# tusen-ai/SST

Hardware: AMD Instinct MI355X
Metric: LiDAR frames/sec (SST backbone fwd+bwd) at Waymo 0.32m voxels (higher is better)
Workload: dtype f32 (storage, accumulation, attention, LayerNorm, reductions: fp32; the dense products of the encoder layers from the EXACT three-way bf16 split of both fp32 operands, six bf16 MFMA products with fp32 accumulation - error vs float64 <= 2 x the fp32 matrix pipe's: tests/test_gpu_dense_f32x6.py)

## Files before the change

### include/sst_amd.h

```cpp
#ifndef SST_AMD_H
#define SST_AMD_H

#include <stdint.h>

#ifdef __cplusplus
extern "C" {
#endif

#define SST_OK 0
#define SST_ERR_ARG (-1)
#define SST_ERR_UNSUPPORTED (-2)
#define SST_ERR_KEYSPACE (-3)

typedef enum { SST_REDUCE_SUM = 0, SST_REDUCE_MEAN = 1, SST_REDUCE_MAX = 2 } sst_reduce_t;

const char* sst_version(void);

int sst_dynamic_voxelize_f32(const float* d_points, int64_t n, int64_t row_stride,
                             const float voxel_size[3], const float coors_range[6],
                             int32_t* d_coors, int64_t coors_stride, int coors_col0, int batch_idx,
                             void* stream);
void sst_dynamic_voxelize_grid(const float voxel_size[3], const float coors_range[6], int32_t grid_xyz[3]);

int64_t sst_scan_workspace_bytes(int64_t n);
// ... 162 lines not shown
  float* out_b;
  int32_t p, bias_side, transpose_out, reserved;
} sst_wgrad_problem_bf16;
int64_t sst_wgrad_group_workspace_bytes(const sst_wgrad_problem_bf16* problems, int n);
int sst_wgrad_group_bf16(const sst_wgrad_problem_bf16* problems, int n, void* d_workspace, void* stream);
typedef struct sst_cast_problem_bf16 {
  const float* src;
  void* dst;
  int64_t ld_src;
  int32_t rows, cols, transpose, reserved;
} sst_cast_problem_bf16;
int sst_cast_group_bf16(const sst_cast_problem_bf16* problems, int n, void* stream);

int sst_gather_rows_f32(const float* d_src, int64_t ld_src, const int32_t* d_idx, int64_t n_out, int c,
                        float fill, float* d_out, int64_t ld_out, void* stream);
int sst_add_table_rows_f32(const float* d_x, int64_t ldx, const float* d_table, int64_t ld_table, const int32_t* d_idx, int64_t m,
                           int c, float* d_out, int64_t ld_out, void* stream);
int sst_scatter_rows_f32(const float* d_src, int64_t ld_src, const int32_t* d_idx, int64_t n_src, int c,
                         float* d_out, int64_t ld_out, void* stream);

int sst_add_layernorm_act_fwd_f32(const float* d_x, const float* d_res, const float* d_weight, const float* d_bias,
                                  int64_t m, int c, float eps, int act, float* d_y, float* d_sum, float* d_stats,
                                  void* stream);
int sst_add_layernorm_act_bwd_f32(const float* d_dy, const float* d_sum, const float* d_stats, const float* d_weight,
                                  const float* d_bias, int act, int64_t m, int c, float* d_dx, float* d_dweight,
                                  float* d_dbias, void* d_workspace, void* stream);
int sst_add_layernorm_fwd_f32(const float* d_x, const float* d_res, const float* d_weight, const float* d_bias,
                              int64_t m, int c, float eps, float* d_y, float* d_sum, float* d_stats,
                              void* stream);
int sst_add_layernorm_pos_fwd_f32(const float* d_x, const float* d_res, const float* d_weight, const float* d_bias, int64_t m,
                                  int c, float eps, float* d_y, float* d_sum, float* d_stats, const float* d_pos_table,
                                  const int32_t* d_pos_idx, float* d_y_plus_pos, void* stream);
int64_t sst_add_layernorm_bwd_workspace_bytes(int64_t m, int c);
int sst_add_layernorm_bwd_f32(const float* d_dy, const float* d_sum, const float* d_stats,
                              const float* d_weight, int64_t m, int c, float* d_dx, float* d_dweight,
                              float* d_dbias, void* d_workspace, void* stream);
int64_t sst_colsum_workspace_bytes(int64_t m, int c);
int sst_colsum_f32(const float* d_x, int64_t m, int c, int64_t ld, float* d_out, void* d_workspace, void* stream);

int64_t sst_weight_grad_workspace_bytes(int64_t m, int out, int in);
int sst_weight_grad_f32(const float* d_dy, const float* d_x, int64_t m, int out, int in, int64_t ld_dy,
                        int64_t ld_x, float* d_dw, float* d_db, void* d_workspace, void* stream);
typedef struct sst_wgrad_problem_f32 {
  const float* dy;
  const float* x;
  int64_t m, ld_dy, ld_x;
  float* dw;
  float* db;
  int32_t out, in;
  const float* x_add_rows;
  const int32_t* x_add_index;
} sst_wgrad_problem_f32;
int64_t sst_weight_grad_group_workspace_bytes(const sst_wgrad_problem_f32* problems, int n);
int sst_weight_grad_group_f32(const sst_wgrad_problem_f32* problems, int n, void* d_workspace, void* stream);
int64_t sst_weight_grad_group_f32x6_workspace_bytes(const sst_wgrad_problem_f32* problems, int n);
int sst_weight_grad_group_f32x6(const sst_wgrad_problem_f32* problems, int n, void* d_workspace, void* stream);
int sst_weight_grad_group_f32x6_plan(const sst_wgrad_problem_f32* problems, int n, int* tiles, int* slices,
                                     int64_t* tokens_per_slice, int* lean_slices);

int64_t sst_bn_workspace_bytes(int64_t n, int c);
int sst_bn_stats_f32(const float* d_x, int64_t n, int c, int64_t ld, float* d_mean, float* d_var,
                     void* d_workspace, void* stream);
int sst_bn_act_fwd_f32(const float* d_x, int64_t n, int c, int64_t ldx, const float* d_scale,
                       const float* d_shift, int act, float* d_y, int64_t ldy, void* stream);
int sst_bn_act_bwd_reduce_f32(const float* d_dy, const float* d_x, int64_t n, int c, int64_t lddy, int64_t ldx,
                              const float* d_mean, const float* d_invstd, const float* d_scale,
                              const float* d_shift, int act, float* d_sum_g, float* d_sum_gxhat,
                              void* d_workspace, void* stream);
int sst_bn_act_bwd_apply_f32(const float* d_dy, const float* d_x, int64_t n, int c, int64_t lddy, int64_t ldx,
                             const float* d_mean, const float* d_invstd, const float* d_scale,
                             const float* d_shift, const float* d_coef_a, const float* d_coef_b, float coef_scale,
                             int act, float* d_dx, int64_t lddx, void* stream);
int sst_bn_prepare_f32(const float* d_x, int64_t n, int c, int64_t ld, const float* d_weight, const float* d_bias,
                       float eps, float* d_running_mean, float* d_running_var, float factor, float* d_out4,
                       void* d_workspace, void* stream);
int sst_bn_prepare_tracked_f32(const float* d_x, int64_t n, int c, int64_t ld, const float* d_weight,
                               const float* d_bias, float eps, float* d_running_mean, float* d_running_var,
                               float factor, int64_t* d_num_batches_tracked, float* d_out4, void* d_workspace,
                               void* stream);
int sst_vfe_linear_moments_f32(const float* d_x, int64_t ldx, int64_t n, int k, const float* d_w, int64_t ldw, int c,
                               float* d_y, int64_t ldy, void* d_workspace, void* stream);
int sst_bn_prepare_from_partials_f32(int64_t n, int c, const float* d_weight, const float* d_bias, float eps,
                                     float* d_running_mean, float* d_running_var, float factor,
                                     int64_t* d_num_batches_tracked, float* d_out4, void* d_workspace, void* stream);
int sst_bn_stats_from_partials_f32(int64_t n, int c, float* d_mean, float* d_var, void* d_workspace, void* stream);
int sst_bn_act_pool_bwd_reduce_f32(const float* d_dy, const float* d_x, int64_t n, int c, int64_t lddy, int64_t ldx,
                                   const float* d_mean, const float* d_invstd, const float* d_scale, const float* d_shift,
                                   int act, const int32_t* d_group, const int32_t* d_arg, const float* d_dpool, int64_t ldp,
                                   float* d_sum_g, float* d_sum_gxhat, void* d_workspace, void* stream);
int sst_bn_act_pool_bwd_apply_f32(const float* d_dy, const float* d_x, int64_t n, int c, int64_t lddy, int64_t ldx,
                                  const float* d_mean, const float* d_invstd, const float* d_scale, const float* d_shift,
                                  const float* d_coef_a, const float* d_coef_b, float coef_scale, int act,
                                  const int32_t* d_group, const int32_t* d_arg, const float* d_dpool, int64_t ldp, float* d_dx,
                                  int64_t lddx, void* stream);
int sst_bn_act_res_fwd_f32(const float* d_x, int64_t n, int c, int64_t ldx, const float* d_res, int64_t ldr,
                           const float* d_scale, const float* d_shift, int act, float* d_y, int64_t ldy, void* stream);
int sst_bn_act_res_bwd_reduce_f32(const float* d_dy, const float* d_x, const float* d_res, int64_t n, int c,
                                  int64_t lddy, int64_t ldx, int64_t ldr, const float* d_mean, const float* d_invstd,
                                  const float* d_scale, const float* d_shift, int act, float* d_sum_g,
                                  float* d_sum_gxhat, void* d_workspace, void* stream);
int sst_bn_act_res_bwd_apply_f32(const float* d_dy, const float* d_x, const float* d_res, int64_t n, int c,
                                 int64_t lddy, int64_t ldx, int64_t ldr, const float* d_mean, const float* d_invstd,
                                 const float* d_scale, const float* d_shift, const float* d_coef_a,
                                 const float* d_coef_b, float coef_scale, int act, float* d_dres, int64_t lddres,
                                 float* d_dx, int64_t lddx, void* stream);

int sst_tall_linear_f32(const float* d_x, int64_t ldx, const float* d_w, int64_t ldw, const float* d_bias,
                        int64_t m, int n, int k, int trans_w, int accumulate, float* d_y, int64_t ldy,
                        void* stream);
int sst_tall_linear_ln_f32(const float* d_x, int64_t ldx, const float* d_w, int64_t ldw, const float* d_bias, int64_t m, int k,
                           const float* d_res, int64_t ldres, const float* d_ln_weight, const float* d_ln_bias, float eps,
                           float* d_y, float* d_sum, float* d_stats, const float* d_pos_table, const int32_t* d_pos_idx,
                           float* d_y_plus_pos, void* stream);
int sst_tall_linear_epi_f32x3(const float* d_x, int64_t ldx, const float* d_w, int64_t ldw, int trans_w, const float* d_bias,
                              int64_t m, int k, int n, int epilogue, const float* d_aux_in, float* d_aux_out, int64_t ldaux,
                              float* d_y, int64_t ldy, void* stream);
int sst_tall_linear_ln_f32x3(const float* d_x, int64_t ldx, const float* d_w, int64_t ldw, const float* d_bias, int64_t m, int k,
                             const float* d_res, int64_t ldres, const float* d_ln_weight, const float* d_ln_bias, float eps,
                             float* d_y, float* d_sum, float* d_stats, const float* d_pos_table, const int32_t* d_pos_idx,
                             float* d_y_plus_pos, void* stream);
int sst_tall_linear_epi_f32x6(const float* d_x, int64_t ldx, const float* d_w, int64_t ldw, int trans_w, const float* d_bias,
                              int64_t m, int k, int n, int epilogue, const float* d_aux_in, float* d_aux_out, int64_t ldaux,
                              float* d_y, int64_t ldy, void* stream);
int sst_tall_linear_epi2_f32x6(const float* d_x, const float* d_x2, int x2_from_col, int64_t ldx, const float* d_w, int64_t ldw,
                               int trans_w, const float* d_bias, int64_t m, int k, int n, int epilogue, const float* d_aux_in,
                               float* d_aux_out, int64_t ldaux, float* d_y, int64_t ldy, void* stream);
int sst_tall_linear_add_rows_f32x6(const float* d_x, int64_t ldx, const float* d_w, int64_t ldw, int64_t m, int k, int n,
                                   const float* d_rows, int64_t ldrows, const int32_t* d_row_index, float* d_y, int64_t ldy,
                                   void* stream);
int sst_inproj_pos_f32x6(const float* d_x, int64_t ldx, const float* d_rows, const int32_t* d_index, const float* d_w, int64_t ldw,
                         const float* d_bias, int64_t m, float* d_y, int64_t ldy, void* stream);
int sst_tall_linear_f32x6_partition(int64_t m, int groups, int64_t* row_blocks, int64_t* rows_per_wave);
int sst_tall_linear_ln_f32x6(const float* d_x, int64_t ldx, const float* d_w, int64_t ldw, const float* d_bias, int64_t m, int k,
                             const float* d_res, int64_t ldres, const float* d_ln_weight, const float* d_ln_bias, float eps,
                             float* d_y, float* d_sum, float* d_stats, const float* d_pos_table, const int32_t* d_pos_idx,
                             float* d_y_plus_pos, void* stream);
int sst_add_layernorm_bwd2_f32(const float* d_dy, const float* d_dy2, const float* d_sum, const float* d_stats,
                               const float* d_weight, int64_t m, int c, float* d_dx, float* d_dweight, float* d_dbias,
                               void* d_workspace, void* stream);
typedef struct sst_encoder_layer_fwd_args {
  int64_t m, n_windows;
  int32_t n_heads, act, max_tokens, impl;
  float eps, scale;
  const float *x, *xp;
  const float *w_in, *b_in, *w_out, *b_out, *w1, *b1, *w2, *b2, *n1w, *n1b, *n2w, *n2b;
  const int32_t *tok, *winoff, *order;
  const float* pos_table;
  const int32_t* pos_idx;
  float *qkv, *o, *lse, *y1, *s1, *st1, *pre, *h, *s2, *y2, *st2, *y2p;
  const float* head_scale;
  void* wpack;
  const float* xpos_table;
  const int32_t* xpos_idx;
} sst_encoder_layer_fwd_args;
typedef struct sst_encoder_layer_bwd_args {
  int64_t m, n_windows;
  int32_t n_heads, act, max_tokens, impl;
  float eps, scale;
  const float *dy2, *dy2p;
  const float *x, *xp, *qkv, *o, *lse, *s1, *st1, *y1, *pre, *h, *s2, *st2;
  const float *w_in, *w_out, *w1, *w2, *n1w, *n2w;
  const int32_t *tok, *winoff, *order;
  float *ds2, *dpre, *ds1, *d_o, *dqkv;
  float *dw_in, *db_in, *dwo, *dbo, *dw1, *db1, *dw2, *db2, *dn1w, *dn1b, *dn2w, *dn2b;
  void* workspace;
  const float* head_scale;
  float* cos_r;
  float* dy1;
  const void* wpack;
  const float* xpos_table;
  const int32_t* xpos_idx;
} sst_encoder_layer_bwd_args;
int64_t sst_encoder_layer_bwd_workspace_bytes(int64_t m, int n_heads);
int64_t sst_encoder_layer_wpack_bytes(void);
int sst_encoder_layer_fwd_f32x6(const sst_encoder_layer_fwd_args* args, void* stream);
int sst_encoder_layer_bwd_f32x6(const sst_encoder_layer_bwd_args* args, void* stream);

typedef struct sst_encoder_tail_fwd_args {
  int64_t m;
  int32_t act, reserved;
  float eps, reserved_f;
  const float *o, *x;
  const void* packed;
  const float *b_out, *b1, *b2, *n1w, *n1b, *n2w, *n2b;
  const float* pos_table;
  const int32_t* pos_idx;
  float *s1, *st1, *y1, *pre, *h, *s2, *st2, *y2, *y2p;
} sst_encoder_tail_fwd_args;
typedef struct sst_encoder_tail_bwd_args {
  int64_t m;
  int32_t act, reserved;
  const float *dy2, *dy2p, *s2, *st2, *pre, *s1, *st1;
  const void* packed;
  const float *n1w, *n2w;
  float *ds2, *dpre, *ds1, *d_o;
  float *dn2w, *dn2b, *dn1w, *dn1b;
  void* workspace;
} sst_encoder_tail_bwd_args;
int64_t sst_encoder_tail_pack_bytes(void);
int sst_encoder_tail_pack_f32x6(const float* d_w_out, const float* d_w1, const float* d_w2, void* d_packed, void* stream);
int sst_encoder_tail_pack_f32x6_many(const float* const* d_w_out, const float* const* d_w1, const float* const* d_w2,
                                     void* const* d_packed, int n, void* stream);
int64_t sst_encoder_tail_bwd_workspace_bytes(int64_t m);
int sst_encoder_tail_fwd_f32x6(const sst_encoder_tail_fwd_args* args, void* stream);
int sst_encoder_tail_bwd_f32x6(const sst_encoder_tail_bwd_args* args, void* stream);

typedef struct sst_encoder_tail_fwd_bf16_args {
  int64_t m;
  int32_t act, reserved;
  float eps, reserved_f;
  const void *o, *x;
  const void* packed;
  const float *b_out, *b1, *b2, *n1w, *n1b, *n2w, *n2b;
  const float* pos_table;
  const int32_t* pos_idx;
  void* s1;
  float* st1;
  void *y1, *pre, *h, *s2;
  float* st2;
  void *y2, *y2p;
} sst_encoder_tail_fwd_bf16_args;
typedef struct sst_encoder_tail_bwd_bf16_args {
  int64_t m;
  int32_t act, reserved;
  const void *dy2, *dy2p, *s2;
  const float* st2;
  const void *pre, *s1;
  const float* st1;
  const void* packed;
  const float *n1w, *n2w;
  void *ds2, *dpre, *ds1, *d_o;
  float *dn2w, *dn2b, *dn1w, *dn1b;
  void* workspace;
} sst_encoder_tail_bwd_bf16_args;
int64_t sst_encoder_tail_pack_bf16_bytes(void);
int sst_encoder_tail_pack_bf16(const float* d_w_out, const float* d_w1, const float* d_w2, void* d_packed, void* stream);
int sst_encoder_tail_pack_bf16_many(const float* const* d_w_out, const float* const* d_w1, const float* const* d_w2,
                                    void* const* d_packed, int n, void* stream);
int64_t sst_encoder_tail_bwd_bf16_workspace_bytes(int64_t m);
int sst_encoder_tail_fwd_bf16(const sst_encoder_tail_fwd_bf16_args* args, void* stream);
int sst_encoder_tail_bwd_bf16(const sst_encoder_tail_bwd_bf16_args* args, void* stream);

typedef struct sst_encoder_layer_fwd_bf16_args {
  int64_t m, n_windows;
  int32_t n_heads, act, max_tokens, reserved;
  float eps, scale;
  const void *x, *xp;
  const void *wqk, *wv, *wout, *w1, *w2;
  const float *b_in, *b_out, *b1, *b2, *n1w, *n1b, *n2w, *n2b;
  const int32_t *tok, *winoff, *order;
  const float* pos_table;
  const int32_t* pos_idx;
  void *qk, *v, *o;
  float* lse;
  void *y1, *s1;
  float* st1;
  void *pre, *h, *s2;
  float* st2;
  void *y2, *y2p;
  const float* head_scale;
  const void* wpack;
} sst_encoder_layer_fwd_bf16_args;
typedef struct sst_encoder_layer_bwd_bf16_args {
  int64_t m, n_windows;
  int32_t n_heads, act, max_tokens, reserved;
  float eps, scale;
  const void *dy2, *dy2p;
  const void *x, *xp, *qk, *v, *o;
  const float* lse;
  const void* s1;
  const float* st1;
  const void *y1, *pre, *h, *s2;
  const float* st2;
  const void *wqk_t, *wv_t, *wout_t, *w1_t, *w2_t;
  const float *n1w, *n2w;
  const int32_t *tok, *winoff, *order;
  void *ds2, *dpre, *dy1, *ds1, *d_o, *dqkv, *dxp, *dx;
  float *dw_in, *db_in, *dwo, *dbo, *dw1, *db1, *dw2, *db2, *dn1w, *dn1b, *dn2w, *dn2b;
  void* workspace;
  const float* head_scale;
  float* cos_r;
  const void* wpack;
} sst_encoder_layer_bwd_bf16_args;
int64_t sst_encoder_layer_bwd_bf16_workspace_bytes(int64_t m);
int sst_encoder_layer_fwd_bf16(const sst_encoder_layer_fwd_bf16_args* args, void* stream);
int sst_encoder_layer_bwd_bf16(const sst_encoder_layer_bwd_bf16_args* args, void* stream);

int sst_tall_linear_epi_f32(const float* d_x, int64_t ldx, const float* d_w, int64_t ldw, int trans_w, const float* d_bias,
                            int64_t m, int k, int n, int epilogue, const float* d_aux_in, float* d_aux_out, int64_t ldaux,
                            float* d_y, int64_t ldy, void* stream);
int sst_tall_linear_gelu_f32(const float* d_x, int64_t ldx, const float* d_w, int64_t ldw, const float* d_bias,
                             int64_t m, int n, int k, int trans_w, int mode, float* d_aux, float* d_y, int64_t ldy,
                             void* stream);

void* sst_event_create(void);
void sst_event_destroy(void* ev);
float sst_event_elapsed_ms(void* start, void* stop);
int sst_sra_attn_profile_next_fwd(void* start, void* stop);
int sst_sra_attn_profile_next_bwd(void* start, void* stop);

int64_t sst_connected_components_workspace_bytes(int64_t n);
int sst_connected_components_xy_f32(const float* d_points, int64_t ld, const int32_t* d_batch, int64_t n, float dist,
                                    int32_t* d_labels, int32_t* d_num_components, void* d_workspace, void* stream);

int64_t sst_dynamic_point_pool_workspace_bytes(int64_t n_rois, int64_t n_pts);
int sst_dynamic_point_pool_f32(const float* d_rois, const int32_t* d_rois_batch, int64_t n_rois, const float* d_pts,
                               int64_t ld_pts, const int32_t* d_pts_batch, int64_t n_pts, const float* extra_wlh,
                               int max_inbox_point, int64_t max_all_pts, int64_t* d_out_pts_idx,
                               int64_t* d_out_roi_idx, float* d_out_feats, int64_t* d_num_out, void* d_workspace,
                               void* stream);

int sst_spconv_candidates_i32(const int32_t* d_coors, int64_t n, const int32_t* in_shape, const int32_t* out_shape,
                              const int32_t* ksize, const int32_t* stride, const int32_t* padding,
                              const int32_t* dilation, int transpose, int32_t* d_rows, void* stream);
int sst_spconv_inverse_to_map_i32(const int32_t* d_inverse, int64_t total, int32_t* d_in2out, void* stream);
int sst_spconv_grid_subm_i32(const int32_t* d_coors, int64_t n, int batch, const int32_t* shape, const int32_t* ksize,
                             const int32_t* dilation, int32_t* d_grid, int32_t* d_in2out, int32_t* d_out2in,
                             void* stream);
int64_t sst_spconv_grid_conv_workspace_bytes(int64_t cells);
int sst_spconv_grid_conv_count_i32(const int32_t* d_coors, int64_t n, int batch, const int32_t* in_shape,
                                   const int32_t* out_shape, const int32_t* ksize, const int32_t* stride,
                                   const int32_t* padding, const int32_t* dilation, int transpose, void* d_workspace,
                                   int32_t* d_num_out, void* stream);
int sst_spconv_grid_conv_maps_i32(const int32_t* d_coors, int64_t n, int batch, const int32_t* in_shape,
                                  const int32_t* out_shape, const int32_t* ksize, const int32_t* stride,
                                  const int32_t* padding, const int32_t* dilation, int transpose, void* d_workspace,
                                  int64_t m, int32_t* d_outids, int32_t* d_in2out, int32_t* d_out2in, void* stream);
int sst_spconv_subm_map_i32(const int32_t* d_coors, int64_t n, const int32_t* shape, const int32_t* ksize,
                            const int32_t* dilation, const uint64_t* d_sorted_keys, const uint32_t* d_perm,
                            int32_t* d_in2out, void* stream);
int sst_spconv_invert_map_i32(const int32_t* d_in2out, int kvol, int64_t n, int64_t m, int32_t* d_out2in,
                              void* stream);
int64_t sst_spconv_pair_lists_workspace_bytes(int kvol, int64_t n);
int sst_spconv_pair_lists_i32(const int32_t* d_in2out, int kvol, int64_t n, int32_t* d_pairs, int32_t* d_num,
                              void* d_workspace, void* stream);
int sst_spconv_gather_gemm_f32(const float* d_x, int64_t ldx, const int32_t* d_map, int64_t m, int kvol,
                               const float* d_w, int cin, int cout, int trans_w, const float* d_bias, float* d_y,
                               int64_t ldy, int form, void* stream);
int sst_spconv_maxpool_fwd_f32(const float* d_x, int64_t ldx, const int32_t* d_out2in, int64_t m, int kvol, int c,
                               float* d_y, int64_t ldy, void* stream);
int sst_spconv_maxpool_bwd_f32(const float* d_x, int64_t ldx, const float* d_y, int64_t ldy, const float* d_dy,
                               int64_t lddy, const int32_t* d_in2out, int64_t n, int kvol, int c, float* d_dx,
                               int64_t lddx, void* stream);
int64_t sst_spconv_conv_os_workspace_bytes(int kvol, int cin, int cout);
int sst_spconv_conv_os_tile_rows(int64_t m, int cout, int tile_cfg);
int sst_spconv_os_tile_work_i32(const int32_t* d_map, int64_t m, int kvol, int tile_rows, int32_t* d_work, void* stream);
int sst_spconv_conv_os_f32(const float* d_x, int64_t ldx, const int32_t* d_map, int64_t m, int kvol, const float* d_w,
                           int cin, int cout, int trans_w, const float* d_bias, float* d_y, int64_t ldy,
                           int tile_cfg, const int32_t* d_tile_order, void* d_workspace, void* stream);
int sst_spconv_conv_os_f32x3(const float* d_x, int64_t ldx, const int32_t* d_map, int64_t m, int kvol, const float* d_w,
                             int cin, int cout, int trans_w, const float* d_bias, float* d_y, int64_t ldy, int tile_cfg,
                             const int32_t* d_tile_order, void* d_workspace, void* stream);
int64_t sst_spconv_conv_os_f32x6_workspace_bytes(int kvol, int cin, int cout);
int sst_spconv_conv_os_f32x6(const float* d_x, int64_t ldx, const int32_t* d_map, int64_t m, int kvol, const float* d_w,
                             int cin, int cout, int trans_w, const float* d_bias, float* d_y, int64_t ldy, int tile_cfg,
// ... 555 lines not shown
```

### sst_amd/_lib.py

```python
import ctypes
import os
import subprocess

import torch

_HERE = os.path.dirname(os.path.abspath(__file__))
_CSRC = os.path.join(_HERE, 'csrc')
LIB_PATH = os.path.join(_CSRC, 'libsst_amd.so')

_lib = None

c_i64 = ctypes.c_int64
c_i32 = ctypes.c_int
c_f32 = ctypes.c_float
c_ptr = ctypes.c_void_p



class WgradProblemBF16(ctypes.Structure):
    _fields_ = [('a', c_ptr), ('b', c_ptr), ('lda', c_i64), ('ldb', c_i64), ('m', c_i64), ('out_w', c_ptr),
                ('out_b', c_ptr), ('p', ctypes.c_int32), ('bias_side', ctypes.c_int32),
                ('transpose_out', ctypes.c_int32), ('reserved', ctypes.c_int32)]


class CastProblemBF16(ctypes.Structure):
    _fields_ = [('src', c_ptr), ('dst', c_ptr), ('ld_src', c_i64), ('rows', ctypes.c_int32), ('cols', ctypes.c_int32),
                ('transpose', ctypes.c_int32), ('reserved', ctypes.c_int32)]


class ClusterLossTask(ctypes.Structure):
    _fields_ = [('logits', c_ptr), ('reg_preds', c_ptr), ('labels', c_ptr), ('bbox_targets', c_ptr), ('bbox_weights', c_ptr),
                ('d_logits', c_ptr), ('d_reg_preds', c_ptr), ('classes', ctypes.c_int32), ('reserved', ctypes.c_int32)]


class WgradProblemF32(ctypes.Structure):
    _fields_ = [('dy', c_ptr), ('x', c_ptr), ('m', c_i64), ('ld_dy', c_i64), ('ld_x', c_i64), ('dw', c_ptr), ('db', c_ptr),
                ('out', ctypes.c_int32), ('inn', ctypes.c_int32), ('x_add_rows', c_ptr), ('x_add_index', c_ptr)]


def _struct(name, doc, fields):
    return type(name, (ctypes.Structure,), {'__doc__': doc, '_fields_': fields})


_I32 = ctypes.c_int32
RoiAssignArgs = _struct('RoiAssignArgs', 'sst_roi_assign_args of include/sst_amd.h', (
    [(k, ctypes.c_void_p) for k in ('props', 'prop_labels', 'prop_offsets', 'gts', 'gt_labels', 'gt_offsets', 'iou', 'max_iou',
                                    'argmax')]
    + [(k, c_i64) for k in ('n_props', 'n_gts', 'ld')]
    + [(k, _I32) for k in ('prop_cols', 'gt_cols', 'batch', 'num_classes', 'class_mask', 'reserved')]))
RoiSampleArgs = _struct('RoiSampleArgs', 'sst_roi_sample_args of include/sst_amd.h', (
    [(k, ctypes.c_void_p) for k in ('props', 'prop_labels', 'prop_offsets', 'gts', 'gt_labels', 'gt_offsets', 'iou', 'max_iou',
                                    'argmax', 'keys', 'assigned', 'rois', 'src', 'gt_index', 'labels', 'iou_out', 'soft_label',
                                    'reg_mask', 'targets', 'counts')]
    + [(k, c_i64) for k in ('n_props', 'n_gts', 'ld', 'max_props_per_sample')]
    + [(k, _I32) for k in ('prop_cols', 'gt_cols', 'batch', 'num_classes', 'class_mask', 'num', 'num_expected_pos', 'n_pieces')]
    + [(k, ctypes.c_float * 16) for k in ('pos_iou_thr', 'neg_iou_thr', 'min_pos_iou')]
    + [('piece_thr', ctypes.c_float * 8)]
    + [(k, ctypes.c_double * 16) for k in ('cls_pos_thr', 'cls_neg_thr')]
    + [('piece_frac', ctypes.c_double * 8)]))
RoiLossArgs = _struct('RoiLossArgs', 'sst_roi_loss_args of include/sst_amd.h', (
    [(k, ctypes.c_void_p) for k in ('cls_score', 'bbox_pred', 'nonempty', 'rois', 'soft_label', 'reg_mask', 'targets',
                                    'gt_index', 'labels', 'gts')]
    + [(k, c_i64) for k in ('n', 'n_gts')]
    + [(k, _I32) for k in ('roi_cols', 'gt_cols', 'with_corner', 'car_index')]
    + [(k, ctypes.c_float) for k in ('beta', 'w_cls', 'w_reg', 'w_corner')]
    + [('code_weight', ctypes.c_float * 7), ('reserved', ctypes.c_float)]))

AnchorGrid = _struct('AnchorGrid', 'sst_anchor_grid of include/sst_amd.h', (
    [('centers', ctypes.c_void_p)] + [(k, _I32) for k in ('H', 'W', 'n_sizes', 'n_rots')]
    + [('sizes', ctypes.c_float * 3 * 8), ('rots', ctypes.c_float * 4)]))
AnchorLossArgs = _struct('AnchorLossArgs', 'sst_anchor_loss_args of include/sst_amd.h', (
    [(k, ctypes.c_void_p) for k in ('cls_score', 'bbox_pred', 'dir_pred', 'assigned', 'gts', 'gt_labels', 'gt_offsets',
                                    'pos_counts')]
    + [('n_gts', c_i64)]
    + [(k, _I32) for k in ('gt_cols', 'batch', 'num_classes', 'smooth_l1', 'sin_diff', 'reserved')]
    + [(k, ctypes.c_float) for k in ('gamma', 'alpha', 'w_cls', 'w_bbox', 'w_dir', 'beta', 'pos_weight', 'dir_offset')]
    + [('code_weight', ctypes.c_float * 7), ('reserved_f', ctypes.c_float)]))

FgSampleArgs = _struct('FgSampleArgs', 'sst_fg_sample_args of include/sst_amd.h', (
    [(k, ctypes.c_void_p) for k in ('logits', 'votes', 'points', 'batch_idx', 'extra_mask', 'slot', 'mask', 'src', 'centers',
                                    'batch_out', 'points_out', 'info', 'aux', 'aux_out', 'aux_inv')]
    + [(k, c_i64) for k in ('n', 'ld_logits', 'ld_votes', 'ld_points', 'max_rows', 'aux_rows')]
    + [(k, _I32) for k in ('num_classes', 'point_cols', 'batch', 'batch_is_i64', 'apply_rule', 'sample_major')]
    + [('thresholds', ctypes.c_float * 32)]))
FgGatherArgs = _struct('FgGatherArgs', 'sst_fg_gather_args of include/sst_amd.h', (
    [(k, ctypes.c_void_p) for k in ('idx', 'logits', 'votes', 'feats', 'points', 'out', 'points_out')]
    + [(k, c_i64) for k in ('m', 'n', 'ld_logits', 'ld_votes', 'ld_feats', 'ld_points')]
    + [(k, _I32) for k in ('c_logits', 'c_votes', 'c_feats', 'c_points')]))
FgGroupSampleArgs = _struct('FgGroupSampleArgs', 'sst_fg_group_sample_args of include/sst_amd.h', (
    [(k, ctypes.c_void_p) for k in ('logits', 'votes', 'points', 'batch_idx', 'extra_mask', 'slot', 'mask', 'src', 'centers',
                                    'batch_out', 'points_out', 'info')]
    + [(k, c_i64) for k in ('n', 'ld_logits', 'ld_votes', 'ld_points', 'max_rows')]
    + [(k, _I32) for k in ('num_groups', 'num_logits', 'point_cols', 'batch', 'batch_is_i64', 'apply_rule')]
    + [('offset_scale', ctypes.c_float), ('thresholds', ctypes.c_float * 32), ('group_begin', ctypes.c_uint8 * 33),
       ('group_class', ctypes.c_uint8 * 64)]))
FgVirtualRowsArgs = _struct('FgVirtualRowsArgs', 'sst_fg_virtual_rows_args of include/sst_amd.h', (
    [(k, ctypes.c_void_p) for k in ('src', 'centers', 'feats', 'logits', 'points', 'out', 'clipped')]
    + [(k, c_i64) for k in ('m', 'n', 'ld_feats', 'ld_logits', 'ld_points')]
    + [(k, _I32) for k in ('c_feats', 'c_logits', 'c_points', 'reserved')]
    + [('lo', ctypes.c_float * 3), ('hi', ctypes.c_float * 3)]))
DeformConvShape = _struct('DeformConvShape', 'sst_deform_conv_shape of include/sst_amd.h', [
    (k, _I32) for k in ('batch', 'in_channels', 'height', 'width', 'out_channels', 'kernel_h', 'kernel_w', 'stride_h', 'stride_w',
                        'pad_h', 'pad_w', 'dil_h', 'dil_w', 'groups', 'deform_groups', 'reserved')])
OptimHyper = _struct('OptimHyper', 'sst_optim_hyper of include/sst_amd.h', (
    [(k, ctypes.c_double * 8) for k in ('lr', 'wd', 'b1', 'b2', 'eps')]
    + [(k, ctypes.c_double) for k in ('max_norm', 'growth_factor', 'backoff_factor')]
    + [(k, _I32) for k in ('growth_interval', 'scale_mode', 'skip_nonfinite', 'n_groups')]))
TrackletTargetsArgs = _struct('TrackletTargetsArgs', 'sst_tracklet_targets_args of include/sst_amd.h', (
    [(k, ctypes.c_void_p) for k in ('boxes', 'ts', 'scores', 'trk_offsets', 'cand_boxes', 'cand_ts', 'cand_offsets',
                                    'trk_cand_offsets', 'trk_class', 'chosen', 'counts', 'matched', 'overlaps',
                                    'assigned_gt_inds', 'rois', 'src', 'frame_inds', 'gt_index', 'labels', 'iou_out',
                                    'scores_out', 'soft_label', 'reg_mask', 'targets', 'pos_gt_bboxes')]
    + [(k, c_i64) for k in ('n_rows', 'n_cand_rows', 'n_cands', 'n_tracklets')]
    + [(k, _I32) for k in ('num_classes', 'object_centric')]
    + [(k, ctypes.c_float) for k in ('candidate_thresh', 'iou_thr')]
    + [(k, ctypes.c_double * 16) for k in ('cls_pos_thr', 'cls_neg_thr')]))
TrackletRowsArgs = _struct('TrackletRowsArgs', 'sst_tracklet_rows_args of include/sst_amd.h', (
    [(k, ctypes.c_void_p) for k in ('feats', 'xyz', 'pts_frame_inds', 'pts_inds', 'roi_inds', 'roi_frame_inds', 'roi_scores',
                                    'out', 'xyz_out')]
    + [(k, c_i64) for k in ('m', 'n_points', 'n_rois', 'ld_feats', 'ld_xyz')]
    + [(k, _I32) for k in ('feat_cols', 'xyz_cols', 'combined', 'with_roi_scores')]))
IncrArgs = _struct('IncrArgs', 'sst_incr_args of include/sst_amd.h', (
    [('points', ctypes.c_void_p * 16), ('frame_inds', ctypes.c_void_p * 16), ('n_points', c_i64 * 16)]
    + [(k, ctypes.c_void_p) for k in ('boxes', 'box_offsets', 'keys', 'counts', 'out', 'workspace')]
    + [('workspace_bytes', c_i64), ('seg_base', c_i64 * (16 * 20))]
    + [(k, _I32) for k in ('n_samples', 'cols', 'n_frames', 'n_queries', 'n_boxes', 'max_crop_points', 'lower_bound')]
    + [(k, _I32 * 4) for k in ('q_inc', 'q_lo', 'q_hi')]
    + [('q_tag', ctypes.c_float * 4), ('lo', ctypes.c_float * 3), ('vs', ctypes.c_float * 3), ('grid', _I32 * 3)]))
IncrDeltaArgs = _struct('IncrDeltaArgs', 'sst_incr_delta_args of include/sst_amd.h', (
    [('base', ctypes.c_void_p * 8), ('n_base', c_i64 * 8), ('ld_base', c_i64 * 8), ('query', ctypes.c_void_p),
     ('n_query', c_i64), ('ld_query', c_i64), ('mask', ctypes.c_void_p), ('workspace', ctypes.c_void_p),
     ('workspace_bytes', c_i64), ('n_clouds', _I32), ('lower_bound', _I32), ('lo', ctypes.c_float * 3),
     ('vs', ctypes.c_float * 3), ('grid', _I32 * 3)]))
FrameTransformArgs = _struct('FrameTransformArgs', 'sst_frame_transform_args of include/sst_amd.h', (
    [('src', ctypes.c_void_p * 8), ('dst', ctypes.c_void_p * 8), ('n', c_i64 * 8), ('mat', (ctypes.c_float * 12) * 8),
     ('n_clouds', _I32), ('cols', _I32)]))
AugmentParams = _struct('AugmentParams', 'sst_augment_params of include/sst_amd.h', (
    [(k, _I32) for k in ('flip_h', 'flip_v', 'rotate', 'shuffle')]
    + [(k, ctypes.c_float) for k in ('cos', 'sin', 'scale', 'angle')]
    + [('trans', ctypes.c_float * 3), ('reserved', ctypes.c_float), ('range', ctypes.c_float * 6), ('seed', ctypes.c_uint64)]))
AugmentArgs = _struct('AugmentArgs', 'sst_augment_args of include/sst_amd.h', (
    [(k, ctypes.c_void_p) for k in ('points', 'row_offsets', 'n_pasted', 'block_offsets', 'params', 'planes', 'plane_offsets',
                                    'out', 'counts', 'workspace')]
    + [(k, c_i64) for k in ('workspace_bytes', 'n_total')]
    + [(k, _I32) for k in ('batch', 'cols', 'n_blocks', 'n_planes', 'norm_mask', 'reserved')]
    + [('norm_mean', ctypes.c_float * 8), ('norm_std', ctypes.c_float * 8)]))
AugmentBoxArgs = _struct('AugmentBoxArgs', 'sst_augment_box_args of include/sst_amd.h', (
    [(k, ctypes.c_void_p) for k in ('boxes', 'labels', 'box_offsets', 'params', 'boxes_out', 'labels_out', 'counts')]
    + [(k, _I32) for k in ('batch', 'cols', 'n_boxes', 'filter', 'always_rotate', 'reserved')]))
FgGroupOffsets = _struct('FgGroupOffsets', 'sst_fg_group_offsets of include/sst_amd.h', [('off', c_i64 * 33)])

_P = ctypes.c_void_p
EncoderLayerFwdArgs = _struct('EncoderLayerFwdArgs', 'sst_encoder_layer_fwd_args of include/sst_amd.h', (
    [('m', c_i64), ('n_windows', c_i64)] + [(k, ctypes.c_int32) for k in ('n_heads', 'act', 'max_tokens', 'impl')]
    + [('eps', ctypes.c_float), ('scale', ctypes.c_float)]
    + [(k, _P) for k in ('x', 'xp', 'w_in', 'b_in', 'w_out', 'b_out', 'w1', 'b1', 'w2', 'b2', 'n1w', 'n1b', 'n2w', 'n2b',
                         'tok', 'winoff', 'order', 'pos_table', 'pos_idx',
                         'qkv', 'o', 'lse', 'y1', 's1', 'st1', 'pre', 'h', 's2', 'y2', 'st2', 'y2p', 'head_scale', 'wpack',
                         'xpos_table', 'xpos_idx')]))
EncoderLayerBwdArgs = _struct('EncoderLayerBwdArgs', 'sst_encoder_layer_bwd_args of include/sst_amd.h', (
    [('m', c_i64), ('n_windows', c_i64)] + [(k, ctypes.c_int32) for k in ('n_heads', 'act', 'max_tokens', 'impl')]
    + [('eps', ctypes.c_float), ('scale', ctypes.c_float)]
    + [(k, _P) for k in ('dy2', 'dy2p', 'x', 'xp', 'qkv', 'o', 'lse', 's1', 'st1', 'y1', 'pre', 'h', 's2', 'st2',
                         'w_in', 'w_out', 'w1', 'w2', 'n1w', 'n2w', 'tok', 'winoff', 'order',
                         'ds2', 'dpre', 'ds1', 'd_o', 'dqkv',
                         'dw_in', 'db_in', 'dwo', 'dbo', 'dw1', 'db1', 'dw2', 'db2', 'dn1w', 'dn1b', 'dn2w', 'dn2b',
                         'workspace', 'head_scale', 'cos_r', 'dy1', 'wpack', 'xpos_table', 'xpos_idx')]))


EncoderTailFwdArgs = _struct('EncoderTailFwdArgs', 'sst_encoder_tail_fwd_args of include/sst_amd.h', (
    [('m', c_i64), ('act', ctypes.c_int32), ('reserved', ctypes.c_int32), ('eps', ctypes.c_float), ('reserved_f', ctypes.c_float)]
    + [(k, _P) for k in ('o', 'x', 'packed', 'b_out', 'b1', 'b2', 'n1w', 'n1b', 'n2w', 'n2b', 'pos_table', 'pos_idx',
                         's1', 'st1', 'y1', 'pre', 'h', 's2', 'st2', 'y2', 'y2p')]))
EncoderTailBwdArgs = _struct('EncoderTailBwdArgs', 'sst_encoder_tail_bwd_args of include/sst_amd.h', (
    [('m', c_i64), ('act', ctypes.c_int32), ('reserved', ctypes.c_int32)]
    + [(k, _P) for k in ('dy2', 'dy2p', 's2', 'st2', 'pre', 's1', 'st1', 'packed', 'n1w', 'n2w',
                         'ds2', 'dpre', 'ds1', 'd_o', 'dn2w', 'dn2b', 'dn1w', 'dn1b', 'workspace')]))

EncoderTailFwdBF16Args = _struct('EncoderTailFwdBF16Args', 'sst_encoder_tail_fwd_bf16_args of include/sst_amd.h', (
    [('m', c_i64), ('act', ctypes.c_int32), ('reserved', ctypes.c_int32), ('eps', ctypes.c_float), ('reserved_f', ctypes.c_float)]
    + [(k, _P) for k in ('o', 'x', 'packed', 'b_out', 'b1', 'b2', 'n1w', 'n1b', 'n2w', 'n2b', 'pos_table', 'pos_idx',
                         's1', 'st1', 'y1', 'pre', 'h', 's2', 'st2', 'y2', 'y2p')]))
EncoderTailBwdBF16Args = _struct('EncoderTailBwdBF16Args', 'sst_encoder_tail_bwd_bf16_args of include/sst_amd.h', (
    [('m', c_i64), ('act', ctypes.c_int32), ('reserved', ctypes.c_int32)]
    + [(k, _P) for k in ('dy2', 'dy2p', 's2', 'st2', 'pre', 's1', 'st1', 'packed', 'n1w', 'n2w',
                         'ds2', 'dpre', 'ds1', 'd_o', 'dn2w', 'dn2b', 'dn1w', 'dn1b', 'workspace')]))


EncoderLayerFwdBF16Args = _struct('EncoderLayerFwdBF16Args', 'sst_encoder_layer_fwd_bf16_args of include/sst_amd.h', (
    [('m', c_i64), ('n_windows', c_i64)] + [(k, ctypes.c_int32) for k in ('n_heads', 'act', 'max_tokens', 'reserved')]
    + [('eps', ctypes.c_float), ('scale', ctypes.c_float)]
    + [(k, _P) for k in ('x', 'xp', 'wqk', 'wv', 'wout', 'w1', 'w2', 'b_in', 'b_out', 'b1', 'b2', 'n1w', 'n1b', 'n2w', 'n2b',
                         'tok', 'winoff', 'order', 'pos_table', 'pos_idx',
                         'qk', 'v', 'o', 'lse', 'y1', 's1', 'st1', 'pre', 'h', 's2', 'st2', 'y2', 'y2p', 'head_scale', 'wpack')]))
EncoderLayerBwdBF16Args = _struct('EncoderLayerBwdBF16Args', 'sst_encoder_layer_bwd_bf16_args of include/sst_amd.h', (
    [('m', c_i64), ('n_windows', c_i64)] + [(k, ctypes.c_int32) for k in ('n_heads', 'act', 'max_tokens', 'reserved')]
    + [('eps', ctypes.c_float), ('scale', ctypes.c_float)]
    + [(k, _P) for k in ('dy2', 'dy2p', 'x', 'xp', 'qk', 'v', 'o', 'lse', 's1', 'st1', 'y1', 'pre', 'h', 's2', 'st2',
                         'wqk_t', 'wv_t', 'wout_t', 'w1_t', 'w2_t', 'n1w', 'n2w', 'tok', 'winoff', 'order',
                         'ds2', 'dpre', 'dy1', 'ds1', 'd_o', 'dqkv', 'dxp', 'dx',
                         'dw_in', 'db_in', 'dwo', 'dbo', 'dw1', 'db1', 'dw2', 'db2', 'dn1w', 'dn1b', 'dn2w', 'dn2b',
                         'workspace', 'head_scale', 'cos_r', 'wpack')]))


_SIGNATURES = {
    'sst_version': (ctypes.c_char_p, []),
    'sst_dynamic_voxelize_f32': (c_i32, [c_ptr, c_i64, c_i64, c_ptr, c_ptr, c_ptr, c_i64, c_i32, c_i32, c_ptr]),
    'sst_dynamic_voxelize_grid': (None, [c_ptr, c_ptr, c_ptr]),
    'sst_scan_workspace_bytes': (c_i64, [c_i64]),
    'sst_exclusive_scan_i32': (c_i32, [c_ptr, c_ptr, c_i64, c_ptr, c_ptr, c_ptr]),
    'sst_sort_workspace_bytes': (c_i64, [c_i64]),
    'sst_sort_pairs_u64': (c_i32, [c_ptr, c_ptr, c_ptr, c_i64, c_i32, c_ptr, c_ptr]),
    'sst_unique_workspace_bytes': (c_i64, [c_i64]),
    'sst_unique_rows': (c_i32, [c_ptr, c_i32, c_i64, c_i32, c_i64, c_ptr, c_ptr, c_i32,
                                c_ptr, c_ptr, c_ptr, c_ptr, c_ptr, c_ptr, c_ptr]),
    'sst_unpack_keys': (c_i32, [c_ptr, c_i64, c_i32, c_ptr, c_ptr, c_ptr, c_i32, c_i64, c_i32, c_ptr]),
    'sst_segment_reduce_fwd_f32': (c_i32, [c_ptr, c_i64, c_i32, c_ptr, c_ptr, c_ptr, c_i64, c_i32, c_ptr, c_ptr,
                                           c_ptr, c_ptr]),
    'sst_encoder_layer_bwd_workspace_bytes': (c_i64, [c_i64, c_i32]),
    'sst_tall_linear_f32x6_partition': (c_i32, [c_i64, c_i32, c_ptr, c_ptr]),
    'sst_inproj_pos_f32x6': (c_i32, [c_ptr, c_i64, c_ptr, c_ptr, c_ptr, c_i64, c_ptr, c_i64, c_ptr, c_i64, c_ptr]),
    'sst_encoder_layer_wpack_bytes': (c_i64, []),
    'sst_encoder_layer_fwd_f32x6': (c_i32, [c_ptr, c_ptr]),
    'sst_encoder_layer_bwd_f32x6': (c_i32, [c_ptr, c_ptr]),
    'sst_encoder_tail_pack_bytes': (c_i64, []),
    'sst_encoder_tail_pack_f32x6': (c_i32, [c_ptr, c_ptr, c_ptr, c_ptr, c_ptr]),
    'sst_encoder_tail_pack_f32x6_many': (c_i32, [c_ptr, c_ptr, c_ptr, c_ptr, c_i32, c_ptr]),
    'sst_encoder_tail_bwd_workspace_bytes': (c_i64, [c_i64]),
    'sst_encoder_tail_fwd_f32x6': (c_i32, [c_ptr, c_ptr]),
    'sst_encoder_tail_bwd_f32x6': (c_i32, [c_ptr, c_ptr]),
    'sst_encoder_tail_pack_bf16_bytes': (c_i64, []),
    'sst_encoder_tail_pack_bf16': (c_i32, [c_ptr, c_ptr, c_ptr, c_ptr, c_ptr]),
    'sst_encoder_tail_pack_bf16_many': (c_i32, [c_ptr, c_ptr, c_ptr, c_ptr, c_i32, c_ptr]),
    'sst_encoder_tail_bwd_bf16_workspace_bytes': (c_i64, [c_i64]),
    'sst_encoder_tail_fwd_bf16': (c_i32, [c_ptr, c_ptr]),
    'sst_encoder_tail_bwd_bf16': (c_i32, [c_ptr, c_ptr]),
    'sst_encoder_layer_bwd_bf16_workspace_bytes': (c_i64, [c_i64]),
    'sst_encoder_layer_fwd_bf16': (c_i32, [c_ptr, c_ptr]),
    'sst_encoder_layer_bwd_bf16': (c_i32, [c_ptr, c_ptr]),
    'sst_segment_reduce_work_words': (c_i64, [c_i64, c_i64, c_i32]),
    'sst_segment_reduce_fwd_work_f32': (c_i32, [c_ptr, c_i64, c_i32, c_ptr, c_ptr, c_ptr, c_i64, c_i32, c_ptr, c_ptr,
                                                c_ptr, c_ptr, c_i64, c_ptr, c_ptr, c_ptr]),
    'sst_vfe_linear_moments_f32': (c_i32, [c_ptr, c_i64, c_i64, c_i32, c_ptr, c_i64, c_i32, c_ptr, c_i64, c_ptr, c_ptr]),
    'sst_bn_prepare_from_partials_f32': (c_i32, [c_i64, c_i32, c_ptr, c_ptr, c_f32, c_ptr, c_ptr, c_f32, c_ptr, c_ptr, c_ptr,
                                                 c_ptr]),
    'sst_bn_stats_from_partials_f32': (c_i32, [c_i64, c_i32, c_ptr, c_ptr, c_ptr, c_ptr]),
    'sst_bn_act_pool_bwd_reduce_f32': (c_i32, [c_ptr, c_ptr, c_i64, c_i32, c_i64, c_i64, c_ptr, c_ptr, c_ptr, c_ptr, c_i32,
                                               c_ptr, c_ptr, c_ptr, c_i64, c_ptr, c_ptr, c_ptr, c_ptr]),
    'sst_bn_act_pool_bwd_apply_f32': (c_i32, [c_ptr, c_ptr, c_i64, c_i32, c_i64, c_i64, c_ptr, c_ptr, c_ptr, c_ptr, c_ptr,
                                              c_ptr, c_f32, c_i32, c_ptr, c_ptr, c_ptr, c_i64, c_ptr, c_i64, c_ptr]),
    'sst_tall_linear_add_rows_f32x6': (c_i32, [c_ptr, c_i64, c_ptr, c_i64, c_i64, c_i32, c_i32, c_ptr, c_i64, c_ptr, c_ptr,
                                               c_i64, c_ptr]),
    'sst_segment_long_scratch_bytes': (c_i64, [c_i64, c_i64, c_i32]),
    'sst_segment_reduce_long_f32': (c_i32, [c_ptr, c_i64, c_i32, c_ptr, c_ptr, c_i32, c_ptr, c_i64, c_i32, c_ptr, c_ptr, c_ptr,
                                            c_ptr]),
    'sst_segment_reduce_profile_next': (c_i32, [c_ptr, c_ptr]),
    'sst_segment_reduce_bwd_f32': (c_i32, [c_ptr, c_i64, c_i32, c_ptr, c_i32, c_ptr, c_ptr, c_ptr, c_i64, c_i32,
                                           c_ptr, c_ptr, c_ptr]),
    'sst_ingroup_rank_workspace_bytes': (c_i64, [c_i64]),
    'sst_ingroup_rank_i64': (c_i32, [c_ptr, c_i64, c_i32, c_ptr, c_ptr, c_ptr]),
    'sst_window_coors': (c_i32, [c_ptr, c_i32, c_i64, c_ptr, c_ptr, c_ptr, c_ptr, c_ptr, c_ptr, c_ptr]),
    'sst_window_order_i32': (c_i32, [c_ptr, c_i32, c_i32, c_ptr, c_ptr]),
    'sst_region_batching_workspace_bytes': (c_i64, [c_i64]),
    'sst_region_batching': (c_i32, [c_ptr, c_ptr, c_i64, c_i32, c_ptr, c_i32] + [c_ptr] * 15 + [c_ptr, c_ptr]),
    'sst_frame_windows_per_sample': (c_i64, [c_ptr, c_ptr]),
    'sst_frame_voxels_i32': (c_i32, [c_ptr, c_ptr, c_ptr, c_i64, c_i32, c_ptr, c_i32, c_ptr, c_ptr, c_ptr, c_ptr,
                                     c_ptr, c_ptr, c_ptr]),
    'sst_window_plan_workspace_bytes': (c_i64, [c_i64, c_i64]),
    'sst_window_plan_i32': (c_i32, [c_ptr, c_ptr, c_i64, c_i32, c_ptr, c_ptr, c_ptr, c_i32, ctypes.c_uint32] + [c_ptr] * 11),
    'sst_sra_attn_fwd_f32': (c_i32, [c_ptr, c_ptr, c_ptr, c_i64, c_i64, c_i64, c_ptr, c_ptr, c_i64, c_i32,
                                     c_f32, c_i32, c_i32, c_ptr, c_i64, c_ptr, c_ptr]),
    'sst_sra_attn_bwd_f32': (c_i32, [c_ptr] * 6 + [c_i64] * 5 + [c_ptr, c_ptr, c_i64, c_i64, c_i32, c_f32,
                                                                 c_i32, c_i32, c_ptr, c_ptr, c_ptr,
                                                                 c_i64, c_i64, c_i64, c_ptr, c_ptr]),
    'sst_sra_attn_fwd_ord_f32': (c_i32, [c_ptr, c_ptr, c_ptr, c_i64, c_i64, c_i64, c_ptr, c_ptr, c_ptr, c_i64, c_i32,
                                         c_f32, c_i32, c_i32, c_ptr, c_i64, c_ptr, c_ptr]),
    'sst_sra_attn_bwd_ord_f32': (c_i32, [c_ptr] * 6 + [c_i64] * 5 + [c_ptr, c_ptr, c_ptr, c_i64, c_i64, c_i32, c_f32,
                                                                     c_i32, c_i32, c_ptr, c_ptr, c_ptr,
                                                                     c_i64, c_i64, c_i64, c_ptr, c_ptr]),
    'sst_sra_attn_bwd_workspace_bytes': (c_i64, [c_i64, c_i32]),
    'sst_sra_attn_cos_fwd_f32': (c_i32, [c_ptr, c_ptr, c_ptr, c_i64, c_i64, c_i64, c_ptr, c_ptr, c_ptr, c_i64, c_i32,
                                         c_ptr, c_i32, c_ptr, c_i64, c_ptr, c_ptr]),
    'sst_sra_attn_cos_bwd_f32': (c_i32, [c_ptr] * 6 + [c_i64] * 5 + [c_ptr, c_ptr, c_ptr, c_i64, c_i64, c_i32, c_ptr,
                                                                     c_i32, c_ptr, c_ptr, c_ptr,
                                                                     c_i64, c_i64, c_i64, c_ptr, c_ptr]),
    'sst_sra_attn_fwd_bf16': (c_i32, [c_ptr, c_ptr, c_ptr, c_i64, c_i64, c_i64, c_ptr, c_ptr, c_i64, c_i32, c_f32, c_i32,
                                      c_ptr, c_i64, c_ptr, c_ptr]),
    'sst_sra_attn_bwd_bf16': (c_i32, [c_ptr] * 6 + [c_i64] * 5 + [c_ptr, c_ptr, c_i64, c_i32, c_f32, c_i32, c_ptr, c_ptr,
                                                                  c_ptr, c_i64, c_i64, c_i64, c_ptr]),
    'sst_sra_attn_bf16_profile_next': (c_i32, [c_i32, c_ptr, c_ptr]),
    'sst_sra_attn_fwd_ord_bf16': (c_i32, [c_ptr, c_ptr, c_ptr, c_i64, c_i64, c_i64, c_ptr, c_ptr, c_ptr, c_i64, c_i32, c_f32,
                                          c_i32, c_ptr, c_i64, c_ptr, c_ptr]),
    'sst_sra_attn_bwd_ord_bf16': (c_i32, [c_ptr] * 6 + [c_i64] * 5 + [c_ptr, c_ptr, c_ptr, c_i64, c_i32, c_f32, c_i32, c_ptr,
                                                                      c_ptr, c_ptr, c_i64, c_i64, c_i64, c_ptr]),
    'sst_sra_attn_cos_fwd_bf16': (c_i32, [c_ptr, c_ptr, c_ptr, c_i64, c_i64, c_i64, c_ptr, c_ptr, c_ptr, c_i64, c_i32, c_ptr,
                                          c_i32, c_ptr, c_i64, c_ptr, c_ptr]),
    'sst_sra_attn_cos_bwd_bf16': (c_i32, [c_ptr] * 6 + [c_i64] * 5 + [c_ptr, c_ptr, c_ptr, c_i64, c_i32, c_ptr, c_i32, c_ptr,
                                                                      c_ptr, c_ptr, c_i64, c_i64, c_i64, c_ptr, c_ptr]),
    'sst_add_layernorm_fwd_bf16': (c_i32, [c_ptr, c_ptr, c_ptr, c_ptr, c_i64, c_i32, c_f32, c_ptr, c_ptr, c_ptr, c_ptr,
                                           c_ptr, c_ptr, c_ptr]),
    'sst_add_layernorm_bwd_bf16': (c_i32, [c_ptr, c_ptr, c_ptr, c_ptr, c_ptr, c_i64, c_i32, c_ptr, c_ptr, c_ptr, c_ptr,
                                           c_ptr]),
    'sst_cast_add_pos_bf16': (c_i32, [c_ptr, c_i32, c_i64, c_i32, c_ptr, c_ptr, c_ptr, c_ptr]),
    'sst_weight_grad_group_workspace_bytes': (c_i64, [c_ptr, c_i32]),
    'sst_weight_grad_group_f32': (c_i32, [c_ptr, c_i32, c_ptr, c_ptr]),
    'sst_weight_grad_group_f32x6_workspace_bytes': (c_i64, [c_ptr, c_i32]),
    'sst_weight_grad_group_f32x6': (c_i32, [c_ptr, c_i32, c_ptr, c_ptr]),
    'sst_weight_grad_group_f32x6_plan': (c_i32, [c_ptr, c_i32, c_ptr, c_ptr, c_ptr, c_ptr]),
    'sst_tall_linear_ln_f32': (c_i32, [c_ptr, c_i64, c_ptr, c_i64, c_ptr, c_i64, c_i32, c_ptr, c_i64, c_ptr, c_ptr, c_f32, c_ptr,
                                       c_ptr, c_ptr, c_ptr, c_ptr, c_ptr, c_ptr]),
    'sst_tall_linear_ln_f32x3': (c_i32, [c_ptr, c_i64, c_ptr, c_i64, c_ptr, c_i64, c_i32, c_ptr, c_i64, c_ptr, c_ptr, c_f32, c_ptr,
                                         c_ptr, c_ptr, c_ptr, c_ptr, c_ptr, c_ptr]),
    'sst_tall_linear_epi_f32x3': (c_i32, [c_ptr, c_i64, c_ptr, c_i64, c_i32, c_ptr, c_i64, c_i32, c_i32, c_i32, c_ptr, c_ptr,
                                          c_i64, c_ptr, c_i64, c_ptr]),
    'sst_tall_linear_ln_f32x6': (c_i32, [c_ptr, c_i64, c_ptr, c_i64, c_ptr, c_i64, c_i32, c_ptr, c_i64, c_ptr, c_ptr, c_f32, c_ptr,
                                         c_ptr, c_ptr, c_ptr, c_ptr, c_ptr, c_ptr]),
    'sst_tall_linear_epi_f32x6': (c_i32, [c_ptr, c_i64, c_ptr, c_i64, c_i32, c_ptr, c_i64, c_i32, c_i32, c_i32, c_ptr, c_ptr,
                                          c_i64, c_ptr, c_i64, c_ptr]),
    'sst_tall_linear_epi2_f32x6': (c_i32, [c_ptr, c_ptr, c_i32, c_i64, c_ptr, c_i64, c_i32, c_ptr, c_i64, c_i32, c_i32, c_i32,
                                           c_ptr, c_ptr, c_i64, c_ptr, c_i64, c_ptr]),
    'sst_add_layernorm_bwd2_f32': (c_i32, [c_ptr, c_ptr, c_ptr, c_ptr, c_ptr, c_i64, c_i32, c_ptr, c_ptr, c_ptr, c_ptr, c_ptr]),
    'sst_tall_linear_epi_f32': (c_i32, [c_ptr, c_i64, c_ptr, c_i64, c_i32, c_ptr, c_i64, c_i32, c_i32, c_i32, c_ptr, c_ptr,
                                        c_i64, c_ptr, c_i64, c_ptr]),
    'sst_tall_linear_bf16': (c_i32, [c_ptr, c_i64, c_ptr, c_ptr, c_i64, c_i32, c_i32, c_i32, c_ptr, c_ptr, c_i64, c_ptr,
                                     c_i64, c_ptr]),
    'sst_tall_linear_bf16_partition': (c_i32, [c_i64, c_i32, c_i32, c_i32, c_ptr, c_ptr]),
    'sst_tall_linear_ln_bf16': (c_i32, [c_ptr, c_i64, c_ptr, c_ptr, c_i64, c_i32, c_ptr, c_i64, c_ptr, c_ptr, c_f32, c_ptr, c_ptr,
                                        c_ptr, c_ptr, c_ptr, c_ptr, c_ptr]),
    'sst_wgrad_group_workspace_bytes': (c_i64, [c_ptr, c_i32]),
    'sst_wgrad_group_bf16': (c_i32, [c_ptr, c_i32, c_ptr, c_ptr]),
    'sst_cast_group_bf16': (c_i32, [c_ptr, c_i32, c_ptr]),
    'sst_gather_rows_f32': (c_i32, [c_ptr, c_i64, c_ptr, c_i64, c_i32, c_f32, c_ptr, c_i64, c_ptr]),
    'sst_add_table_rows_f32': (c_i32, [c_ptr, c_i64, c_ptr, c_i64, c_ptr, c_i64, c_i32, c_ptr, c_i64, c_ptr]),
    'sst_scatter_rows_f32': (c_i32, [c_ptr, c_i64, c_ptr, c_i64, c_i32, c_ptr, c_i64, c_ptr]),
    'sst_add_layernorm_fwd_f32': (c_i32, [c_ptr, c_ptr, c_ptr, c_ptr, c_i64, c_i32, c_f32, c_ptr, c_ptr, c_ptr,
                                          c_ptr]),
    'sst_add_layernorm_bwd_workspace_bytes': (c_i64, [c_i64, c_i32]),
    'sst_add_layernorm_pos_fwd_f32': (c_i32, [c_ptr, c_ptr, c_ptr, c_ptr, c_i64, c_i32, c_f32, c_ptr, c_ptr, c_ptr, c_ptr, c_ptr,
                                              c_ptr, c_ptr]),
    'sst_add_layernorm_act_fwd_f32': (c_i32, [c_ptr, c_ptr, c_ptr, c_ptr, c_i64, c_i32, c_f32, c_i32, c_ptr, c_ptr, c_ptr,
                                              c_ptr]),
    'sst_add_layernorm_act_bwd_f32': (c_i32, [c_ptr, c_ptr, c_ptr, c_ptr, c_ptr, c_i32, c_i64, c_i32, c_ptr, c_ptr, c_ptr,
                                              c_ptr, c_ptr]),
    'sst_add_layernorm_bwd_f32': (c_i32, [c_ptr, c_ptr, c_ptr, c_ptr, c_i64, c_i32, c_ptr, c_ptr, c_ptr, c_ptr,
                                          c_ptr]),
    'sst_weight_grad_workspace_bytes': (c_i64, [c_i64, c_i32, c_i32]),
    'sst_weight_grad_f32': (c_i32, [c_ptr, c_ptr, c_i64, c_i32, c_i32, c_i64, c_i64, c_ptr, c_ptr, c_ptr, c_ptr]),
    'sst_colsum_workspace_bytes': (c_i64, [c_i64, c_i32]),
    'sst_colsum_f32': (c_i32, [c_ptr, c_i64, c_i32, c_i64, c_ptr, c_ptr, c_ptr]),
    'sst_tall_linear_f32': (c_i32, [c_ptr, c_i64, c_ptr, c_i64, c_ptr, c_i64, c_i32, c_i32, c_i32, c_i32, c_ptr, c_i64,
                                    c_ptr]),
    'sst_tall_linear_gelu_f32': (c_i32, [c_ptr, c_i64, c_ptr, c_i64, c_ptr, c_i64, c_i32, c_i32, c_i32, c_i32, c_ptr, c_ptr,
                                         c_i64, c_ptr]),
    'sst_connected_components_workspace_bytes': (c_i64, [c_i64]),
    'sst_connected_components_xy_f32': (c_i32, [c_ptr, c_i64, c_ptr, c_i64, ctypes.c_float, c_ptr, c_ptr, c_ptr, c_ptr]),
    'sst_dynamic_point_pool_workspace_bytes': (c_i64, [c_i64, c_i64]),
    'sst_dynamic_point_pool_f32': (c_i32, [c_ptr, c_ptr, c_i64, c_ptr, c_i64, c_ptr, c_i64, c_ptr, c_i32, c_i64, c_ptr,
                                           c_ptr, c_ptr, c_ptr, c_ptr, c_ptr]),
    'sst_spconv_candidates_i32': (c_i32, [c_ptr, c_i64, c_ptr, c_ptr, c_ptr, c_ptr, c_ptr, c_ptr, c_i32, c_ptr, c_ptr]),
    'sst_spconv_inverse_to_map_i32': (c_i32, [c_ptr, c_i64, c_ptr, c_ptr]),
    'sst_spconv_grid_subm_i32': (c_i32, [c_ptr, c_i64, c_i32, c_ptr, c_ptr, c_ptr, c_ptr, c_ptr, c_ptr, c_ptr]),
    'sst_spconv_grid_conv_workspace_bytes': (c_i64, [c_i64]),
    'sst_spconv_grid_conv_count_i32': (c_i32, [c_ptr, c_i64, c_i32, c_ptr, c_ptr, c_ptr, c_ptr, c_ptr, c_ptr, c_i32, c_ptr,
                                               c_ptr, c_ptr]),
    'sst_spconv_grid_conv_maps_i32': (c_i32, [c_ptr, c_i64, c_i32, c_ptr, c_ptr, c_ptr, c_ptr, c_ptr, c_ptr, c_i32, c_ptr,
                                              c_i64, c_ptr, c_ptr, c_ptr, c_ptr]),
    'sst_spconv_subm_map_i32': (c_i32, [c_ptr, c_i64, c_ptr, c_ptr, c_ptr, c_ptr, c_ptr, c_ptr, c_ptr]),
    'sst_spconv_invert_map_i32': (c_i32, [c_ptr, c_i32, c_i64, c_i64, c_ptr, c_ptr]),
    'sst_spconv_pair_lists_workspace_bytes': (c_i64, [c_i32, c_i64]),
    'sst_spconv_pair_lists_i32': (c_i32, [c_ptr, c_i32, c_i64, c_ptr, c_ptr, c_ptr, c_ptr]),
    'sst_spconv_gather_gemm_f32': (c_i32, [c_ptr, c_i64, c_ptr, c_i64, c_i32, c_ptr, c_i32, c_i32, c_i32, c_ptr, c_ptr,
                                           c_i64, c_i32, c_ptr]),
    'sst_spconv_conv_os_workspace_bytes': (c_i64, [c_i32, c_i32, c_i32]),
    'sst_spconv_conv_os_f32': (c_i32, [c_ptr, c_i64, c_ptr, c_i64, c_i32, c_ptr, c_i32, c_i32, c_i32, c_ptr, c_ptr, c_i64,
                                       c_i32, c_ptr, c_ptr, c_ptr]),
    'sst_spconv_conv_os_tile_rows': (c_i32, [c_i64, c_i32, c_i32]),
    'sst_spconv_conv_os_f32x3': (c_i32, [c_ptr, c_i64, c_ptr, c_i64, c_i32, c_ptr, c_i32, c_i32, c_i32, c_ptr, c_ptr, c_i64,
                                         c_i32, c_ptr, c_ptr, c_ptr]),
    'sst_spconv_conv_os_f32x6': (c_i32, [c_ptr, c_i64, c_ptr, c_i64, c_i32, c_ptr, c_i32, c_i32, c_i32, c_ptr, c_ptr, c_i64,
                                         c_i32, c_ptr, c_ptr, c_ptr]),
# ... 291 lines not shown
```

### sst_amd/csrc/layer_exec.hip

```cpp
#include <stdint.h>
#include "common.h"

namespace {

enum { kEpiBias = 0, kEpiGelu = 1, kEpiRelu = 2, kEpiMulGeluGrad = 3, kEpiMulReluGrad = 4, kEpiAdd = 5 };
constexpr int kC = 128, kFF = 256;

int64_t wg_ws(int64_t m, int which) {
  sst_wgrad_problem_f32 p[5];
  float* const any = (float*)(uintptr_t)256;
  for (auto& q : p) {
    q.dy = q.x = any;
    q.dw = q.db = any;
    q.m = m;
    q.x_add_rows = nullptr, q.x_add_index = nullptr;
  }
  if (which == 0 || which == 2) {
    p[0].ld_dy = kC, p[0].ld_x = kFF, p[0].out = kC, p[0].in = kFF;
    p[1].ld_dy = kFF, p[1].ld_x = kC, p[1].out = kFF, p[1].in = kC;
    if (which == 0) return sst_weight_grad_group_f32x6_workspace_bytes(p, 2);
    p[2].ld_dy = kC, p[2].ld_x = kC, p[2].out = kC, p[2].in = kC;
    p[3].ld_dy = 3 * kC, p[3].ld_x = kC, p[3].out = 2 * kC, p[3].in = kC;
    p[4].ld_dy = 3 * kC, p[4].ld_x = kC, p[4].out = kC, p[4].in = kC;
    return sst_weight_grad_group_f32x6_workspace_bytes(p, 5);
  }
  p[0].ld_dy = kC, p[0].ld_x = kC, p[0].out = kC, p[0].in = kC;
  p[1].ld_dy = 3 * kC, p[1].ld_x = kC, p[1].out = 2 * kC, p[1].in = kC;
  p[2].ld_dy = 3 * kC, p[2].ld_x = kC, p[2].out = kC, p[2].in = kC;
  return sst_weight_grad_group_f32x6_workspace_bytes(p, 3);
}

int64_t wg_ws_bf16(int64_t m) {
  sst_wgrad_problem_bf16 p[5];
  for (auto& q : p) q.m = m;
  p[0].p = 2 * kC, p[1].p = kC, p[2].p = kC, p[3].p = kFF, p[4].p = kFF;
  return sst_wgrad_group_workspace_bytes(p, 5);
}

}

extern "C" {

int64_t sst_encoder_layer_bwd_workspace_bytes(int64_t m, int n_heads) {
  if (m < 0 || n_heads < 1) return SST_ERR_ARG;
  const int64_t a = sst_encoder_tail_bwd_workspace_bytes(m), d = sst_sra_attn_bwd_workspace_bytes(m, n_heads), e = wg_ws(m, 2);
  if (a < 0 || d < 0 || e < 0) return SST_ERR_UNSUPPORTED;
  return sst_align_up(a, 256) + sst_align_up(e, 256) + sst_align_up(d, 256) + 256;
}

int64_t sst_encoder_layer_wpack_bytes(void) { return sst_encoder_tail_pack_bytes(); }

int sst_encoder_layer_fwd_f32x6(const sst_encoder_layer_fwd_args* a, void* stream) {
  if (!a || a->m < 0 || a->n_heads * 16 != kC || (a->act != 1 && a->act != 2)) return SST_ERR_ARG;
  if (a->m == 0) return SST_OK;
  if (!a->x || !a->qkv || !a->o || !a->lse || !a->y1 || !a->st1 || !a->pre || !a->h || !a->s2 || !a->y2 || !a->st2)
    return SST_ERR_ARG;
  if (!a->xp && (!a->xpos_table || !a->xpos_idx)) return SST_ERR_ARG;
  const int64_t m = a->m;
  int rc;
  if (a->xp == nullptr)
    rc = sst_inproj_pos_f32x6(a->x, kC, a->xpos_table, a->xpos_idx, a->w_in, kC, a->b_in, m, a->qkv, 3 * kC, stream);
  else
    rc = sst_tall_linear_epi2_f32x6(a->xp, a->x, 2 * kC, kC, a->w_in, kC, 0, a->b_in, m, kC, 3 * kC, kEpiBias, nullptr, nullptr, 0,
                                    a->qkv, 3 * kC, stream);
  if (rc) return rc;
  if (a->head_scale != nullptr)
    rc = sst_sra_attn_cos_fwd_f32(a->qkv, a->qkv + kC, a->qkv + 2 * kC, 3 * kC, 3 * kC, 3 * kC, a->tok, a->winoff, a->order,
                                  a->n_windows, a->n_heads, a->head_scale, a->max_tokens, a->o, kC, a->lse, stream);
  else
    rc = sst_sra_attn_fwd_ord_f32(a->qkv, a->qkv + kC, a->qkv + 2 * kC, 3 * kC, 3 * kC, 3 * kC, a->tok, a->winoff, a->order,
                                  a->n_windows, a->n_heads, a->scale, a->max_tokens, a->impl, a->o, kC, a->lse, stream);
  if (rc) return rc;
  if (!a->wpack) return SST_ERR_ARG;
  if (a->w_out || a->w1 || a->w2) {
    rc = sst_encoder_tail_pack_f32x6(a->w_out, a->w1, a->w2, a->wpack, stream);
    if (rc) return rc;
  }
  sst_encoder_tail_fwd_args t;
  t.m = m, t.act = a->act, t.reserved = 0, t.eps = a->eps, t.reserved_f = 0.f;
  t.o = a->o, t.x = a->x, t.packed = a->wpack;
  t.b_out = a->b_out, t.b1 = a->b1, t.b2 = a->b2, t.n1w = a->n1w, t.n1b = a->n1b, t.n2w = a->n2w, t.n2b = a->n2b;
  t.pos_table = a->pos_table, t.pos_idx = a->pos_idx;
  t.s1 = a->s1, t.st1 = a->st1, t.y1 = a->y1, t.pre = a->pre, t.h = a->h, t.s2 = a->s2, t.st2 = a->st2, t.y2 = a->y2;
  t.y2p = a->pos_table != nullptr ? a->y2p : nullptr;
  return sst_encoder_tail_fwd_f32x6(&t, stream);
}

int sst_encoder_layer_bwd_f32x6(const sst_encoder_layer_bwd_args* a, void* stream) {
  if (!a || a->m < 0 || a->n_heads * 16 != kC || (a->act != 1 && a->act != 2)) return SST_ERR_ARG;
  if (a->m == 0) return SST_OK;
  if (!a->dy2 || !a->workspace || !a->ds2 || !a->dpre || !a->ds1 || !a->d_o || !a->dqkv || !a->wpack) return SST_ERR_ARG;
  if (!a->dn2w || !a->dn2b || !a->dn1w || !a->dn1b) return SST_ERR_ARG;
  if (!a->xp && (!a->xpos_table || !a->xpos_idx)) return SST_ERR_ARG;
  const int64_t m = a->m;
  char* ws = (char*)a->workspace;
  void* ws_tail = ws;
  ws += sst_align_up(sst_encoder_tail_bwd_workspace_bytes(m), 256);
  void* ws_wg = ws;
  ws += sst_align_up(wg_ws(m, 2), 256);
  void* ws_sra = ws;
  int rc;
  sst_encoder_tail_bwd_args t;
  t.m = m, t.act = a->act, t.reserved = 0;
  t.dy2 = a->dy2, t.dy2p = a->dy2p, t.s2 = a->s2, t.st2 = a->st2, t.pre = a->pre, t.s1 = a->s1, t.st1 = a->st1;
  t.packed = a->wpack, t.n1w = a->n1w, t.n2w = a->n2w;
  t.ds2 = a->ds2, t.dpre = a->dpre, t.ds1 = a->ds1, t.d_o = a->d_o;
  t.dn2w = a->dn2w, t.dn2b = a->dn2b, t.dn1w = a->dn1w, t.dn1b = a->dn1b;
  t.workspace = ws_tail;
  float *part2 = nullptr, *part1 = nullptr;
  int rows = 0;
  rc = sst_internal_encoder_tail_bwd_f32x6(&t, &part2, &part1, &rows, stream);
  if (rc) return rc;
  sst_colsum_rider riders[2];
  riders[0].partials = part2, riders[0].nb = rows, riders[0].width = 2 * kC, riders[0].split = kC;
  riders[0].out0 = a->dn2w, riders[0].out1 = a->dn2b;
  riders[1].partials = part1, riders[1].nb = rows, riders[1].width = 2 * kC, riders[1].split = kC;
  riders[1].out0 = a->dn1w, riders[1].out1 = a->dn1b;
  if (a->head_scale != nullptr)
    rc = sst_sra_attn_cos_bwd_f32(a->qkv, a->qkv + kC, a->qkv + 2 * kC, a->o, a->d_o, a->lse, 3 * kC, 3 * kC, 3 * kC, kC, kC, a->tok,
                                  a->winoff, a->order, a->n_windows, m, a->n_heads, a->head_scale, a->max_tokens, a->dqkv,
                                  a->dqkv + kC, a->dqkv + 2 * kC, 3 * kC, 3 * kC, 3 * kC, a->cos_r, stream);
  else
    rc = sst_sra_attn_bwd_ord_f32(a->qkv, a->qkv + kC, a->qkv + 2 * kC, a->o, a->d_o, a->lse, 3 * kC, 3 * kC, 3 * kC, kC, kC, a->tok,
                                  a->winoff, a->order, a->n_windows, m, a->n_heads, a->scale, a->max_tokens, a->impl, a->dqkv,
                                  a->dqkv + kC, a->dqkv + 2 * kC, 3 * kC, 3 * kC, 3 * kC, ws_sra, stream);
  if (rc) return rc;
  sst_wgrad_problem_f32 g[5];
  for (auto& q : g) q.x_add_rows = nullptr, q.x_add_index = nullptr;
  g[0].dy = a->ds2, g[0].x = a->h, g[0].m = m, g[0].ld_dy = kC, g[0].ld_x = kFF, g[0].dw = a->dw2, g[0].db = a->db2;
  g[0].out = kC, g[0].in = kFF;
  g[1].dy = a->dpre, g[1].x = a->y1, g[1].m = m, g[1].ld_dy = kFF, g[1].ld_x = kC, g[1].dw = a->dw1, g[1].db = a->db1;
  g[1].out = kFF, g[1].in = kC;
  g[2].dy = a->ds1, g[2].x = a->o, g[2].m = m, g[2].ld_dy = kC, g[2].ld_x = kC, g[2].dw = a->dwo, g[2].db = a->dbo;
  g[2].out = kC, g[2].in = kC;
  g[3].dy = a->dqkv, g[3].x = a->xp ? a->xp : a->x, g[3].m = m, g[3].ld_dy = 3 * kC, g[3].ld_x = kC, g[3].dw = a->dw_in;
  g[3].db = a->db_in, g[3].out = 2 * kC, g[3].in = kC;
  if (!a->xp) g[3].x_add_rows = a->xpos_table, g[3].x_add_index = a->xpos_idx;
  g[4].dy = a->dqkv + 2 * kC, g[4].x = a->x, g[4].m = m, g[4].ld_dy = 3 * kC, g[4].ld_x = kC;
  g[4].dw = a->dw_in + 2 * kC * kC, g[4].db = a->db_in + 2 * kC, g[4].out = kC, g[4].in = kC;
  rc = sst_internal_weight_grad_group_f32x6(g, 5, ws_wg, riders, 2, stream);
  if (rc) return rc;
  return sst_tall_linear_epi_f32x6(a->dqkv, 3 * kC, a->w_in, kC, 1, nullptr, m, 3 * kC, kC, kEpiAdd, a->ds1, nullptr, kC, a->ds1, kC,
                                   stream);
}

int64_t sst_encoder_layer_bwd_bf16_workspace_bytes(int64_t m) {
  if (m < 0) return SST_ERR_ARG;
  const int64_t a = sst_encoder_tail_bwd_bf16_workspace_bytes(m), b = wg_ws_bf16(m);
  if (a < 0 || b < 0) return SST_ERR_UNSUPPORTED;
  return sst_align_up(a, 256) + sst_align_up(b, 256) + 256;
}

int sst_encoder_layer_fwd_bf16(const sst_encoder_layer_fwd_bf16_args* a, void* stream) {
  if (!a || a->m < 0 || a->n_heads * 16 != kC || (a->act != 1 && a->act != 2)) return SST_ERR_ARG;
  if (a->m == 0) return SST_OK;
  if (!a->x || !a->xp || !a->wqk || !a->wv || !a->wout || !a->w1 || !a->w2 || !a->qk || !a->v || !a->o || !a->lse || !a->y1 ||
      !a->st1 || !a->pre || !a->h || !a->y2 || !a->st2)
    return SST_ERR_ARG;
  const int64_t m = a->m;
  const unsigned short* qk = (const unsigned short*)a->qk;
  int rc;
  rc = sst_tall_linear_bf16(a->xp, kC, a->wqk, a->b_in, m, kC, 2 * kC, kEpiBias, nullptr, nullptr, 0, a->qk, 2 * kC, stream);
  if (rc) return rc;
  rc = sst_tall_linear_bf16(a->x, kC, a->wv, a->b_in ? a->b_in + 2 * kC : nullptr, m, kC, kC, kEpiBias, nullptr, nullptr, 0, a->v,
                            kC, stream);
  if (rc) return rc;
  if (a->head_scale != nullptr)
    rc = sst_sra_attn_cos_fwd_bf16(qk, qk + kC, a->v, 2 * kC, 2 * kC, kC, a->tok, a->winoff, a->order, a->n_windows, a->n_heads,
                                   a->head_scale, a->max_tokens, a->o, kC, a->lse, stream);
  else
    rc = sst_sra_attn_fwd_ord_bf16(qk, qk + kC, a->v, 2 * kC, 2 * kC, kC, a->tok, a->winoff, a->order, a->n_windows, a->n_heads,
                                   a->scale, a->max_tokens, a->o, kC, a->lse, stream);
  if (rc) return rc;
  if (!a->wpack) return SST_ERR_ARG;
  sst_encoder_tail_fwd_bf16_args t;
  t.m = m, t.act = a->act, t.reserved = 0, t.eps = a->eps, t.reserved_f = 0.f;
  t.o = a->o, t.x = a->x, t.packed = a->wpack;
  t.b_out = a->b_out, t.b1 = a->b1, t.b2 = a->b2, t.n1w = a->n1w, t.n1b = a->n1b, t.n2w = a->n2w, t.n2b = a->n2b;
  t.pos_table = a->pos_table, t.pos_idx = a->pos_idx;
  t.s1 = a->s1, t.st1 = a->st1, t.y1 = a->y1, t.pre = a->pre, t.h = a->h, t.s2 = a->s2, t.st2 = a->st2, t.y2 = a->y2;
  t.y2p = a->pos_table ? a->y2p : nullptr;
  return sst_encoder_tail_fwd_bf16(&t, stream);
}

int sst_encoder_layer_bwd_bf16(const sst_encoder_layer_bwd_bf16_args* a, void* stream) {
  if (!a || a->m < 0 || a->n_heads * 16 != kC || (a->act != 1 && a->act != 2)) return SST_ERR_ARG;
  if (a->m == 0) return SST_OK;
  if (!a->dy2 || !a->workspace || !a->ds2 || !a->dpre || !a->ds1 || !a->d_o || !a->dqkv || !a->dxp || !a->dx ||
      !a->s1 || !a->s2 || !a->wpack)
    return SST_ERR_ARG;
  if (!a->dn2w || !a->dn2b || !a->dn1w || !a->dn1b) return SST_ERR_ARG;
  const int64_t m = a->m;
  char* ws = (char*)a->workspace;
  void* ws_tail = ws;
  ws += sst_align_up(sst_encoder_tail_bwd_bf16_workspace_bytes(m), 256);
  void* ws_wg = ws;
  const unsigned short* qk = (const unsigned short*)a->qk;
  unsigned short* dqkv = (unsigned short*)a->dqkv;
  int rc;
  sst_encoder_tail_bwd_bf16_args t;
  t.m = m, t.act = a->act, t.reserved = 0;
  t.dy2 = a->dy2, t.dy2p = a->dy2p, t.s2 = a->s2, t.st2 = a->st2, t.pre = a->pre, t.s1 = a->s1, t.st1 = a->st1;
  t.packed = a->wpack, t.n1w = a->n1w, t.n2w = a->n2w;
  t.ds2 = a->ds2, t.dpre = a->dpre, t.ds1 = a->ds1, t.d_o = a->d_o;
  t.dn2w = a->dn2w, t.dn2b = a->dn2b, t.dn1w = a->dn1w, t.dn1b = a->dn1b;
  t.workspace = ws_tail;
  float *part2 = nullptr, *part1 = nullptr;
  int rows = 0;
  rc = sst_internal_encoder_tail_bwd_bf16(&t, &part2, &part1, &rows, stream);
  if (rc) return rc;
  sst_colsum_rider riders[2];
  riders[0].partials = part2, riders[0].nb = rows, riders[0].width = 2 * kC, riders[0].split = kC;
  riders[0].out0 = a->dn2w, riders[0].out1 = a->dn2b;
  riders[1].partials = part1, riders[1].nb = rows, riders[1].width = 2 * kC, riders[1].split = kC;
  riders[1].out0 = a->dn1w, riders[1].out1 = a->dn1b;
  if (a->head_scale != nullptr)
    rc = sst_sra_attn_cos_bwd_bf16(qk, qk + kC, a->v, a->o, a->d_o, a->lse, 2 * kC, 2 * kC, kC, kC, kC, a->tok, a->winoff,
                                   a->order, a->n_windows, a->n_heads, a->head_scale, a->max_tokens, dqkv, dqkv + kC,
                                   dqkv + 2 * kC, 3 * kC, 3 * kC, 3 * kC, a->cos_r, stream);
  else
    rc = sst_sra_attn_bwd_ord_bf16(qk, qk + kC, a->v, a->o, a->d_o, a->lse, 2 * kC, 2 * kC, kC, kC, kC, a->tok, a->winoff,
                                   a->order, a->n_windows, a->n_heads, a->scale, a->max_tokens, dqkv, dqkv + kC, dqkv + 2 * kC,
                                   3 * kC, 3 * kC, 3 * kC, stream);
  if (rc) return rc;
  rc = sst_tall_linear_bf16(dqkv, 3 * kC, a->wqk_t, nullptr, m, 2 * kC, kC, kEpiBias, nullptr, nullptr, 0, a->dxp, kC, stream);
  if (rc) return rc;
  rc = sst_tall_linear_bf16(dqkv + 2 * kC, 3 * kC, a->wv_t, nullptr, m, kC, kC, kEpiAdd, a->ds1, nullptr, kC, a->dx, kC, stream);
  if (rc) return rc;
  sst_wgrad_problem_bf16 g[5];
  for (auto& q : g) {
    q.m = m;
    q.ldb = kC;
    q.bias_side = 1;
    q.transpose_out = 0;
    q.reserved = 0;
  }
  g[0].a = dqkv, g[0].lda = 3 * kC, g[0].b = a->xp, g[0].out_w = a->dw_in, g[0].out_b = a->db_in, g[0].p = 2 * kC;
// ... 11 lines not shown
```

### sst_amd/csrc/layer_tail_x6.hip

```cpp
#include <math.h>
#include <stdlib.h>
#include "common.h"
#include "gelu.h"
#include "mfma_tile.h"

#ifndef SST_NT_OUT
#define SST_NT_OUT false
#endif
#ifndef SST_NT_BWD
#define SST_NT_BWD true
#endif

namespace {

struct img3 {
  u32x4 p0, p1, p2;
};
__device__ __forceinline__ img3 split8(const f32x4& a, const f32x4& b) {
  img3 r;
  split8(a, b, r.p0, r.p1, r.p2);
  return r;
}
__device__ __forceinline__ void join8(const img3& v, f32x4& a, f32x4& b) {
#pragma unroll
  for (int i = 0; i < 2; ++i) {
    a[2 * i] = (lo_f(v.p2[i]) + lo_f(v.p1[i])) + lo_f(v.p0[i]);
    a[2 * i + 1] = (hi_f(v.p2[i]) + hi_f(v.p1[i])) + hi_f(v.p0[i]);
    b[2 * i] = (lo_f(v.p2[2 + i]) + lo_f(v.p1[2 + i])) + lo_f(v.p0[2 + i]);
    b[2 * i + 1] = (hi_f(v.p2[2 + i]) + hi_f(v.p1[2 + i])) + hi_f(v.p0[2 + i]);
  }
}

constexpr int kC = 128, kFF = 256, kHC = 32, kNF = kFF / kHC;
constexpr int kI1 = 2 * 4 * kFrag;
constexpr int kI2 = 8 * 1 * kFrag;
constexpr int kIA = 8 * 2 * kFrag;
constexpr int kPart1 = 3 * kI1, kPart2 = 3 * kI2;
constexpr int kSlot = kPart1 + kPart2;
static_assert(3 * kIA <= kSlot, "slot");
#ifndef SST_TAIL_WAVES
#define SST_TAIL_WAVES 4
#endif
constexpr int kWaves = SST_TAIL_WAVES, kNTH = 64 * kWaves, kRowsPerWg = 16 * kWaves;
static_assert(kNTH >= 2 * kC, "one thread per LayerNorm parameter-gradient column");
constexpr int kNChunks = kNF + 2;
constexpr int kPackDir = kNChunks * kSlot;
constexpr int kParF = 6 * kC + kFF;
constexpr int kArea = kSlot;
constexpr int kScr = 2048;
constexpr int kLdsFwd = kArea + kParF * 4 + kWaves * kScr;
constexpr int kLdsBwd = kArea + 2 * kC * 4 + kWaves * 2 * kC * 4 + kWaves * kScr;

struct tail_weights {
  const float* wo;
  const float* w1;
  const float* w2;
};

template <bool BWD>
__device__ __forceinline__ void stage_load(const tail_weights W, int chunk, int t, float (&r)[16]) {
  if (!BWD) {
    if (chunk < 2) {
#pragma unroll
      for (int u = 0; u < 2; ++u) {
        const int idx = t + 512 * u, n = idx >> 3, k8 = (idx & 7) * 8;
        const float* p = W.wo + n * kC + 64 * chunk + k8;
        const f32x4 a = *(const f32x4*)p, b = *(const f32x4*)(p + 4);
#pragma unroll
        for (int e = 0; e < 4; ++e) r[8 * u + e] = a[e], r[8 * u + 4 + e] = b[e];
      }
    } else {
      const int j = chunk - 2;
      {
        const float* p = W.w1 + (size_t)(kHC * j + (t >> 4)) * kC + (t & 15) * 8;
        const f32x4 a = *(const f32x4*)p, b = *(const f32x4*)(p + 4);
#pragma unroll
        for (int e = 0; e < 4; ++e) r[e] = a[e], r[4 + e] = b[e];
      }
      {
        const float* p = W.w2 + (size_t)(t >> 2) * kFF + kHC * j + (t & 3) * 8;
        const f32x4 a = *(const f32x4*)p, b = *(const f32x4*)(p + 4);
#pragma unroll
        for (int e = 0; e < 4; ++e) r[8 + e] = a[e], r[12 + e] = b[e];
      }
    }
  } else {
    if (chunk >= kNF) {
      const int q = chunk - kNF;
#pragma unroll
      for (int u = 0; u < 2; ++u) {
        const int idx = t + 512 * u, jn = idx & 127, k8 = (idx >> 7) * 8;
        const float* p = W.wo + (size_t)(64 * q + k8) * kC + jn;
#pragma unroll
        for (int e = 0; e < 8; ++e) r[8 * u + e] = p[e * kC];
      }
    } else {
      const int j = chunk;
      {
        const float* p = W.w2 + (size_t)((t >> 5) * 8) * kFF + kHC * j + (t & 31);
#pragma unroll
        for (int e = 0; e < 8; ++e) r[e] = p[e * kFF];
      }
      {
        const float* p = W.w1 + (size_t)(kHC * j + (t >> 7) * 8) * kC + (t & 127);
#pragma unroll
        for (int e = 0; e < 8; ++e) r[8 + e] = p[e * kC];
      }
    }
  }
}

__device__ __forceinline__ void store_images(unsigned char* base, int image_bytes, int off, const float* v) {
  const f32x4 a = {v[0], v[1], v[2], v[3]}, b = {v[4], v[5], v[6], v[7]};
  const img3 s = split8(a, b);
  *(u32x4*)(base + off) = s.p0;
  *(u32x4*)(base + image_bytes + off) = s.p1;
  *(u32x4*)(base + 2 * image_bytes + off) = s.p2;
}

template <bool BWD>
__device__ __forceinline__ void stage_store(unsigned char* slot, int chunk, int t, const float (&r)[16]) {
  const bool outproj = BWD ? chunk >= kNF : chunk < 2;
  if (outproj) {
#pragma unroll
    for (int u = 0; u < 2; ++u) {
      const int idx = t + 512 * u;
      const int n = BWD ? (idx & 127) : (idx >> 3), k8 = BWD ? (idx >> 7) * 8 : (idx & 7) * 8;
      store_images(slot, kIA, frag_off(w_lds_row(n), k8, 2), r + 8 * u);
    }
  } else {
    const int n1 = BWD ? (t & 31) : (t >> 4), k1 = BWD ? (t >> 5) * 8 : (t & 15) * 8;
    store_images(slot, kI1, frag_off(w_lds_row(n1), k1, 4), r);
    const int n2 = BWD ? (t & 127) : (t >> 2), k2 = BWD ? (t >> 7) * 8 : (t & 3) * 8;
    store_images(slot + kPart1, kI2, frag_off(w_lds_row(n2), k2, 1), r + 8);
  }
}

constexpr int kPackMany = 16;
struct pack_batch {
  tail_weights w[kPackMany];
  unsigned char* dst[kPackMany];
};
__global__ __launch_bounds__(512) void encoder_tail_pack_k(const pack_batch B) {
  extern __shared__ __attribute__((aligned(16))) unsigned char lds[];
  const int layer = blockIdx.x / (2 * kNChunks), blk = blockIdx.x % (2 * kNChunks);
  const tail_weights W = B.w[layer];
  const int chunk = blk % kNChunks, dir = blk / kNChunks;
  float r[16];
  if (dir == 0) {
    stage_load<false>(W, chunk, threadIdx.x, r);
    stage_store<false>(lds, chunk, threadIdx.x, r);
  } else {
    stage_load<true>(W, chunk, threadIdx.x, r);
    stage_store<true>(lds, chunk, threadIdx.x, r);
  }
  __syncthreads();
  unsigned char* dst = B.dst[layer] + (size_t)blk * kSlot;
  for (int i = threadIdx.x; i < kSlot / 16; i += 512) *(u32x4*)(dst + 16 * i) = *(const u32x4*)(lds + 16 * i);
}

__device__ __forceinline__ void barrier_lds_only() { asm volatile("s_waitcnt lgkmcnt(0)\n\ts_barrier" ::: "memory"); }

struct tile_io {
  unsigned char* scr;
  int frag_off0;
  int row_off[2];
  int64_t rrow[2];
  bool rvalid[2];
  int rcol;
};
__device__ __forceinline__ tile_io make_tile_io(unsigned char* scr, int lane, int64_t r0, int64_t m) {
  tile_io t;
  const int c = lane & 15, g = lane >> 4;
  t.scr = scr;
  t.frag_off0 = c * 128 + (((2 * g) ^ (c & 7)) << 4);
#pragma unroll
  for (int i = 0; i < 2; ++i) {
    const int r = 8 * i + (lane >> 3), p = lane & 7;
    t.row_off[i] = r * 128 + ((p ^ (r & 7)) << 4);
    t.rvalid[i] = r0 + r < m;
    t.rrow[i] = t.rvalid[i] ? r0 + r : m - 1;
  }
  t.rcol = (lane & 7) * 4;
  return t;
}
template <bool STREAM>
__device__ __forceinline__ void store32(const tile_io& t, float* __restrict__ base, int64_t ld, int col0, const f32x4& v0,
                                        const f32x4& v1) {
  *(f32x4*)(t.scr + t.frag_off0) = v0;
  *(f32x4*)(t.scr + (t.frag_off0 ^ 16)) = v1;
#pragma unroll
  for (int i = 0; i < 2; ++i) {
    const f32x4 w = *(const f32x4*)(t.scr + t.row_off[i]);
    if (t.rvalid[i]) {
      if (STREAM)
        __builtin_nontemporal_store(w, (f32x4*)(base + t.rrow[i] * ld + col0 + t.rcol));
      else
        *(f32x4*)(base + t.rrow[i] * ld + col0 + t.rcol) = w;
    }
  }
}
__device__ __forceinline__ void load32_issue(const tile_io& t, const float* __restrict__ base, int64_t ld, int col0, f32x4 (&w)[2]) {
#pragma unroll
  for (int i = 0; i < 2; ++i) w[i] = *(const f32x4*)(base + t.rrow[i] * ld + col0 + t.rcol);
}
__device__ __forceinline__ void load32_finish(const tile_io& t, const f32x4 (&w)[2], f32x4& v0, f32x4& v1) {
#pragma unroll
  for (int i = 0; i < 2; ++i) *(f32x4*)(t.scr + t.row_off[i]) = w[i];
  v0 = *(const f32x4*)(t.scr + t.frag_off0);
  v1 = *(const f32x4*)(t.scr + (t.frag_off0 ^ 16));
}

template <int HALF>
__device__ __forceinline__ void mma_half(const unsigned char* slot, int lane_off, const f32x4 (&x)[4][2], f32x4 (&acc)[8]) {
#pragma unroll
  for (int s2 = 0; s2 < 2; ++s2) {
    const img3 xs = split8(x[2 * HALF + s2][0], x[2 * HALF + s2][1]);
#pragma unroll
    for (int t0 = 0; t0 < 8; t0 += 4) {
      u32x4 a0[4], a1[4], a2[4];
#pragma unroll
      for (int u = 0; u < 4; ++u) {
        const int off = lane_off + ((t0 + u) * 2 + s2) * kFrag;
        a0[u] = *(const u32x4*)(slot + off);
        a1[u] = *(const u32x4*)(slot + kIA + off);
        a2[u] = *(const u32x4*)(slot + 2 * kIA + off);
      }
#pragma unroll
      for (int u = 0; u < 4; ++u) acc[t0 + u] = mma32(a0[u], xs.p2, acc[t0 + u]);
#pragma unroll
      for (int u = 0; u < 4; ++u) acc[t0 + u] = mma32(a2[u], xs.p0, acc[t0 + u]);
#pragma unroll
      for (int u = 0; u < 4; ++u) acc[t0 + u] = mma32(a1[u], xs.p1, acc[t0 + u]);
#pragma unroll
      for (int u = 0; u < 4; ++u) acc[t0 + u] = mma32(a0[u], xs.p1, acc[t0 + u]);
#pragma unroll
      for (int u = 0; u < 4; ++u) acc[t0 + u] = mma32(a1[u], xs.p0, acc[t0 + u]);
#pragma unroll
      for (int u = 0; u < 4; ++u) acc[t0 + u] = mma32(a0[u], xs.p0, acc[t0 + u]);
    }
  }
}

__device__ __forceinline__ f32x4 add4(const f32x4& a, const f32x4& b) {
  return (f32x4){a[0] + b[0], a[1] + b[1], a[2] + b[2], a[3] + b[3]};
}

__device__ __forceinline__ void mma_first(const unsigned char* slot, int lane_off1, const img3 (&y)[4], f32x4& out0, f32x4& out1) {
  const f32x4 z = {0.f, 0.f, 0.f, 0.f};
  f32x4 am[2] = {z, z}, ca[2] = {z, z}, cb[2] = {z, z};
#pragma unroll
  for (int s = 0; s < 4; ++s) {
    u32x4 a0[2], a1[2], a2[2];
#pragma unroll
    for (int T = 0; T < 2; ++T) {
      const int off = lane_off1 + (T * 4 + s) * kFrag;
      a0[T] = *(const u32x4*)(slot + off);
      a1[T] = *(const u32x4*)(slot + kI1 + off);
      a2[T] = *(const u32x4*)(slot + 2 * kI1 + off);
    }
#pragma unroll
    for (int T = 0; T < 2; ++T) ca[T] = mma32(a0[T], y[s].p2, ca[T]);
#pragma unroll
    for (int T = 0; T < 2; ++T) cb[T] = mma32(a0[T], y[s].p1, cb[T]);
#pragma unroll
    for (int T = 0; T < 2; ++T) ca[T] = mma32(a2[T], y[s].p0, ca[T]);
#pragma unroll
    for (int T = 0; T < 2; ++T) am[T] = mma32(a0[T], y[s].p0, am[T]);
#pragma unroll
    for (int T = 0; T < 2; ++T) ca[T] = mma32(a1[T], y[s].p1, ca[T]);
#pragma unroll
    for (int T = 0; T < 2; ++T) cb[T] = mma32(a1[T], y[s].p0, cb[T]);
  }
  out0 = add4(am[0], add4(cb[0], ca[0]));
  out1 = add4(am[1], add4(cb[1], ca[1]));
}

__device__ __forceinline__ void mma_second(const unsigned char* slot2, int lane_off2, const img3& h, f32x4 (&acc)[8]) {
#pragma unroll
  for (int t0 = 0; t0 < 8; t0 += 4) {
    u32x4 a0[4], a1[4], a2[4];
#pragma unroll
    for (int u = 0; u < 4; ++u) {
      const int off = lane_off2 + (t0 + u) * kFrag;
      a0[u] = *(const u32x4*)(slot2 + off);
      a1[u] = *(const u32x4*)(slot2 + kI2 + off);
      a2[u] = *(const u32x4*)(slot2 + 2 * kI2 + off);
    }
#pragma unroll
    for (int u = 0; u < 4; ++u) acc[t0 + u] = mma32(a0[u], h.p2, acc[t0 + u]);
#pragma unroll
    for (int u = 0; u < 4; ++u) acc[t0 + u] = mma32(a2[u], h.p0, acc[t0 + u]);
#pragma unroll
    for (int u = 0; u < 4; ++u) acc[t0 + u] = mma32(a1[u], h.p1, acc[t0 + u]);
#pragma unroll
    for (int u = 0; u < 4; ++u) acc[t0 + u] = mma32(a0[u], h.p1, acc[t0 + u]);
#pragma unroll
    for (int u = 0; u < 4; ++u) acc[t0 + u] = mma32(a1[u], h.p0, acc[t0 + u]);
#pragma unroll
    for (int u = 0; u < 4; ++u) acc[t0 + u] = mma32(a0[u], h.p0, acc[t0 + u]);
  }
}

__device__ __forceinline__ void ln_stats(f32x4 (&v)[4][2], float eps, float& mean, float& rstd) {
  float sum = 0.f;
#pragma unroll
  for (int s = 0; s < 4; ++s)
#pragma unroll
    for (int r = 0; r < 4; ++r) sum += v[s][0][r] + v[s][1][r];
  sum += __shfl_xor(sum, 16, 64);
  sum += __shfl_xor(sum, 32, 64);
  mean = sum * (1.f / 128.f);
  float sq = 0.f;
#pragma unroll
  for (int s = 0; s < 4; ++s)
#pragma unroll
    for (int h = 0; h < 2; ++h)
#pragma unroll
      for (int r = 0; r < 4; ++r) {
        v[s][h][r] -= mean;
        sq = fmaf(v[s][h][r], v[s][h][r], sq);
      }
  sq += __shfl_xor(sq, 16, 64);
  sq += __shfl_xor(sq, 32, 64);
  rstd = rsqrtf(sq * (1.f / 128.f) + eps);
}

struct tail_fwd_params {
  const float *o, *x;
  const unsigned char* packed;
  const float *b_out, *b1, *b2, *n1w, *n1b, *n2w, *n2b;
  float eps;
  int64_t m;
  float *s1, *st1, *y1, *pre, *h, *s2, *st2, *y2;
  const float* pos_table;
  const int32_t* pos_idx;
  float* y2p;
};

template <int ACT>
__global__ __launch_bounds__(kNTH, 2) void encoder_tail_fwd_x6_k(const tail_fwd_params P) {
  extern __shared__ __attribute__((aligned(16))) unsigned char lds[];
  float* par = (float*)(lds + kArea);
  const int lane = threadIdx.x & 63, g = lane >> 4, c = lane & 15, wave = threadIdx.x >> 6;
  const int64_t r0 = (int64_t)blockIdx.x * kRowsPerWg + wave * 16;
  const bool valid = r0 + c < P.m;
  const int64_t row = valid ? r0 + c : P.m - 1;
  const tile_io io = make_tile_io(lds + kArea + kParF * 4 + wave * kScr, lane, r0, P.m);
  const unsigned char* packed = P.packed;
  unsigned char* const part2 = lds + kPart1;
  dma_pieces<kWaves>(packed, lds, 3 * kIA / 1024, wave, lane);
  f32x4 ob[4][2], xr[4][2];
  {
    f32x4 wo[4][2], wx[4][2];
#pragma unroll
    for (int s = 0; s < 4; ++s) load32_issue(io, P.o, kC, 32 * s, wo[s]);
#pragma unroll
    for (int s = 0; s < 4; ++s) load32_issue(io, P.x, kC, 32 * s, wx[s]);
#pragma unroll
    for (int s = 0; s < 4; ++s) load32_finish(io, wo[s], ob[s][0], ob[s][1]);
#pragma unroll
    for (int s = 0; s < 4; ++s) load32_finish(io, wx[s], xr[s][0], xr[s][1]);
  }
  for (int i = threadIdx.x; i < kC; i += kNTH) {
    par[i] = P.b_out ? P.b_out[i] : 0.f;
    par[kC + i] = P.n1w[i];
    par[2 * kC + i] = P.n1b[i];
    par[3 * kC + i] = P.b2 ? P.b2[i] : 0.f;
    par[4 * kC + i] = P.n2w[i];
    par[5 * kC + i] = P.n2b[i];
  }
  for (int i = threadIdx.x; i < kFF; i += kNTH) par[6 * kC + i] = P.b1 ? P.b1[i] : 0.f;

  const int lane_offA = lane * 16, lane_off1 = lane * 16, lane_off2 = lane * 16;
  const f32x4 z4 = {0.f, 0.f, 0.f, 0.f};
  f32x4 acc[8];
#pragma unroll
  for (int T = 0; T < 8; ++T) acc[T] = z4;
  img3 yi[4];

  barrier_drain();
  mma_half<0>(lds, lane_offA, ob, acc);
  barrier_drain();
  dma_pieces<kWaves>(packed + kSlot, lds, 3 * kIA / 1024, wave, lane);
  barrier_drain();
  mma_half<1>(lds, lane_offA, ob, acc);
  barrier_drain();
  dma_pieces<kWaves>(packed + 2 * kSlot, lds, kSlot / 1024, wave, lane);
  {
    f32x4 v[4][2];
#pragma unroll
    for (int s = 0; s < 4; ++s) {
      const int n0 = 32 * s + 8 * g;
      v[s][0] = acc[2 * s] + *(const f32x4*)(par + n0) + xr[s][0];
      v[s][1] = acc[2 * s + 1] + *(const f32x4*)(par + n0 + 4) + xr[s][1];
      if (P.s1 != nullptr) store32<true>(io, P.s1, kC, 32 * s, v[s][0], v[s][1]);
    }
    float mean, rstd;
    ln_stats(v, P.eps, mean, rstd);
    if (valid && g == 0) ((float2*)P.st1)[row] = make_float2(mean, rstd);
#pragma unroll
    for (int s = 0; s < 4; ++s) {
      const int n0 = 32 * s + 8 * g;
      const f32x4 y0 = v[s][0] * rstd * *(const f32x4*)(par + kC + n0) + *(const f32x4*)(par + 2 * kC + n0);
      const f32x4 y1 = v[s][1] * rstd * *(const f32x4*)(par + kC + n0 + 4) + *(const f32x4*)(par + 2 * kC + n0 + 4);
      store32<true>(io, P.y1, kC, 32 * s, y0, y1);
      yi[s] = split8(y0, y1);
    }
#pragma unroll
    for (int T = 0; T < 8; ++T) acc[T] = z4;
  }
  barrier_drain();
  f32x4 sp0 = z4, sp1 = z4, sh0 = z4, sh1 = z4;
#pragma unroll 1
  for (int j = 0; j < kNF; ++j) {
    if (j > 0) {
      store32<true>(io, P.pre, kFF, kHC * (j - 1), sp0, sp1);
      store32<true>(io, P.h, kFF, kHC * (j - 1), sh0, sh1);
    }
    f32x4 p0, p1;
    mma_first(lds, lane_off1, yi, p0, p1);
    const int nl = kHC * j + 8 * g;
    p0 = add4(p0, *(const f32x4*)(par + 6 * kC + nl));
    p1 = add4(p1, *(const f32x4*)(par + 6 * kC + nl + 4));
    f32x4 h0, h1;
#pragma unroll
    for (int r = 0; r < 4; ++r) {
      h0[r] = ACT == 1 ? gelu_f(p0[r]) : fmaxf(p0[r], 0.f);
      h1[r] = ACT == 1 ? gelu_f(p1[r]) : fmaxf(p1[r], 0.f);
    }
    const img3 hs = split8(h0, h1);
    barrier_drain();
    if (j + 1 < kNF) dma_pieces<kWaves>(packed + (size_t)(j + 3) * kSlot, lds, kPart1 / 1024, wave, lane);
    mma_second(part2, lane_off2, hs, acc);
    sp0 = p0, sp1 = p1, sh0 = h0, sh1 = h1;
    barrier_drain();
    if (j + 1 < kNF) dma_pieces<kWaves>(packed + (size_t)(j + 3) * kSlot + kPart1, part2, kPart2 / 1024, wave, lane);
  }
  store32<true>(io, P.pre, kFF, kHC * (kNF - 1), sp0, sp1);
  store32<true>(io, P.h, kFF, kHC * (kNF - 1), sh0, sh1);
  f32x4 v[4][2];
#pragma unroll
  for (int s = 0; s < 4; ++s) {
    const int n0 = 32 * s + 8 * g;
    f32x4 ya, yb;
    join8(yi[s], ya, yb);
    v[s][0] = acc[2 * s] + *(const f32x4*)(par + 3 * kC + n0) + ya;
    v[s][1] = acc[2 * s + 1] + *(const f32x4*)(par + 3 * kC + n0 + 4) + yb;
    if (P.s2 != nullptr) store32<true>(io, P.s2, kC, 32 * s, v[s][0], v[s][1]);
  }
  float mean, rstd;
  ln_stats(v, P.eps, mean, rstd);
  if (valid && g == 0) ((float2*)P.st2)[row] = make_float2(mean, rstd);
  const float* prow = P.pos_table != nullptr ? P.pos_table + (size_t)P.pos_idx[row] * kC : nullptr;
#pragma unroll
  for (int s = 0; s < 4; ++s) {
    const int n0 = 32 * s + 8 * g;
    const f32x4 y0 = v[s][0] * rstd * *(const f32x4*)(par + 4 * kC + n0) + *(const f32x4*)(par + 5 * kC + n0);
    const f32x4 y1 = v[s][1] * rstd * *(const f32x4*)(par + 4 * kC + n0 + 4) + *(const f32x4*)(par + 5 * kC + n0 + 4);
    store32<SST_NT_OUT>(io, P.y2, kC, 32 * s, y0, y1);
    if (prow != nullptr) store32<SST_NT_OUT>(io, P.y2p, kC, 32 * s, y0 + *(const f32x4*)(prow + n0), y1 + *(const f32x4*)(prow + n0 + 4));
  }
}

struct tail_bwd_params {
  const float *dy2, *dy2p, *s2, *st2, *n2w, *pre, *s1, *st1, *n1w;
  const unsigned char* packed;
  int64_t m;
  float *ds2, *dpre, *ds1, *d_o;
  float *part2, *part1;
};

__device__ __forceinline__ void ln_bwd(f32x4 (&d)[4][2], f32x4 (&sv)[4][2], const float2 st, const float* gamma, int g, int c,
                                       bool valid, float* red) {
  float sg = 0.f, sgx = 0.f;
#pragma unroll
  for (int s = 0; s < 4; ++s)
#pragma unroll
    for (int h = 0; h < 2; ++h) {
      const f32x4 w = *(const f32x4*)(gamma + 32 * s + 8 * g + 4 * h);
      sv[s][h] = (sv[s][h] - st.x) * st.y;
      f32x4 a, b;
#pragma unroll
      for (int r = 0; r < 4; ++r) {
        a[r] = row_sum16(valid ? d[s][h][r] * sv[s][h][r] : 0.f);
        b[r] = row_sum16(valid ? d[s][h][r] : 0.f);
      }
      if (c == 0) {
        *(f32x4*)(red + 32 * s + 8 * g + 4 * h) = a;
        *(f32x4*)(red + kC + 32 * s + 8 * g + 4 * h) = b;
      }
      d[s][h] *= w;
#pragma unroll
      for (int r = 0; r < 4; ++r) {
        sg += d[s][h][r];
        sgx = fmaf(d[s][h][r], sv[s][h][r], sgx);
      }
    }
  sg += __shfl_xor(sg, 16, 64);
  sg += __shfl_xor(sg, 32, 64);
  sgx += __shfl_xor(sgx, 16, 64);
  sgx += __shfl_xor(sgx, 32, 64);
  const float mg = sg * (1.f / 128.f), mgx = sgx * (1.f / 128.f);
#pragma unroll
  for (int s = 0; s < 4; ++s)
#pragma unroll
    for (int h = 0; h < 2; ++h)
#pragma unroll
      for (int r = 0; r < 4; ++r) d[s][h][r] = st.y * (d[s][h][r] - mg - sv[s][h][r] * mgx);
}

template <int ACT>
__global__ __launch_bounds__(kNTH, 2) void encoder_tail_bwd_x6_k(const tail_bwd_params P) {
  extern __shared__ __attribute__((aligned(16))) unsigned char lds[];
  float* par = (float*)(lds + kArea);
  float* red = par + 2 * kC;
  const int lane = threadIdx.x & 63, g = lane >> 4, c = lane & 15, wave = threadIdx.x >> 6;
  const int64_t r0 = (int64_t)blockIdx.x * kRowsPerWg + wave * 16;
  const bool valid = r0 + c < P.m;
  const int64_t row = valid ? r0 + c : P.m - 1;
  const tile_io io = make_tile_io(lds + kArea + 2 * kC * 4 + kWaves * 2 * kC * 4 + wave * kScr, lane, r0, P.m);
  const unsigned char* packed = P.packed;
  unsigned char* const part2 = lds + kPart1;
  dma_pieces<kWaves>(packed, lds, kSlot / 1024, wave, lane);
  f32x4 d[4][2], sv[4][2];
  {
    f32x4 wd[4][2], we[4][2];
#pragma unroll
    for (int s = 0; s < 4; ++s) load32_issue(io, P.dy2, kC, 32 * s, wd[s]);
    if (P.dy2p != nullptr) {
#pragma unroll
      for (int s = 0; s < 4; ++s) load32_issue(io, P.dy2p, kC, 32 * s, we[s]);
#pragma unroll
      for (int s = 0; s < 4; ++s) {
        wd[s][0] += we[s][0];
        wd[s][1] += we[s][1];
      }
    }
#pragma unroll
    for (int s = 0; s < 4; ++s) load32_issue(io, P.s2, kC, 32 * s, we[s]);
#pragma unroll
    for (int s = 0; s < 4; ++s) load32_finish(io, wd[s], d[s][0], d[s][1]);
#pragma unroll
    for (int s = 0; s < 4; ++s) load32_finish(io, we[s], sv[s][0], sv[s][1]);
  }
  const float2 st2 = ((const float2*)P.st2)[row];
  for (int i = threadIdx.x; i < kC; i += kNTH) {
    par[i] = P.n2w[i];
    par[kC + i] = P.n1w[i];
  }
  barrier_drain();

  img3 di[4];
  {
    ln_bwd(d, sv, st2, par, g, c, valid, red + wave * 2 * kC);
#pragma unroll
    for (int s = 0; s < 4; ++s) {
      store32<SST_NT_BWD>(io, P.ds2, kC, 32 * s, d[s][0], d[s][1]);
      di[s] = split8(d[s][0], d[s][1]);
    }
  }
  const int lane_offA = lane * 16, lane_off1 = lane * 16, lane_off2 = lane * 16;
  const f32x4 z4 = {0.f, 0.f, 0.f, 0.f};
  f32x4 acc[8];
#pragma unroll
  for (int T = 0; T < 8; ++T) acc[T] = z4;
  f32x4 xs1[4][2];
  f32x4 pq[2];
  load32_issue(io, P.pre, kFF, 0, pq);

  f32x4 sd0 = z4, sd1 = z4;
  auto ffn_chunk = [&](int j, const f32x4 q0, const f32x4 q1) __attribute__((always_inline)) {
    if (j > 0) store32<SST_NT_BWD>(io, P.dpre, kFF, kHC * (j - 1), sd0, sd1);
    f32x4 p0, p1;
    mma_first(lds, lane_off1, di, p0, p1);
#pragma unroll
    for (int r = 0; r < 4; ++r) {
      p0[r] *= ACT == 1 ? gelu_grad_f(q0[r]) : (q0[r] > 0.f ? 1.f : 0.f);
      p1[r] *= ACT == 1 ? gelu_grad_f(q1[r]) : (q1[r] > 0.f ? 1.f : 0.f);
    }
    const img3 hs = split8(p0, p1);
    barrier_drain();
    if (j + 1 < kNF) dma_pieces<kWaves>(packed + (size_t)(j + 1) * kSlot, lds, kPart1 / 1024, wave, lane);
    mma_second(part2, lane_off2, hs, acc);
    sd0 = p0, sd1 = p1;
    barrier_drain();
    if (j + 1 < kNF)
      dma_pieces<kWaves>(packed + (size_t)(j + 1) * kSlot + kPart1, part2, kPart2 / 1024, wave, lane);
    else
      dma_pieces<kWaves>(packed + (size_t)kNF * kSlot, lds, 3 * kIA / 1024, wave, lane);
  };
  barrier_drain();
  if (threadIdx.x < 2 * kC) {
    float a = 0.f;
#pragma unroll
    for (int w = 0; w < kWaves; ++w) a += red[w * 2 * kC + threadIdx.x];
    P.part2[(int64_t)blockIdx.x * 2 * kC + threadIdx.x] = a;
  }
#pragma unroll 1
  for (int j = 0; j < kNF - 1; ++j) {
    f32x4 q0, q1;
    load32_finish(io, pq, q0, q1);
    load32_issue(io, P.pre, kFF, kHC * (j + 1), pq);
    ffn_chunk(j, q0, q1);
  }
  {
    f32x4 q0, q1;
    load32_finish(io, pq, q0, q1);
    ffn_chunk(kNF - 1, q0, q1);
    store32<SST_NT_BWD>(io, P.dpre, kFF, kHC * (kNF - 1), sd0, sd1);
    {
      f32x4 ws[4][2];
#pragma unroll
      for (int s = 0; s < 4; ++s) load32_issue(io, P.s1, kC, 32 * s, ws[s]);
#pragma unroll
      for (int s = 0; s < 4; ++s) load32_finish(io, ws[s], xs1[s][0], xs1[s][1]);
    }
    f32x4 dd[4][2];
#pragma unroll
    for (int s = 0; s < 4; ++s) {
      f32x4 ya, yb;
      join8(di[s], ya, yb);
      dd[s][0] = acc[2 * s] + ya;
      dd[s][1] = acc[2 * s + 1] + yb;
    }
    const float2 st1 = ((const float2*)P.st1)[row];
    barrier_drain();
    ln_bwd(dd, xs1, st1, par + kC, g, c, valid, red + wave * 2 * kC);
#pragma unroll
    for (int s = 0; s < 4; ++s) {
      store32<SST_NT_BWD>(io, P.ds1, kC, 32 * s, dd[s][0], dd[s][1]);
      xs1[s][0] = dd[s][0];
      xs1[s][1] = dd[s][1];
    }
#pragma unroll
    for (int T = 0; T < 8; ++T) acc[T] = z4;
    barrier_drain();
    mma_half<0>(lds, lane_offA, xs1, acc);
    barrier_drain();
    dma_pieces<kWaves>(packed + (size_t)(kNF + 1) * kSlot, lds, 3 * kIA / 1024, wave, lane);
    barrier_drain();
    mma_half<1>(lds, lane_offA, xs1, acc);
  }
#pragma unroll
  for (int s = 0; s < 4; ++s) store32<SST_NT_OUT>(io, P.d_o, kC, 32 * s, acc[2 * s], acc[2 * s + 1]);
  barrier_drain();
  if (threadIdx.x < 2 * kC) {
    float b = 0.f;
#pragma unroll
    for (int w = 0; w < kWaves; ++w) b += red[w * 2 * kC + threadIdx.x];
    P.part1[(int64_t)blockIdx.x * 2 * kC + threadIdx.x] = b;
  }
}

bool aligned16(const void* p) { return ((uintptr_t)p & 15) == 0; }

template <typename K>
int configure(K kernel, int lds_bytes, unsigned long long* mask) {
  if (sst_first_use_on_device(mask)) {
    SST_HIP(hipFuncSetAttribute((const void*)kernel, hipFuncAttributeMaxDynamicSharedMemorySize, lds_bytes));
    sst_mark_device(mask);
  }
  return SST_OK;
}

}

int sst_internal_encoder_tail_bwd_f32x6(const sst_encoder_tail_bwd_args* a, float** part2, float** part1, int* partial_rows,
                                        void* stream) {
  if (!a || a->m <= 0 || (a->act != 1 && a->act != 2)) return SST_ERR_ARG;
  const void* need[] = {a->dy2, a->s2, a->st2, a->n2w, a->pre, a->s1, a->st1, a->n1w, a->packed,
                        a->ds2, a->dpre, a->ds1, a->d_o, a->workspace};
  for (const void* p : need)
    if (!p || !aligned16(p)) return SST_ERR_ARG;
  if (a->dy2p && !aligned16(a->dy2p)) return SST_ERR_ARG;
  const int64_t rows = sst_div_up(a->m, (int64_t)kRowsPerWg);
  if (rows > 0x7fffffff / 2) return SST_ERR_UNSUPPORTED;
  tail_bwd_params P;
  P.dy2 = a->dy2, P.dy2p = a->dy2p, P.s2 = a->s2, P.st2 = a->st2, P.n2w = a->n2w, P.pre = a->pre, P.s1 = a->s1, P.st1 = a->st1;
  P.n1w = a->n1w, P.packed = (const unsigned char*)a->packed + kPackDir, P.m = a->m;
  P.ds2 = a->ds2, P.dpre = a->dpre, P.ds1 = a->ds1, P.d_o = a->d_o;
  P.part2 = (float*)a->workspace;
  P.part1 = P.part2 + rows * 2 * kC;
  hipStream_t st = (hipStream_t)stream;
  static unsigned long long cfg1 = 0, cfg2 = 0;
  if (a->act == 1) {
    const int rc = configure(encoder_tail_bwd_x6_k<1>, kLdsBwd, &cfg1);
    if (rc) return rc;
    hipLaunchKernelGGL(encoder_tail_bwd_x6_k<1>, dim3((unsigned)rows), dim3(kNTH), kLdsBwd, st, P);
  } else {
    const int rc = configure(encoder_tail_bwd_x6_k<2>, kLdsBwd, &cfg2);
    if (rc) return rc;
    hipLaunchKernelGGL(encoder_tail_bwd_x6_k<2>, dim3((unsigned)rows), dim3(kNTH), kLdsBwd, st, P);
  }
  SST_LAUNCH_CHECK();
  *part2 = P.part2, *part1 = P.part1, *partial_rows = (int)rows;
  return SST_OK;
}

namespace {
__global__ __launch_bounds__(1024) void tail_colsum_k(const float* __restrict__ partials, int nb, int width, float* __restrict__ out0,
                                                      float* __restrict__ out1, int split) {
  __shared__ float red[32][33];
  const int cx = threadIdx.x & 31, gy = threadIdx.x >> 5;
  const int i = blockIdx.x * 32 + cx;
  float acc = 0.f;
  if (i < width)
    for (int b = gy; b < nb; b += 32) acc += partials[(int64_t)b * width + i];
  red[gy][cx] = acc;
  __syncthreads();
  if (gy == 0 && i < width) {
    float t = 0.f;
#pragma unroll
    for (int k = 0; k < 32; ++k) t += red[k][cx];
    if (i < split)
      out0[i] = t;
    else
      out1[i - split] = t;
  }
}
}

extern "C" {

int64_t sst_encoder_tail_pack_bytes(void) { return 2 * (int64_t)kPackDir; }

int sst_encoder_tail_pack_f32x6_many(const float* const* d_w_out, const float* const* d_w1, const float* const* d_w2,
                                     void* const* d_packed, int n, void* stream) {
  if (n < 0 || (n > 0 && (!d_w_out || !d_w1 || !d_w2 || !d_packed))) return SST_ERR_ARG;
  static unsigned long long cfg = 0;
  const int rc = configure(encoder_tail_pack_k, kSlot, &cfg);
  if (rc) return rc;
  for (int base = 0; base < n; base += kPackMany) {
    pack_batch B;
    const int cnt = n - base < kPackMany ? n - base : kPackMany;
    for (int i = 0; i < cnt; ++i) {
      const float *wo = d_w_out[base + i], *w1 = d_w1[base + i], *w2 = d_w2[base + i];
      void* dst = d_packed[base + i];
      if (!wo || !w1 || !w2 || !dst || !aligned16(wo) || !aligned16(w1) || !aligned16(w2) || !aligned16(dst)) return SST_ERR_ARG;
      B.w[i].wo = wo, B.w[i].w1 = w1, B.w[i].w2 = w2;
      B.dst[i] = (unsigned char*)dst;
    }
    hipLaunchKernelGGL(encoder_tail_pack_k, dim3(cnt * 2 * kNChunks), dim3(512), kSlot, (hipStream_t)stream, B);
  }
  SST_LAUNCH_CHECK();
  return SST_OK;
}

int sst_encoder_tail_pack_f32x6(const float* d_w_out, const float* d_w1, const float* d_w2, void* d_packed, void* stream) {
  return sst_encoder_tail_pack_f32x6_many(&d_w_out, &d_w1, &d_w2, &d_packed, 1, stream);
}

int64_t sst_encoder_tail_bwd_workspace_bytes(int64_t m) {
  if (m < 0) return SST_ERR_ARG;
  return sst_align_up(2 * sst_div_up(m > 0 ? m : 1, (int64_t)kRowsPerWg) * 2 * kC * (int64_t)sizeof(float), 256);
}

int sst_encoder_tail_fwd_f32x6(const sst_encoder_tail_fwd_args* a, void* stream) {
  if (!a || a->m < 0 || (a->act != 1 && a->act != 2)) return SST_ERR_ARG;
  if (a->m == 0) return SST_OK;
  const void* need[] = {a->o, a->x, a->packed, a->n1w, a->n1b, a->n2w, a->n2b, a->st1, a->y1, a->pre, a->h, a->st2, a->y2};
  for (const void* p : need)
    if (!p || !aligned16(p)) return SST_ERR_ARG;
  if ((a->s1 && !aligned16(a->s1)) || (a->s2 && !aligned16(a->s2))) return SST_ERR_ARG;
  if ((a->pos_table != nullptr) != (a->pos_idx != nullptr) || (a->pos_table != nullptr) != (a->y2p != nullptr)) return SST_ERR_ARG;
  if (a->pos_table && (!aligned16(a->pos_table) || !aligned16(a->y2p))) return SST_ERR_ARG;
  tail_fwd_params P;
  P.o = a->o, P.x = a->x, P.packed = (const unsigned char*)a->packed;
  P.b_out = a->b_out, P.b1 = a->b1, P.b2 = a->b2, P.n1w = a->n1w, P.n1b = a->n1b, P.n2w = a->n2w, P.n2b = a->n2b;
  P.eps = a->eps, P.m = a->m;
  P.s1 = a->s1, P.st1 = a->st1, P.y1 = a->y1, P.pre = a->pre, P.h = a->h, P.s2 = a->s2, P.st2 = a->st2, P.y2 = a->y2;
  P.pos_table = a->pos_table, P.pos_idx = a->pos_idx, P.y2p = a->y2p;
  const int64_t rows = sst_div_up(a->m, (int64_t)kRowsPerWg);
  if (rows > 0x7fffffff) return SST_ERR_UNSUPPORTED;
  hipStream_t st = (hipStream_t)stream;
  static unsigned long long cfg1 = 0, cfg2 = 0;
  if (a->act == 1) {
    const int rc = configure(encoder_tail_fwd_x6_k<1>, kLdsFwd, &cfg1);
    if (rc) return rc;
    hipLaunchKernelGGL(encoder_tail_fwd_x6_k<1>, dim3((unsigned)rows), dim3(kNTH), kLdsFwd, st, P);
  } else {
    const int rc = configure(encoder_tail_fwd_x6_k<2>, kLdsFwd, &cfg2);
    if (rc) return rc;
    hipLaunchKernelGGL(encoder_tail_fwd_x6_k<2>, dim3((unsigned)rows), dim3(kNTH), kLdsFwd, st, P);
  }
  SST_LAUNCH_CHECK();
  return SST_OK;
}

int sst_encoder_tail_bwd_f32x6(const sst_encoder_tail_bwd_args* a, void* stream) {
  if (!a || a->m < 0) return SST_ERR_ARG;
  if (!a->dn2w || !a->dn2b || !a->dn1w || !a->dn1b) return SST_ERR_ARG;
  hipStream_t st = (hipStream_t)stream;
  if (a->m == 0) {
    for (float* p : {a->dn2w, a->dn2b, a->dn1w, a->dn1b}) SST_HIP(hipMemsetAsync(p, 0, sizeof(float) * kC, st));
    return SST_OK;
  }
  float *part2 = nullptr, *part1 = nullptr;
  int rows = 0;
  const int rc = sst_internal_encoder_tail_bwd_f32x6(a, &part2, &part1, &rows, stream);
  if (rc) return rc;
  hipLaunchKernelGGL(tail_colsum_k, dim3(2 * kC / 32), dim3(1024), 0, st, part2, rows, 2 * kC, a->dn2w, a->dn2b, kC);
  hipLaunchKernelGGL(tail_colsum_k, dim3(2 * kC / 32), dim3(1024), 0, st, part1, rows, 2 * kC, a->dn1w, a->dn1b, kC);
  SST_LAUNCH_CHECK();
  return SST_OK;
}

}
```

### sst_amd/dense.py

```python
import torch
from torch.autograd import Function

from . import _lib


def colsum(x):
    m, c = x.shape
    if x.dtype != torch.float32 or (c % 4) != 0 or c > 1024 or x.stride(1) != 1 or not x.is_cuda:
        return x.sum(0)
    out = torch.empty(c, dtype=torch.float32, device=x.device)
    lib = _lib.load()
    ws = _lib.workspace(lib.sst_colsum_workspace_bytes(m, c), x.device)
    rc = lib.sst_colsum_f32(_lib.ptr(x), m, c, x.stride(0), _lib.ptr(out), _lib.ptr(ws), _lib.stream_ptr())
    _lib.check(rc, 'sst_colsum_f32')
    return out


def weight_grad_splitk(dy, x, chunk=1024):
    m = dy.size(0)
    s = m // chunk
    if s < 4:
        return dy.t() @ x
    body = s * chunk
    dw = torch.bmm(dy[:body].view(s, chunk, -1).transpose(1, 2), x[:body].view(s, chunk, -1)).sum(0)
# ... 219 lines not shown
    return pre, h


def dgrad_gelu(dy, w2, pre):
    m, k = dy.shape
    n = w2.size(1)
    if w2.size(0) != k or not _gelu_gemm_ok(dy, w2, n, k) or pre.shape != (m, n) or not pre.is_contiguous():
        return None
    out = torch.empty((m, n), dtype=torch.float32, device=dy.device)
    lib = _lib.load()
    for j in range(0, n, 128):
        rc = lib.sst_tall_linear_gelu_f32(_lib.ptr(dy), dy.stride(0), _lib.ptr(w2[:, j:]), w2.stride(0), None, m, 128,
                                          k, 1, 1, _lib.ptr(pre[:, j:]), _lib.ptr(out[:, j:]), n, _lib.stream_ptr())
        _lib.check(rc, 'sst_tall_linear_gelu_f32')
    return out


class TallLinear(Function):

    @staticmethod
    def forward(ctx, x, weight, bias):
        ctx.save_for_backward(x, weight)
        ctx.has_bias = bias is not None
        if bias is not None:
            return torch.addmm(bias, x, weight.t())
        return x @ weight.t()

    @staticmethod
    def backward(ctx, dy):
        x, weight = ctx.saved_tensors
        dy = dy.contiguous()
        dx = dw = db = None
        if ctx.needs_input_grad[0]:
            dx = dy @ weight
        want_b = ctx.has_bias and ctx.needs_input_grad[2]
        if ctx.needs_input_grad[1]:
            dw, db = weight_bias_grad(dy, x, want_b)
        elif want_b:
            db = colsum(dy)
        return dx, dw, db


def tall_linear(x, weight, bias=None):
    if x.dim() != 2 or x.dtype != torch.float32 or not x.is_cuda:
        return torch.nn.functional.linear(x, weight, bias)
    return TallLinear.apply(x, weight, bias)


_LN_ACTS = {None: 0, 'gelu': 1, 'relu': 2}


def add_ln_fwd(x, res, weight, bias, eps, save_sum=True, act=None, pos=None):
    x = x.contiguous()
    m, c = x.shape
    if res is not None:
        res = res.contiguous()
    y = torch.empty_like(x)
    s = (torch.empty_like(x) if save_sum else None) if res is not None else x
    stats = torch.empty((m, 2), dtype=torch.float32, device=x.device)
    if pos is not None:
        assert act is None
        yp = torch.empty_like(x)
        rc = _lib.load().sst_add_layernorm_pos_fwd_f32(_lib.ptr(x), _lib.ptr(res), _lib.ptr(weight), _lib.ptr(bias), m, c, float(eps),
                                                       _lib.ptr(y), _lib.ptr(s) if (res is not None and save_sum) else None,
                                                       _lib.ptr(stats), _lib.ptr(pos[0]), _lib.ptr(pos[1]), _lib.ptr(yp),
                                                       _lib.stream_ptr())
        _lib.check(rc, 'sst_add_layernorm_pos_fwd_f32')
        return y, s, stats, yp
    rc = _lib.load().sst_add_layernorm_act_fwd_f32(_lib.ptr(x), _lib.ptr(res), _lib.ptr(weight), _lib.ptr(bias), m, c,
                                                   float(eps), _LN_ACTS[act], _lib.ptr(y),
                                                   _lib.ptr(s) if (res is not None and save_sum) else None,
                                                   _lib.ptr(stats), _lib.stream_ptr())
    _lib.check(rc, 'sst_add_layernorm_act_fwd_f32')
    return y, s, stats


def add_ln_act_bwd(dy, s, stats, weight, bias, act):
    dy = dy.contiguous()
    m, c = s.shape
    dx = torch.empty_like(s)
    dw = torch.empty(c, dtype=torch.float32, device=s.device)
    db = torch.empty(c, dtype=torch.float32, device=s.device)
    lib = _lib.load()
    ws = _lib.workspace(lib.sst_add_layernorm_bwd_workspace_bytes(m, c), s.device)
    rc = lib.sst_add_layernorm_act_bwd_f32(_lib.ptr(dy), _lib.ptr(s), _lib.ptr(stats), _lib.ptr(weight), _lib.ptr(bias),
                                           _LN_ACTS[act], m, c, _lib.ptr(dx), _lib.ptr(dw), _lib.ptr(db), _lib.ptr(ws),
                                           _lib.stream_ptr())
    _lib.check(rc, 'sst_add_layernorm_act_bwd_f32')
    return dx, dw, db


def add_ln_bwd(dy, s, stats, weight, dy2=None):
    dy = dy.contiguous()
    m, c = s.shape
    dx = torch.empty_like(s)
    dw = torch.empty(c, dtype=torch.float32, device=s.device)
    db = torch.empty(c, dtype=torch.float32, device=s.device)
    lib = _lib.load()
    ws = _lib.workspace(lib.sst_add_layernorm_bwd_workspace_bytes(m, c), s.device)
    if dy2 is not None and c != 128:
        dy, dy2 = dy + dy2, None
    rc = lib.sst_add_layernorm_bwd2_f32(_lib.ptr(dy), _lib.ptr(dy2.contiguous() if dy2 is not None else None), _lib.ptr(s),
                                        _lib.ptr(stats), _lib.ptr(weight), m, c, _lib.ptr(dx), _lib.ptr(dw), _lib.ptr(db),
                                        _lib.ptr(ws), _lib.stream_ptr())
    _lib.check(rc, 'sst_add_layernorm_bwd2_f32')
    return dx, dw, db


def lds_linear_add_ln_ok(x, w, res, c):
    return (c == 128 and lds_linear_ok(x, w) and w.size(0) == 128 and res.is_cuda and res.dtype == torch.float32
            and res.shape == (x.size(0), 128) and res.is_contiguous() and res.data_ptr() % 16 == 0)


def lds_linear_add_ln(x, w, bias, res, ln_weight, ln_bias, eps, save_sum=True, pos=None):
    m, k = x.shape
    y = torch.empty((m, 128), dtype=torch.float32, device=x.device)
    s = torch.empty((m, 128), dtype=torch.float32, device=x.device) if save_sum else None
    stats = torch.empty((m, 2), dtype=torch.float32, device=x.device)
    yp = torch.empty((m, 128), dtype=torch.float32, device=x.device) if pos is not None else None
    lib = _lib.load()
    if _MATMUL_MODE == 'f32x6' and k != 128:
        s = lds_linear(x, w, bias, EPI_ADD, aux_in=res)
        out = add_ln_fwd(s, None, ln_weight, ln_bias, eps, pos=pos)
        return out[0], s, out[2], (out[3] if pos is not None else None)
    entry = getattr(lib, 'sst_tall_linear_ln_' + _MATMUL_MODE)
    rc = entry(
        _lib.ptr(x), x.stride(0), _lib.ptr(w), w.stride(0), _lib.ptr(bias), m, k, _lib.ptr(res), 128, _lib.ptr(ln_weight),
        _lib.ptr(ln_bias), float(eps), _lib.ptr(y), _lib.ptr(s), _lib.ptr(stats),
        _lib.ptr(pos[0]) if pos is not None else None, _lib.ptr(pos[1]) if pos is not None else None, _lib.ptr(yp),
        _lib.stream_ptr())
    _lib.check(rc, 'sst_tall_linear_ln_' + _MATMUL_MODE)
    return y, s, stats, yp


def encoder_tail_ok(o, x, w_out, w1, w2):
    if _MATMUL_MODE != 'f32x6':
        return False
    if not (o.shape == x.shape and x.dim() == 2 and x.size(1) == 128 and w_out.shape == (128, 128) and w1.shape == (256, 128)
            and w2.shape == (128, 256)):
        return False
    return all(t.is_cuda and t.dtype == torch.float32 and t.is_contiguous() and t.data_ptr() % 16 == 0
               for t in (o, x, w_out, w1, w2))


def encoder_tail_pack(w_out, w1, w2, out=None):
    lib = _lib.load()
    if out is None:
        out = torch.empty(int(lib.sst_encoder_tail_pack_bytes()), dtype=torch.uint8, device=w_out.device)
    _lib.check(lib.sst_encoder_tail_pack_f32x6(_lib.ptr(w_out), _lib.ptr(w1), _lib.ptr(w2), _lib.ptr(out), _lib.stream_ptr()),
               'sst_encoder_tail_pack_f32x6')
    return out


def encoder_tail_fwd(o, x, packed, b_out, b1, b2, n1w, n1b, n2w, n2b, eps, act, save=True, pos=None, out=None):
    m = x.size(0)
    dev = x.device
    out = dict(out) if out else {}

    def e(name, cols):
        if name not in out or out[name] is None:
            out[name] = torch.empty((m, cols), dtype=torch.float32, device=dev)
        return out[name]
    s1 = e('s1', 128) if save else None
    out['s1'] = s1
    st1, y1, pre, h, s2, st2, y2 = e('st1', 2), e('y1', 128), e('pre', 256), e('h', 256), e('s2', 128), e('st2', 2), e('y2', 128)
    y2p = e('y2p', 128) if pos is not None else None
    out['y2p'] = y2p
    P = lambda t: None if t is None else t.data_ptr()
    args = _lib.EncoderTailFwdArgs(
        m, 1 if act == 'gelu' else 2, 0, float(eps), 0.0, P(o), P(x), P(packed), P(b_out), P(b1), P(b2), P(n1w), P(n1b),
        P(n2w), P(n2b), P(pos[0]) if pos is not None else None, P(pos[1]) if pos is not None else None,
        P(s1), P(st1), P(y1), P(pre), P(h), P(s2), P(st2), P(y2), P(y2p))
    import ctypes
    _lib.check(_lib.load().sst_encoder_tail_fwd_f32x6(ctypes.byref(args), _lib.stream_ptr()), 'sst_encoder_tail_fwd_f32x6')
    return out


def encoder_tail_bwd(dy2, dy2p, s2, st2, pre, s1, st1, packed, n1w, n2w, act, out=None):
    m = dy2.size(0)
    dev = dy2.device
    out = out or {}

    def e(name, cols):
        return out[name] if name in out else torch.empty((m, cols), dtype=torch.float32, device=dev)
    ds2, dpre, ds1, d_o = e('ds2', 128), e('dpre', 256), e('ds1', 128), e('d_o', 128)
    dn = out['dn'] if 'dn' in out else torch.empty((4, 128), dtype=torch.float32, device=dev)
    lib = _lib.load()
    ws = out['ws'] if 'ws' in out else _lib.workspace(lib.sst_encoder_tail_bwd_workspace_bytes(m), dev)
    P = lambda t: None if t is None else t.data_ptr()
    d0 = dn.data_ptr()
    args = _lib.EncoderTailBwdArgs(m, 1 if act == 'gelu' else 2, 0, P(dy2), P(dy2p), P(s2), P(st2), P(pre), P(s1), P(st1), P(packed),
                                   P(n1w), P(n2w), P(ds2), P(dpre), P(ds1), P(d_o), d0, d0 + 512, d0 + 1024, d0 + 1536, P(ws))
    import ctypes
    _lib.check(lib.sst_encoder_tail_bwd_f32x6(ctypes.byref(args), _lib.stream_ptr()), 'sst_encoder_tail_bwd_f32x6')
    return ds2, dpre, ds1, d_o, dn


class AddLayerNorm(Function):

    @staticmethod
    def forward(ctx, x, res, weight, bias, eps, act=None):
        y, s, stats = add_ln_fwd(x, res, weight, bias, eps, act=act)
        ctx.save_for_backward(s, stats, weight, bias)
        ctx.has_res, ctx.act = res is not None, act
        return y

    @staticmethod
    def backward(ctx, dy):
        s, stats, weight, bias = ctx.saved_tensors
        if ctx.act is None:
            dx, dw, db = add_ln_bwd(dy, s, stats, weight)
        else:
            dx, dw, db = add_ln_act_bwd(dy, s, stats, weight, bias, ctx.act)
        return dx, (dx if ctx.has_res else None), dw, db, None, None


def _act_name(act):
    if act is None or isinstance(act, torch.nn.Identity):
        return None
    if isinstance(act, torch.nn.GELU) and getattr(act, 'approximate', 'none') == 'none':
        return 'gelu'
    if type(act) is torch.nn.ReLU:
        return 'relu'
    return False


def add_layer_norm(x, res, norm, act=None):
    c = x.size(-1)
    post = (lambda t: t) if act is None else act
    if not isinstance(norm, torch.nn.LayerNorm):
        return post(norm(x + res if res is not None else x))
    ok = (x.dim() == 2 and x.dtype == torch.float32 and x.is_cuda
          and norm.elementwise_affine and norm.bias is not None and 1 <= c <= 512 and len(norm.normalized_shape) == 1)
    if not ok:
        y = x + res if res is not None else x
        return post(torch.nn.functional.layer_norm(y, norm.normalized_shape, norm.weight, norm.bias, norm.eps))
    name = _act_name(act)
    if name is False:
        return act(AddLayerNorm.apply(x, res, norm.weight, norm.bias, norm.eps))
    return AddLayerNorm.apply(x, res, norm.weight, norm.bias, norm.eps, name)
```

### sst_amd/sst_basic_block.py

```python
import math

import torch
import torch.nn as nn
import torch.nn.functional as F
from torch.utils.checkpoint import checkpoint

from . import _lib
from . import kernels as K
from .sra_composed import sra_attention_composed
from .dense import (encoder_tail_ok, encoder_tail_pack, encoder_tail_fwd, encoder_tail_bwd, inproj_pos_ok, inproj_pos,
                    EPI_ADD, EPI_BIAS, EPI_GELU, EPI_MUL_GELU_GRAD, EPI_MUL_RELU_GRAD, EPI_RELU, lds_linear, lds_linear_ok,
                    lds_linear_add_ln, lds_linear_add_ln_ok, lds_linear_dqkv_ok, lds_linear_qkv, lds_linear_qkv_ok,
                    weight_bias_grad_group,
                    tall_gemm, add_layer_norm, add_ln_bwd, add_ln_fwd, dgrad_gelu, linear_gelu, tall_linear,
                    weight_bias_grad)
from .norm import build_norm_layer


class CosineMultiheadAttention(nn.MultiheadAttention):

    def __init__(self, embed_dim, num_heads, dropout=0.0, batch_first=False, tau_min=0.01, cosine=True,
                 non_shared_tau=False):
        super().__init__(embed_dim, num_heads, dropout=dropout)
        self.tau_min = tau_min
        self.cosine = cosine
        if cosine:
            if non_shared_tau:
                self.tau = nn.Parameter(torch.ones(1, num_heads, 1, 1))
            else:
                self.tau = nn.Parameter(torch.ones(1, 1, 1))


def plan_from_reference_dicts(ind_dict, num_voxels, device):
    info = ind_dict['batching_info']
    wkeys, inner, toks = [], [], []
    wbase, tmax = 0, 1
    for dl in info:
        if dl not in ind_dict:
            continue
        f2w, (flat_pos,) = ind_dict[dl][0].long(), ind_dict[dl][1]
        if f2w.numel() == 0:
            continue
        t = int(info[dl]['max_tokens'])
        tmax = max(tmax, t)
        w = torch.div(f2w, t, rounding_mode='floor')
        wkeys.append(w + wbase)
        inner.append(f2w - w * t)
        toks.append(flat_pos.long())
        wbase += int(w.max().item()) + 1
    wkeys, inner, toks = torch.cat(wkeys), torch.cat(inner), torch.cat(toks)
    order = torch.argsort(wkeys * tmax + inner)
    _, counts = torch.unique_consecutive(wkeys[order], return_counts=True)
    winoff = torch.zeros(counts.numel() + 1, dtype=torch.int32, device=device)
    winoff[1:] = torch.cumsum(counts, 0).to(torch.int32)
    return K.WindowPlan(toks[order].to(torch.int32).contiguous(), winoff, counts.numel(), num_voxels, tmax)


def flat_pos_from_reference_dict(pos_dict, ind_dict, num_voxels):
    from .sst_ops import window2flat_v2
    if pos_dict is None or any(v is None for v in pos_dict.values()):
        return None
    return window2flat_v2(pos_dict, ind_dict)


class WindowAttention(nn.Module):

    def __init__(self, d_model, nhead, dropout, batch_first=False, layer_id=None, layer_cfg=dict()):
        super().__init__()
        self.nhead = nhead
        self.d_model = d_model
        if d_model % nhead != 0:
            raise ValueError('embed_dim must be divisible by num_heads')
        self.head_dim = d_model // nhead
        self.cosine = layer_cfg.get('cosine', False)
        if self.cosine:
            tau_min = layer_cfg.get('tau_min', 0.01)
            self.self_attn = CosineMultiheadAttention(
                d_model, nhead, dropout=dropout, batch_first=False, tau_min=tau_min, cosine=True,
                non_shared_tau=layer_cfg.get('non_shared_tau', False))
        elif layer_cfg.get('linear', False):
            raise NotImplementedError
        else:
            self.self_attn = nn.MultiheadAttention(d_model, nhead, dropout=dropout)
        self.attn_dropout = dropout
        self.exe_counter = 0
        self.layer_id = layer_id
        self.impl = 0

    def head_scale(self):
        if not self.cosine:
            return None
        attn = self.self_attn
        return (1.0 / attn.tau.float().clamp(min=attn.tau_min)).reshape(-1).expand(self.nhead).contiguous()

    def forward(self, feat_2d, pos_dict, ind_dict, key_padding_dict=None):
        composed = self.head_dim != 16 or (self.attn_dropout > 0 and self.training)
        if isinstance(ind_dict, K.WindowPlan):
            plan, pos = ind_dict, pos_dict
        else:
            plan = plan_from_reference_dicts(ind_dict, feat_2d.size(0), feat_2d.device)
            pos = flat_pos_from_reference_dict(pos_dict, ind_dict, feat_2d.size(0)) if isinstance(pos_dict, dict) \
                else pos_dict
        attn = self.self_attn
        c = self.d_model
        x = feat_2d.float()
        w, b = attn.in_proj_weight, attn.in_proj_bias
        xp = x + pos if pos is not None else x
        qk = tall_linear(xp, w[:2 * c], b[:2 * c])
        v = tall_linear(x, w[2 * c:], b[2 * c:])
        if self.cosine and not composed and K.cosine_kernels_ok(plan, self.nhead, self.impl) and qk.is_cuda:
            o = K.sra_cosine_attention_qk_v(qk, v, self.head_scale(), plan, self.nhead)
        elif self.cosine:
            h = self.nhead
            q = F.normalize(qk[:, :c].reshape(-1, h, self.head_dim), dim=2)
            k = F.normalize(qk[:, c:].reshape(-1, h, self.head_dim), dim=2)
            tau = attn.tau.clamp(min=attn.tau_min).reshape(1, -1, 1)
            q = (q / tau).reshape(-1, c)
            if composed:
                o = sra_attention_composed(q, k.reshape(-1, c), v, plan, h, 1.0, self.attn_dropout, self.training)
            else:
                o = K.sra_attention(q, k.reshape(-1, c), v, plan, h, scale=1.0, impl=self.impl)
        elif composed:
            o = sra_attention_composed(qk[:, :c], qk[:, c:], v, plan, self.nhead, 1.0 / math.sqrt(self.head_dim),
                                       self.attn_dropout, self.training)
        else:
            o = K.sra_attention_qk_v(qk, v, plan, self.nhead, scale=1.0 / math.sqrt(16.0), impl=self.impl)
        return tall_linear(o, attn.out_proj.weight, attn.out_proj.bias)


import os as _os
_TALL_GEMM = int(_os.environ.get('SST_AMD_TALL_GEMM', '1'))
_FUSED_GELU = int(_os.environ.get('SST_AMD_FUSED_GELU', '0'))
_LDS_LINEAR = int(_os.environ.get('SST_AMD_LDS_LINEAR', '1'))


def _linear_fwd(x, w, b):
    if _LDS_LINEAR and lds_linear_ok(x, w):
        return lds_linear(x, w, b)
    if _TALL_GEMM and w.size(0) == 128 and (w.size(1) == 128 or _TALL_GEMM > 1):
        y = tall_gemm(x, w, b)
        if y is not None:
            return y
    return torch.addmm(b, x, w.t())


def _linear_dgrad(dy, w, out=None, add=None):
    if _LDS_LINEAR and lds_linear_ok(dy, w, trans_w=True):
        if out is not None:
            return lds_linear(dy, w, None, EPI_ADD, trans_w=True, aux_in=out if add is None else add, out=out)
        return lds_linear(dy, w, None, trans_w=True)
    if out is not None and add is not None:
        out.copy_(add)
    if _TALL_GEMM and w.size(1) == 128 and (w.size(0) == 128 or _TALL_GEMM > 1):
        y = tall_gemm(dy, w, None, trans_w=True, out=out, accumulate=out is not None)
        if y is not None:
            return y
    if out is not None:
        return out.addmm_(dy, w)
    return dy @ w


_LAYER_EXEC = int(_os.environ.get('SST_AMD_LAYER_EXEC', '1'))
_POS_FOLD = int(_os.environ.get('SST_AMD_POS_FOLD', '1'))


def _layer_exec_ok(x, xp, plan, nhead, act, params):
    from . import dense
    if not (_LAYER_EXEC and _LDS_LINEAR and dense.matmul_mode() == 'f32x6' and act in ('gelu', 'relu') and nhead == 8):
        return False
    w_in, b_in, w_out, b_out, w1, b1, w2, b2, n1w, n1b, n2w, n2b = params
    if any(p is None for p in params):
        return False
    m = x.size(0)
    shapes_ok = (x.shape == (m, 128) and (xp is None or xp.shape == (m, 128)) and w_in.shape == (384, 128) and w_out.shape == (128, 128)
                 and w1.shape == (256, 128) and w2.shape == (128, 256) and plan.n_tokens == m
                 and m >= 4096)
    if not shapes_ok:
        return False
    for t in (x,) + ((xp,) if xp is not None else ()) + tuple(params):
        if not (t.is_cuda and t.dtype == torch.float32 and t.is_contiguous() and t.data_ptr() % 16 == 0):
            return False
    from . import _lib
    return int(_lib.load().sst_encoder_layer_bwd_workspace_bytes(m, nhead)) >= 0


_SLAB = (('qkv', 384), ('o', 128), ('lse', 8), ('s1', 128), ('st1', 2), ('y1', 128), ('pre', 256), ('h', 256), ('s2', 128),
         ('st2', 2))


def _slab_offsets(m):
    off, out = 0, {}
    for name, cols in _SLAB:
        out[name] = off
        off += (m * cols * 4 + 255) // 256 * 256
    return out, off


def _layer_exec_fwd(x, xp, plan, nhead, impl, act, params, eps, scale, pos_next, need_bwd, head_scale=None, pos_spec=None,
                    wpack=None):
    from . import _lib
    import ctypes
    w_in, b_in, w_out, b_out, w1, b1, w2, b2, n1w, n1b, n2w, n2b = params
    m = x.size(0)
    dev = x.device
    offs, total = _slab_offsets(m)
    slab = torch.empty(total, dtype=torch.uint8, device=dev)
    base = slab.data_ptr()
    y2 = torch.empty((m, 128), dtype=torch.float32, device=dev)
    y2p = torch.empty((m, 128), dtype=torch.float32, device=dev) if pos_next is not None else None
    lib = _lib.load()
    packed = wpack is not None
    if not packed:
        wpack = torch.empty(int(lib.sst_encoder_layer_wpack_bytes()), dtype=torch.uint8, device=dev)
    order = plan.order
    P = lambda t: None if t is None else t.data_ptr()
    S = lambda name: base + offs[name]
    args = _lib.EncoderLayerFwdArgs(
        m, plan.n_windows, nhead, 1 if act == 'gelu' else 2, plan.max_tokens, impl, float(eps), float(scale),
        P(x), P(xp), P(w_in), P(b_in), None if packed else P(w_out), P(b_out), None if packed else P(w1), P(b1),
        None if packed else P(w2), P(b2), P(n1w), P(n1b), P(n2w), P(n2b),
        None if plan.tok_ptr(impl) is None else plan.tok.data_ptr(), P(plan.winoff), P(order),
        P(pos_next[0]) if pos_next is not None else None, P(pos_next[1]) if pos_next is not None else None,
        S('qkv'), S('o'), S('lse'), S('y1'), S('s1') if need_bwd else None, S('st1'), S('pre'), S('h'), S('s2'), P(y2), S('st2'),
        P(y2p), P(head_scale), P(wpack), P(pos_spec[0]) if pos_spec is not None else None,
        P(pos_spec[1]) if pos_spec is not None else None)
    rc = K._bracket('sra_fwd', plan.n_tokens, lambda: lib.sst_encoder_layer_fwd_f32x6(ctypes.byref(args), _lib.stream_ptr()))
    if rc == _lib.SST_ERR_UNSUPPORTED:
        return None
    _lib.check(rc, 'sst_encoder_layer_fwd_f32x6')
    return slab, y2, y2p, wpack


def _layer_exec_bwd(ctx, dy2, dy2p, saved):
    from . import _lib
    import ctypes
    x, xp, slab, w_in, w_out, w1, w2, n1w, n2w, wpack = saved[:10]
    rest = list(saved[10:])
    pos_spec = (rest.pop(0), rest.pop(0)) if ctx.pos_fold else None
    if ctx.pos_fold:
        xp = None
    head_scale = rest.pop(0) if rest else None
    m = x.size(0)
    dev = x.device
    plan, nhead, impl = ctx.plan, ctx.nhead, ctx.impl
    offs, _ = _slab_offsets(m)
    base = slab.data_ptr()

    def e(*shape):
        return torch.empty(shape, dtype=torch.float32, device=dev)
    dy2 = dy2.contiguous()
    dy2p = dy2p.contiguous() if dy2p is not None else None
    ds1 = e(m, 128)
    scratch = e(m, 128 + 256 + 128 + 384)
    sb = scratch.data_ptr()
    p_ds2, p_dpre, p_do, p_dqkv = sb, sb + 4 * m * 128, sb + 4 * m * 384, sb + 4 * m * 512
    dw_in, db_in, dwo, dbo = e(384, 128), e(384), e(128, 128), e(128)
    dw1, db1, dw2, db2 = e(256, 128), e(256), e(128, 256), e(128)
    dn = e(4, 128)
    cos_r = e(m, nhead) if head_scale is not None else None
    lib = _lib.load()
    nbytes = lib.sst_encoder_layer_bwd_workspace_bytes(m, nhead)
    if nbytes < 0:
        _lib.check(int(nbytes), 'sst_encoder_layer_bwd_workspace_bytes')
    ws = _lib.workspace(nbytes, dev)
    order = plan.order
    P = lambda t: None if t is None else t.data_ptr()
    S = lambda name: base + offs[name]
    dnp = dn.data_ptr()
    args = _lib.EncoderLayerBwdArgs(
        m, plan.n_windows, nhead, 1 if ctx.act == 'gelu' else 2, plan.max_tokens, impl, 0.0, float(ctx.scale),
        P(dy2), P(dy2p), P(x), P(xp), S('qkv'), S('o'), S('lse'), S('s1'), S('st1'), S('y1'), S('pre'), S('h'), S('s2'), S('st2'),
        P(w_in), P(w_out), P(w1), P(w2), P(n1w), P(n2w),
        None if plan.tok_ptr(impl) is None else plan.tok.data_ptr(), P(plan.winoff), P(order),
        p_ds2, p_dpre, P(ds1), p_do, p_dqkv,
        P(dw_in), P(db_in), P(dwo), P(dbo), P(dw1), P(db1), P(dw2), P(db2), dnp, dnp + 512, dnp + 1024, dnp + 1536, P(ws),
        P(head_scale), P(cos_r), None, P(wpack), P(pos_spec[0]) if pos_spec is not None else None,
        P(pos_spec[1]) if pos_spec is not None else None)
    rc = K._bracket('sra_bwd', plan.n_tokens, lambda: lib.sst_encoder_layer_bwd_f32x6(ctypes.byref(args), _lib.stream_ptr()))
    _lib.check(rc, 'sst_encoder_layer_bwd_f32x6')
    d_scale = K.head_scale_grad(cos_r, head_scale) if head_scale is not None else None
    return (ds1, None, None, None, None, None, dw_in, db_in, dwo, dbo, dw1, db1, dw2, db2, dn[0], dn[1], dn[2], dn[3], None, None,
            None, d_scale, None, None, None, None)


def _bn_rows_fwd(bn, s):
    from .norm import bn_prepare
    prep, batch_stats, count, sync = bn_prepare(bn, s)
    m, c = s.shape
    y = torch.empty((m, c), dtype=torch.float32, device=s.device)
    _lib.check(_lib.load().sst_bn_act_res_fwd_f32(_lib.ptr(s), m, c, s.stride(0), None, 0, _lib.ptr(prep[2]), _lib.ptr(prep[3]), 0,
                                                  _lib.ptr(y), y.stride(0), _lib.stream_ptr()), 'sst_bn_act_res_fwd_f32')
    return y, prep, (bool(batch_stats), float(count), bool(sync))


def _bn_rows_bwd(dy, s, prep, cfg):
    from torch import distributed as dist
    batch_stats, count, sync = cfg
    m, c = s.shape
    dy = dy.contiguous()
    lib = _lib.load()
    sums = torch.empty((2, c), dtype=torch.float32, device=s.device)
    ws = _lib.workspace(lib.sst_bn_workspace_bytes(m, c), s.device)
    _lib.check(lib.sst_bn_act_res_bwd_reduce_f32(_lib.ptr(dy), _lib.ptr(s), None, m, c, dy.stride(0), s.stride(0), 0, _lib.ptr(prep[0]),
                                                 _lib.ptr(prep[1]), _lib.ptr(prep[2]), _lib.ptr(prep[3]), 0, _lib.ptr(sums[0]),
                                                 _lib.ptr(sums[1]), _lib.ptr(ws), _lib.stream_ptr()), 'sst_bn_act_res_bwd_reduce_f32')
    total = sums
    if sync and batch_stats:
        total = sums.clone()
        dist.all_reduce(total, async_op=False)
    ds = torch.empty((m, c), dtype=torch.float32, device=s.device)
    _lib.check(lib.sst_bn_act_res_bwd_apply_f32(_lib.ptr(dy), _lib.ptr(s), None, m, c, dy.stride(0), s.stride(0), 0, _lib.ptr(prep[0]),
                                                _lib.ptr(prep[1]), _lib.ptr(prep[2]), _lib.ptr(prep[3]), _lib.ptr(total[0]),
                                                _lib.ptr(total[1]), (1.0 / count) if batch_stats else 0.0, 0, None, 0, _lib.ptr(ds),
                                                ds.stride(0), _lib.stream_ptr()), 'sst_bn_act_res_bwd_apply_f32')
    return ds, sums[1], sums[0]


def _bn_layer_ok(norm, c):
    return (isinstance(norm, nn.BatchNorm1d) and norm.weight is not None and norm.bias is not None and norm.num_features == c
            and c % 4 == 0 and c <= 1024)


class FusedEncoderLayerFn(torch.autograd.Function):

    @staticmethod
    def forward(ctx, x, pos, plan, nhead, impl, act, w_in, b_in, w_out, b_out, w1, b1, w2, b2, n1w, n1b, n2w, n2b, eps,
                xp=None, pos_next=None, head_scale=None, xp_shares_x=False, pos_spec=None, bn=None, wpack=None):
        c = x.size(1)
        x = x.contiguous()
        if head_scale is not None:
            head_scale = head_scale.contiguous()
        ctx.cosine = head_scale is not None
        from . import dense as _dense
        ctx.matmul = _dense.matmul_mode()
        ctx.set_materialize_grads(False)
        ctx.pos_fold = False
        if pos_spec is not None:
            assert xp is None and pos is None, 'pos_spec replaces pos / xp'
            if _LDS_LINEAR and inproj_pos_ok(x, pos_spec, w_in):
                ctx.pos_fold = True
            else:
                xp = K.add_table_rows(x, pos_spec[0], pos_spec[1])
                xp_shares_x = True
        ctx.split_input = xp is not None
        ctx.fold_xp = (xp is None) or bool(xp_shares_x)
        if xp is None and not ctx.pos_fold:
            xp = x + pos if pos is not None else x
        params = (w_in, b_in, w_out, b_out, w1, b1, w2, b2, n1w, n1b, n2w, n2b)
        ctx.exec = False
        ctx.bn = bn is not None
        if bn is None and c == 128 and ctx.fold_xp and _layer_exec_ok(x, xp, plan, nhead, act, params):
            need_bwd = any(ctx.needs_input_grad)
            scale = 1.0 / math.sqrt(16.0)
            done = _layer_exec_fwd(x, xp, plan, nhead, impl, act, params, eps, scale, pos_next, need_bwd, head_scale,
                                   pos_spec if ctx.pos_fold else None, wpack)
            if done is not None:
                slab, y2, y2p, wpack = done
                if need_bwd:
                    ctx.save_for_backward(x, xp if xp is not None else x, slab, w_in, w_out, w1, w2, n1w, n2w, wpack,
                                          *(pos_spec if ctx.pos_fold else ()), *((head_scale,) if ctx.cosine else ()))
                    ctx.plan, ctx.nhead, ctx.impl, ctx.act, ctx.scale = plan, nhead, impl, act, scale
                    ctx.exec = True
                ctx.two = pos_next is not None
                return (y2, y2p) if ctx.two else y2
        if ctx.pos_fold:
            qkv = inproj_pos(x, pos_spec, w_in, b_in)
            qk, v = qkv[:, :2 * c], qkv[:, 2 * c:]
            xp = x
        elif _LDS_LINEAR and c == 128 and lds_linear_qkv_ok(xp, x, w_in):
            qkv = lds_linear_qkv(xp, x, w_in, b_in)
            qk, v = qkv[:, :2 * c], qkv[:, 2 * c:]
        else:
            qk = _linear_fwd(xp, w_in[:2 * c], b_in[:2 * c])
            v = _linear_fwd(x, w_in[2 * c:], b_in[2 * c:])
        scale = 1.0 / math.sqrt(16.0)
        if ctx.cosine:
            res = K._sra_cos_fwd(qk[:, :c], qk[:, c:], v, plan, nhead, head_scale)
            if res is None:
                raise RuntimeError('sst_amd: cosine attention kernels refused a layout _can_fuse admitted')
            o, lse = res
        else:
            o, lse = K._sra_fwd(qk[:, :c], qk[:, c:], v, plan, nhead, scale, impl)
        need_bwd = any(ctx.needs_input_grad)
        ctx.tail = False
        if bn is not None:
            y1, s1, st1, pre, h, s2, st2, y2, y2p, ctx.bn_cfg = FusedEncoderLayerFn._tail_batch_norm(
                o, x, w_out, b_out, w1, b1, w2, b2, bn, act, pos_next)
        elif (_LDS_LINEAR and c == 128 and act in ('gelu', 'relu') and o.is_contiguous()
                and encoder_tail_ok(o, x, w_out, w1, w2) and all(t is not None for t in (b_out, b1, b2))):
            if wpack is None:
                wpack = encoder_tail_pack(w_out, w1, w2)
            t = encoder_tail_fwd(o, x, wpack, b_out, b1, b2, n1w, n1b, n2w, n2b, eps, act, save=need_bwd, pos=pos_next)
            s1, st1, y1, pre, h, s2, st2, y2, y2p = (t[k] for k in ('s1', 'st1', 'y1', 'pre', 'h', 's2', 'st2', 'y2', 'y2p'))
            ctx.tail = True
        else:
            y1, s1, st1, pre, h, s2, st2, y2, y2p = FusedEncoderLayerFn._tail_by_products(
                o, x, w_out, b_out, w1, b1, w2, b2, n1w, n1b, n2w, n2b, eps, act, need_bwd, pos_next, c)
        if need_bwd:
            ctx.save_for_backward(x, xp, qk, v, o, lse, s1, st1, y1, pre, h, s2, st2, w_in, w_out, w1, w2, n1w, n2w,
                                  *((wpack,) if ctx.tail else ()), *(pos_spec if ctx.pos_fold else ()),
                                  *((head_scale,) if ctx.cosine else ()))
            ctx.plan, ctx.nhead, ctx.impl, ctx.act, ctx.scale = plan, nhead, impl, act, scale
        ctx.two = pos_next is not None
        return (y2, y2p) if ctx.two else y2

    @staticmethod
    def _tail_batch_norm(o, x, w_out, b_out, w1, b1, w2, b2, bn, act, pos_next):
        if _LDS_LINEAR and lds_linear_ok(o, w_out) and x.is_contiguous():
            s1 = lds_linear(o, w_out, b_out, EPI_ADD, aux_in=x)
        else:
            s1 = torch.addmm(b_out, o, w_out.t()).add_(x)
        y1, prep1, cfg1 = _bn_rows_fwd(bn[0], s1)
        if _LDS_LINEAR and lds_linear_ok(y1, w1) and act in ('gelu', 'relu'):
            h, pre = lds_linear(y1, w1, b1, EPI_GELU if act == 'gelu' else EPI_RELU, want_pre=True)
        else:
            pre = torch.addmm(b1, y1, w1.t())
            h = F.gelu(pre) if act == 'gelu' else F.relu(pre)
        if _LDS_LINEAR and lds_linear_ok(h, w2):
            s2 = lds_linear(h, w2, b2, EPI_ADD, aux_in=y1)
        else:
            s2 = torch.addmm(b2, h, w2.t()).add_(y1)
        y2, prep2, cfg2 = _bn_rows_fwd(bn[1], s2)
        y2p = y2 + pos_next[0].index_select(0, pos_next[1].long()) if pos_next is not None else None
        return y1, s1, prep1, pre, h, s2, prep2, y2, y2p, (cfg1, cfg2)

    @staticmethod
    def _tail_by_products(o, x, w_out, b_out, w1, b1, w2, b2, n1w, n1b, n2w, n2b, eps, act, need_bwd, pos_next, c):
        fuse_ln = _LDS_LINEAR and lds_linear_add_ln_ok(o, w_out, x, c)
        if fuse_ln:
            y1, s1, st1, _ = lds_linear_add_ln(o, w_out, b_out, x, n1w, n1b, eps, save_sum=need_bwd)
        else:
            a = _linear_fwd(o, w_out, b_out)
            y1, s1, st1 = add_ln_fwd(x, a, n1w, n1b, eps, save_sum=need_bwd)
        fused_act = linear_gelu(y1, w1, b1) if (act == 'gelu' and _FUSED_GELU) else None
        if _LDS_LINEAR and lds_linear_ok(y1, w1):
            h, pre = lds_linear(y1, w1, b1, EPI_GELU if act == 'gelu' else EPI_RELU, want_pre=True)
        elif fused_act is not None:
            pre, h = fused_act
        else:
            pre = torch.addmm(b1, y1, w1.t())
            h = F.gelu(pre) if act == 'gelu' else F.relu(pre)
        y2p = None
        if fuse_ln and lds_linear_add_ln_ok(h, w2, y1, c):
            y2, s2, st2, y2p = lds_linear_add_ln(h, w2, b2, y1, n2w, n2b, eps, save_sum=need_bwd, pos=pos_next)
        elif _LDS_LINEAR and lds_linear_ok(h, w2):
            s2 = lds_linear(h, w2, b2, EPI_ADD, aux_in=y1)
            y2, _, st2 = add_ln_fwd(s2, None, n2w, n2b, eps)
        else:
            f = _linear_fwd(h, w2, b2)
            y2, s2, st2 = add_ln_fwd(y1, f, n2w, n2b, eps, save_sum=need_bwd)
        if pos_next is not None and y2p is None:
            y2p = y2 + pos_next[0].index_select(0, pos_next[1].long())
        return y1, s1, st1, pre, h, s2, st2, y2, y2p

    @staticmethod
    def backward(ctx, dy2, dy2p=None):
        from . import dense as _dense
        with _dense.matmul_mode_scope(ctx.matmul):
            return FusedEncoderLayerFn._backward(ctx, dy2, dy2p)

    @staticmethod
    def _backward(ctx, dy2, dy2p=None):
        if ctx.exec:
            if dy2 is None:
                dy2, dy2p = dy2p, None
            return _layer_exec_bwd(ctx, dy2, dy2p if ctx.two else None, ctx.saved_tensors)
        saved = ctx.saved_tensors
        x, xp, qk, v, o, lse, s1, st1, y1, pre, h, s2, st2, w_in, w_out, w1, w2, n1w, n2w = saved[:19]
        rest = list(saved[19:])
        wpack = rest.pop(0) if ctx.tail else None
        pos_spec = (rest.pop(0), rest.pop(0)) if ctx.pos_fold else None
        head_scale = rest.pop(0) if ctx.cosine else None
        c = x.size(1)
        if dy2 is None:
            dy2, dy2p = dy2p, None
        f32 = dict(dtype=torch.float32, device=x.device)
        dw2, db2 = torch.empty_like(w2), torch.empty(w2.size(0), **f32)
        dw1, db1 = torch.empty_like(w1), torch.empty(w1.size(0), **f32)
        if ctx.tail:
            ds2, dpre, ds1, do, dn = encoder_tail_bwd(dy2.contiguous(), dy2p.contiguous() if (ctx.two and dy2p is not None) else None,
                                                      s2, st2, pre, s1, st1, wpack, n1w, n2w, ctx.act)
            ds2_for_w2 = ds2
            dn2w, dn2b, dn1w, dn1b = dn[0], dn[1], dn[2], dn[3]
        else:
            if ctx.bn:
                if ctx.two and dy2p is not None:
                    dy2 = dy2 + dy2p
                ds2, dn2w, dn2b = _bn_rows_bwd(dy2, s2, st2, ctx.bn_cfg[1])
            else:
                ds2, dn2w, dn2b = add_ln_bwd(dy2, s2, st2, n2w, dy2=dy2p if ctx.two else None)
            ds2_for_w2 = ds2
            dpre = dgrad_gelu(ds2, w2, pre) if (ctx.act == 'gelu' and _FUSED_GELU) else None
            if _LDS_LINEAR and lds_linear_ok(ds2, w2, trans_w=True) and pre.is_contiguous():
                dpre = lds_linear(ds2, w2, None, EPI_MUL_GELU_GRAD if ctx.act == 'gelu' else EPI_MUL_RELU_GRAD, trans_w=True,
                                  aux_in=pre)
            if dpre is None:
                dh = ds2 @ w2
                if ctx.act == 'gelu':
                    dpre = torch.ops.aten.gelu_backward(dh, pre)
                else:
                    dpre = dh * (pre > 0).to(dh.dtype)
            dy1 = _linear_dgrad(dpre, w1, out=torch.empty_like(ds2), add=ds2)
            if ctx.bn:
                ds1, dn1w, dn1b = _bn_rows_bwd(dy1, s1, st1, ctx.bn_cfg[0])
            else:
                ds1, dn1w, dn1b = add_ln_bwd(dy1, s1, st1, n1w)
            do = _linear_dgrad(ds1, w_out)
        dqkv = torch.empty((x.size(0), 3 * c), dtype=torch.float32, device=x.device)
        dqk, dv = dqkv[:, :2 * c], dqkv[:, 2 * c:]
        d_scale = None
        if ctx.cosine:
            r = K._sra_cos_bwd(qk[:, :c], qk[:, c:], v, o, lse, do, ctx.plan, ctx.nhead, head_scale, dqkv[:, :c],
                               dqkv[:, c:2 * c], dv)
            d_scale = K.head_scale_grad(r, head_scale)
        else:
            K._sra_bwd(qk[:, :c], qk[:, c:], v, o, lse, do, ctx.plan, ctx.nhead, ctx.scale, ctx.impl, dqkv[:, :c],
                       dqkv[:, c:2 * c], dv)
        dw_in = torch.empty_like(w_in)
        db_in = torch.empty(3 * c, **f32)
        dwo, dbo = torch.empty_like(w_out), torch.empty(w_out.size(0), **f32)
        weight_bias_grad_group([(ds2_for_w2, h, dw2, db2), (dpre, y1, dw1, db1), (ds1, o, dwo, dbo),
                                (dqk, x, dw_in[:2 * c], db_in[:2 * c], pos_spec) if ctx.pos_fold else
                                (dqk, xp, dw_in[:2 * c], db_in[:2 * c]), (dv, x, dw_in[2 * c:], db_in[2 * c:])])
        dxp = None
        if ctx.fold_xp and _LDS_LINEAR and c == 128 and lds_linear_dqkv_ok(dqkv, w_in):
            dx = lds_linear(dqkv, w_in, None, EPI_ADD, trans_w=True, aux_in=ds1, out=ds1)
        elif ctx.split_input:
            dxp = _linear_dgrad(dqk, w_in[:2 * c])
            dx = _linear_dgrad(dv, w_in[2 * c:], out=ds1)
        elif _LDS_LINEAR and lds_linear_ok(dqk, w_in[:2 * c], trans_w=True) and lds_linear_ok(dv, w_in[2 * c:], trans_w=True):
            dx = _linear_dgrad(dv, w_in[2 * c:], out=_linear_dgrad(dqk, w_in[:2 * c], out=ds1))
        else:
            dx = ds1.addmm_(dqkv, w_in)
        return (dx, None, None, None, None, None, dw_in, db_in, dwo, dbo, dw1, db1, dw2, db2, dn1w, dn1b, dn2w, dn2b,
                None, dxp, None, d_scale, None, None, None, None)


class _StackHeadScales(torch.autograd.Function):

    @staticmethod
    def forward(ctx, nhead, tau_mins, *taus):
        flat = torch.cat([t.reshape(-1).expand(nhead) if t.numel() == 1 else t.reshape(-1) for t in taus]).view(len(taus), nhead)
        mins = K.const_tensor(tau_mins, flat.device).view(-1, 1)
        scales = 1.0 / torch.maximum(flat.float(), mins)
        ctx.save_for_backward(flat, scales, mins)
        ctx.shapes = [tuple(t.shape) for t in taus]
        return scales

    @staticmethod
    def backward(ctx, g):
        flat, scales, mins = ctx.saved_tensors
        d = torch.where(flat >= mins, -(g * scales * scales), torch.zeros((), dtype=g.dtype, device=g.device))
        per_layer_sum = None
        out = []
        for l, shape in enumerate(ctx.shapes):
            n = 1
            for v in shape:
                n *= v
            if n == 1:
                if per_layer_sum is None:
                    per_layer_sum = d.sum(1)
                out.append(per_layer_sum[l].reshape(shape))
            else:
                out.append(d[l].reshape(shape))
        return (None, None) + tuple(out)


def stack_head_scales(layers):
    cos = [(i, enc.win_attn) for i, enc in enumerate(layers) if enc.win_attn.cosine]
    out = [None] * len(layers)
    if not cos:
        return out
    heads = {wa.nhead for _, wa in cos}
    if len(heads) != 1:
        for i, wa in cos:
            out[i] = wa.head_scale()
        return out
    nhead = heads.pop()
    rows = _StackHeadScales.apply(nhead, tuple(float(wa.self_attn.tau_min) for _, wa in cos),
                                  *[wa.self_attn.tau for _, wa in cos]).unbind(0)
    for (i, _), row in zip(cos, rows):
        out[i] = row
    return out


def stack_tail_images(layers, like):
    import ctypes
    out = [None] * len(layers)
    take = []
    for i, enc in enumerate(layers):
        attn = enc.win_attn.self_attn
        wo, w1, w2 = attn.out_proj.weight, enc.linear1.weight, enc.linear2.weight
        if (enc.bn_modules() is None and wo.is_cuda and wo.shape == (128, 128) and w1.shape == (256, 128) and w2.shape == (128, 256)
                and all(w.dtype == torch.float32 and w.is_contiguous() and w.data_ptr() % 16 == 0 for w in (wo, w1, w2))
                and enc.act_name in ('gelu', 'relu') and all(b is not None for b in (attn.out_proj.bias, enc.linear1.bias,
                                                                                     enc.linear2.bias))):
            take.append((i, wo, w1, w2))
    if not take or not like.is_cuda:
        return out
    lib = _lib.load()
    nbytes = (int(lib.sst_encoder_tail_pack_bytes()) + 255) // 256 * 256
    buf = torch.empty(len(take) * nbytes, dtype=torch.uint8, device=like.device)
    n = len(take)
    P = ctypes.c_void_p * n
    d = [buf[j * nbytes:(j + 1) * nbytes] for j in range(n)]
    with torch.no_grad():
        _lib.check(lib.sst_encoder_tail_pack_f32x6_many(P(*[t[1].data_ptr() for t in take]), P(*[t[2].data_ptr() for t in take]),
                                                        P(*[t[3].data_ptr() for t in take]), P(*[v.data_ptr() for v in d]), n,
                                                        _lib.stream_ptr()), 'sst_encoder_tail_pack_f32x6_many')
    for (i, _, _, _), v in zip(take, d):
        out[i] = v
    return out


def run_encoder_stack_fp32(blocks, feats, plans, pos_specs, checkpoint_blocks=()):
    n_layers = 2 * len(blocks)

    scales = stack_head_scales([enc for block in blocks for enc in block.encoder_list])

    from . import dense as _dense
    mode = _dense.matmul_mode()
    fold = _POS_FOLD and mode == 'f32x6' and _LDS_LINEAR and all(inproj_pos_ok(feats.contiguous(), spec, blocks[0].encoder_list[0].win_attn.
                                                                 self_attn.in_proj_weight) for spec in pos_specs[:2])

    layers = [enc for block in blocks for enc in block.encoder_list]
    wpacks = stack_tail_images(layers, feats) if (mode == 'f32x6' and _LDS_LINEAR) else [None] * n_layers

    def layer(enc, li, x, xp):
        attn = enc.win_attn.self_attn
        if fold:
            out = FusedEncoderLayerFn.apply(
                x, None, plans[li % 2], enc.win_attn.nhead, enc.win_attn.impl, enc.act_name, attn.in_proj_weight,
                attn.in_proj_bias, attn.out_proj.weight, attn.out_proj.bias, enc.linear1.weight, enc.linear1.bias,
                enc.linear2.weight, enc.linear2.bias, enc.norm1.weight, enc.norm1.bias, enc.norm2.weight, enc.norm2.bias,
                enc.norm1.eps, None, None, scales[li], False, pos_specs[li % 2], enc.bn_modules(), wpacks[li])
            return out, None
        pos_next = pos_specs[(li + 1) % 2] if li + 1 < n_layers else None
        out = FusedEncoderLayerFn.apply(
            x, None, plans[li % 2], enc.win_attn.nhead, enc.win_attn.impl, enc.act_name, attn.in_proj_weight,
            attn.in_proj_bias, attn.out_proj.weight, attn.out_proj.bias, enc.linear1.weight, enc.linear1.bias,
            enc.linear2.weight, enc.linear2.bias, enc.norm1.weight, enc.norm1.bias, enc.norm2.weight, enc.norm2.bias,
            enc.norm1.eps, xp, pos_next, scales[li], True, None, enc.bn_modules(), wpacks[li])
        return out if pos_next is not None else (out, None)

    def block_fn(bi):
        def run(x, xp):
            with _dense.matmul_mode_scope(mode):
                for j, enc in enumerate(blocks[bi].encoder_list):
                    x, xp = layer(enc, 2 * bi + j, x, xp)
            return (x, xp) if xp is not None else (x,)
        return run

    x = feats.contiguous()
    xp = None if fold else K.add_table_rows(x, pos_specs[0][0], pos_specs[0][1])
    for bi in range(len(blocks)):
        if bi in checkpoint_blocks and torch.is_grad_enabled():
            out = checkpoint(block_fn(bi), x, xp, use_reentrant=False)
        else:
            out = block_fn(bi)(x, xp)
        x, xp = (out[0], out[1]) if len(out) > 1 else (out[0], None)
    return x


class EncoderLayer(nn.Module):

    def __init__(self, d_model, nhead, dim_feedforward=2048, dropout=0.1, activation="relu", batch_first=False,
                 layer_id=None, mlp_dropout=0, layer_cfg=dict()):
        super().__init__()
        assert not batch_first
        self.batch_first = batch_first
        self.win_attn = WindowAttention(d_model, nhead, dropout, layer_id=layer_id, layer_cfg=layer_cfg)
        self.linear1 = nn.Linear(d_model, dim_feedforward)
        self.dropout = nn.Dropout(mlp_dropout)
        self.linear2 = nn.Linear(dim_feedforward, d_model)
        use_bn = layer_cfg.get('use_bn', False)
        if use_bn:
            self.norm1 = build_norm_layer(dict(type='naiveSyncBN1d', momentum=layer_cfg.get('mom', 0.1)), d_model)[1]
            self.norm2 = build_norm_layer(dict(type='naiveSyncBN1d', momentum=layer_cfg.get('mom', 0.1)), d_model)[1]
        else:
            self.norm1 = nn.LayerNorm(d_model)
            self.norm2 = nn.LayerNorm(d_model)
        self.dropout1 = nn.Dropout(mlp_dropout)
        self.dropout2 = nn.Dropout(mlp_dropout)
        self.activation = _get_activation_fn(activation)
        self.act_name = activation
        self.fused = True
        self.post_norm = layer_cfg.get('post_norm', True)
        self.fp16_enabled = False

    def bn_modules(self):
        return (self.norm1, self.norm2) if isinstance(self.norm1, nn.BatchNorm1d) else None

    def _ffn(self, x):
        h = self.activation(tall_linear(x, self.linear1.weight, self.linear1.bias))
        return tall_linear(self.dropout(h), self.linear2.weight, self.linear2.bias)

    def _can_fuse(self, src, pos_dict, ind_dict):
        wa = self.win_attn
        return (self.fused and self.post_norm and isinstance(ind_dict, K.WindowPlan)
                and ind_dict.n_tokens == src.size(0)
                and (pos_dict is None or torch.is_tensor(pos_dict)) and wa.head_dim == 16
                and (not wa.cosine or K.cosine_kernels_ok(ind_dict, wa.nhead, wa.impl))
                and ((isinstance(self.norm1, nn.LayerNorm) and isinstance(self.norm2, nn.LayerNorm))
                     or (_bn_layer_ok(self.norm1, src.size(1)) and _bn_layer_ok(self.norm2, src.size(1))))
                and self.act_name in ('gelu', 'relu') and src.dtype == torch.float32 and src.is_cuda
                and src.size(1) % 32 == 0 and self.linear1.out_features % 32 == 0
                and not (self.training and (wa.attn_dropout > 0 or self.dropout.p > 0 or self.dropout1.p > 0)))

    def forward(self, src, pos_dict, ind_dict, key_padding_mask_dict=None):
        if self._can_fuse(src, pos_dict, ind_dict):
            attn = self.win_attn.self_attn
            return FusedEncoderLayerFn.apply(
                src, pos_dict, ind_dict, self.win_attn.nhead, self.win_attn.impl, self.act_name, attn.in_proj_weight,
                attn.in_proj_bias, attn.out_proj.weight, attn.out_proj.bias, self.linear1.weight, self.linear1.bias,
                self.linear2.weight, self.linear2.bias, self.norm1.weight, self.norm1.bias, self.norm2.weight,
                self.norm2.bias, self.norm1.eps, None, None, self.win_attn.head_scale(), False, None, self.bn_modules())
        if self.post_norm:
            src2 = self.win_attn(src, pos_dict, ind_dict, key_padding_mask_dict)
            src = add_layer_norm(src, self.dropout1(src2), self.norm1)
            src2 = self._ffn(src)
            src = add_layer_norm(src, self.dropout2(src2), self.norm2)
        else:
            src2 = add_layer_norm(src, None, self.norm1)
            src2 = self.win_attn(src2, pos_dict, ind_dict, key_padding_mask_dict)
            src = src + self.dropout1(src2)
            src2 = add_layer_norm(src, None, self.norm2)
            src2 = self._ffn(src2)
            src = src + self.dropout2(src2)
        return src


class BasicShiftBlockV2(nn.Module):

    def __init__(self, d_model, nhead, dim_feedforward=2048, dropout=0.1, activation="relu", batch_first=False,
                 block_id=-100, layer_cfg=dict()):
        super().__init__()
        encoder_1 = EncoderLayer(d_model, nhead, dim_feedforward, dropout, activation, batch_first,
                                 layer_id=block_id * 2 + 0, layer_cfg=layer_cfg)
        encoder_2 = EncoderLayer(d_model, nhead, dim_feedforward, dropout, activation, batch_first,
                                 layer_id=block_id * 2 + 1, layer_cfg=layer_cfg)
        self.encoder_list = nn.ModuleList([encoder_1, encoder_2])

    def forward(self, src, pos_dict_list, ind_dict_list, key_mask_dict_list=None, using_checkpoint=False):
        num_shifts = len(pos_dict_list)
        assert num_shifts in (1, 2)
        output = src
        for i in range(2):
            this_id = i % num_shifts
            pos_dict = pos_dict_list[this_id]
            ind_dict = ind_dict_list[this_id]
            key_mask_dict = key_mask_dict_list[this_id] if key_mask_dict_list is not None else None
            layer = self.encoder_list[i]
            if using_checkpoint and self.training:
                output = checkpoint(layer, output, pos_dict, ind_dict, key_mask_dict, use_reentrant=False)
            else:
                output = layer(output, pos_dict, ind_dict, key_mask_dict)
        return output


def _get_activation_fn(activation):
    if activation == "relu":
        return F.relu
    if activation == "gelu":
        return F.gelu
    if activation == "glu":
        return F.glu
    raise RuntimeError(F"activation should be relu/gelu, not {activation}.")
```

Baseline: 101.8.

## Fuse next layer's in-projection into the encoder tail forward kernel

The fused encoder tail kernel can now compute the next layer's QKV in-projection, with the positional embedding added to the q/k inputs, straight from the LayerNorm2 output still held in registers. It streams a separately packed bf16x3 image of the next layer's w_in through the LDS slot parts that the FFN weights used before. The next layer then skips its own in-projection launch and the re-read of y2. In exchange the kernel needs more LDS, a static_assert keeps two workgroups per CU, and it does extra MFMA work at the tail. Python plumbing passes the precomputed qkv between layers, except across checkpointed blocks.

```diff
diff --git a/include/sst_amd.h b/include/sst_amd.h
--- a/include/sst_amd.h
+++ b/include/sst_amd.h
@@ -338,6 +338,12 @@
   void* wpack;
   const float* xpos_table;
   const int32_t* xpos_idx;
+  const void* next_in_packed;
+  const float* next_b_in;
+  const float* next_pos_table;
+  const int32_t* next_pos_idx;
+  float* qkv_next;
+  int64_t qkv_formed;
 } sst_encoder_layer_fwd_args;
 typedef struct sst_encoder_layer_bwd_args {
   int64_t m, n_windows;
@@ -372,6 +378,11 @@
   const float* pos_table;
   const int32_t* pos_idx;
   float *s1, *st1, *y1, *pre, *h, *s2, *st2, *y2, *y2p;
+  const void* in_packed;
+  const float* in_bias;
+  const float* in_pos_table;
+  const int32_t* in_pos_idx;
+  float* qkv_next;
 } sst_encoder_tail_fwd_args;
 typedef struct sst_encoder_tail_bwd_args {
   int64_t m;
@@ -387,6 +398,9 @@
 int sst_encoder_tail_pack_f32x6(const float* d_w_out, const float* d_w1, const float* d_w2, void* d_packed, void* stream);
 int sst_encoder_tail_pack_f32x6_many(const float* const* d_w_out, const float* const* d_w1, const float* const* d_w2,
                                      void* const* d_packed, int n, void* stream);
+int64_t sst_encoder_tail_inproj_pack_bytes(void);
+int sst_encoder_tail_inproj_pack_f32x6(const float* d_w_in, void* d_packed, void* stream);
+int sst_encoder_tail_inproj_pack_f32x6_many(const float* const* d_w_in, void* const* d_packed, int n, void* stream);
 int64_t sst_encoder_tail_bwd_workspace_bytes(int64_t m);
 int sst_encoder_tail_fwd_f32x6(const sst_encoder_tail_fwd_args* args, void* stream);
 int sst_encoder_tail_bwd_f32x6(const sst_encoder_tail_bwd_args* args, void* stream);
diff --git a/sst_amd/_lib.py b/sst_amd/_lib.py
--- a/sst_amd/_lib.py
+++ b/sst_amd/_lib.py
@@ -157,7 +157,8 @@
     + [(k, _P) for k in ('x', 'xp', 'w_in', 'b_in', 'w_out', 'b_out', 'w1', 'b1', 'w2', 'b2', 'n1w', 'n1b', 'n2w', 'n2b',
                          'tok', 'winoff', 'order', 'pos_table', 'pos_idx',
                          'qkv', 'o', 'lse', 'y1', 's1', 'st1', 'pre', 'h', 's2', 'y2', 'st2', 'y2p', 'head_scale', 'wpack',
-                         'xpos_table', 'xpos_idx')]))
+                         'xpos_table', 'xpos_idx', 'next_in_packed', 'next_b_in', 'next_pos_table', 'next_pos_idx',
+                         'qkv_next')] + [('qkv_formed', c_i64)]))
 EncoderLayerBwdArgs = _struct('EncoderLayerBwdArgs', 'sst_encoder_layer_bwd_args of include/sst_amd.h', (
     [('m', c_i64), ('n_windows', c_i64)] + [(k, ctypes.c_int32) for k in ('n_heads', 'act', 'max_tokens', 'impl')]
     + [('eps', ctypes.c_float), ('scale', ctypes.c_float)]
@@ -171,7 +172,8 @@
 EncoderTailFwdArgs = _struct('EncoderTailFwdArgs', 'sst_encoder_tail_fwd_args of include/sst_amd.h', (
     [('m', c_i64), ('act', ctypes.c_int32), ('reserved', ctypes.c_int32), ('eps', ctypes.c_float), ('reserved_f', ctypes.c_float)]
     + [(k, _P) for k in ('o', 'x', 'packed', 'b_out', 'b1', 'b2', 'n1w', 'n1b', 'n2w', 'n2b', 'pos_table', 'pos_idx',
-                         's1', 'st1', 'y1', 'pre', 'h', 's2', 'st2', 'y2', 'y2p')]))
+                         's1', 'st1', 'y1', 'pre', 'h', 's2', 'st2', 'y2', 'y2p',
+                         'in_packed', 'in_bias', 'in_pos_table', 'in_pos_idx', 'qkv_next')]))
 EncoderTailBwdArgs = _struct('EncoderTailBwdArgs', 'sst_encoder_tail_bwd_args of include/sst_amd.h', (
     [('m', c_i64), ('act', ctypes.c_int32), ('reserved', ctypes.c_int32)]
     + [(k, _P) for k in ('dy2', 'dy2p', 's2', 'st2', 'pre', 's1', 'st1', 'packed', 'n1w', 'n2w',
@@ -226,6 +228,9 @@
     'sst_encoder_tail_pack_bytes': (c_i64, []),
     'sst_encoder_tail_pack_f32x6': (c_i32, [c_ptr, c_ptr, c_ptr, c_ptr, c_ptr]),
     'sst_encoder_tail_pack_f32x6_many': (c_i32, [c_ptr, c_ptr, c_ptr, c_ptr, c_i32, c_ptr]),
+    'sst_encoder_tail_inproj_pack_bytes': (c_i64, []),
+    'sst_encoder_tail_inproj_pack_f32x6': (c_i32, [c_ptr, c_ptr, c_ptr]),
+    'sst_encoder_tail_inproj_pack_f32x6_many': (c_i32, [c_ptr, c_ptr, c_i32, c_ptr]),
     'sst_encoder_tail_bwd_workspace_bytes': (c_i64, [c_i64]),
     'sst_encoder_tail_fwd_f32x6': (c_i32, [c_ptr, c_ptr]),
     'sst_encoder_tail_bwd_f32x6': (c_i32, [c_ptr, c_ptr]),
diff --git a/sst_amd/csrc/layer_exec.hip b/sst_amd/csrc/layer_exec.hip
--- a/sst_amd/csrc/layer_exec.hip
+++ b/sst_amd/csrc/layer_exec.hip
@@ -56,9 +56,19 @@
   if (!a->x || !a->qkv || !a->o || !a->lse || !a->y1 || !a->st1 || !a->pre || !a->h || !a->s2 || !a->y2 || !a->st2)
     return SST_ERR_ARG;
   if (!a->xp && (!a->xpos_table || !a->xpos_idx)) return SST_ERR_ARG;
-  const int64_t m = a->m;
-  int rc;
-  if (a->xp == nullptr)
+  const bool next = a->next_in_packed != nullptr;
+  if (next != (a->next_pos_table != nullptr) || next != (a->next_pos_idx != nullptr) || next != (a->qkv_next != nullptr) ||
+      (!next && a->next_b_in != nullptr))
+    return SST_ERR_ARG;
+  for (const void* p : {(const void*)a->qkv, a->next_in_packed, (const void*)a->next_b_in, (const void*)a->next_pos_table,
+                        (const void*)a->qkv_next})
+    if ((uintptr_t)p & 15) return SST_ERR_ARG;
+  if (next && a->qkv_next == a->qkv) return SST_ERR_ARG;
+  const int64_t m = a->m;
+  int rc;
+  if (a->qkv_formed)
+    rc = SST_OK;
+  else if (a->xp == nullptr)
     rc = sst_inproj_pos_f32x6(a->x, kC, a->xpos_table, a->xpos_idx, a->w_in, kC, a->b_in, m, a->qkv, 3 * kC, stream);
   else
     rc = sst_tall_linear_epi2_f32x6(a->xp, a->x, 2 * kC, kC, a->w_in, kC, 0, a->b_in, m, kC, 3 * kC, kEpiBias, nullptr, nullptr, 0,
@@ -83,6 +93,8 @@
   t.pos_table = a->pos_table, t.pos_idx = a->pos_idx;
   t.s1 = a->s1, t.st1 = a->st1, t.y1 = a->y1, t.pre = a->pre, t.h = a->h, t.s2 = a->s2, t.st2 = a->st2, t.y2 = a->y2;
   t.y2p = a->pos_table != nullptr ? a->y2p : nullptr;
+  t.in_packed = a->next_in_packed, t.in_bias = a->next_b_in, t.in_pos_table = a->next_pos_table, t.in_pos_idx = a->next_pos_idx;
+  t.qkv_next = a->qkv_next;
   return sst_encoder_tail_fwd_f32x6(&t, stream);
 }
 
diff --git a/sst_amd/csrc/layer_tail_x6.hip b/sst_amd/csrc/layer_tail_x6.hip
--- a/sst_amd/csrc/layer_tail_x6.hip
+++ b/sst_amd/csrc/layer_tail_x6.hip
@@ -48,7 +48,13 @@
 constexpr int kParF = 6 * kC + kFF;
 constexpr int kArea = kSlot;
 constexpr int kScr = 2048;
-constexpr int kLdsFwd = kArea + kParF * 4 + kWaves * kScr;
+constexpr int kCI = 3 * kC, kNIn = kCI / 64;
+constexpr int kIP = 4 * 2 * kFrag;
+constexpr int kPiece = 3 * kIP;
+static_assert(kPiece == kPart1 && kPiece == kPart2, "an in-projection piece fills one slot part");
+constexpr int kPackIn = 2 * kNIn * kPiece;
+constexpr int kLdsFwd = kArea + (kParF + kCI) * 4 + kWaves * kScr;
+static_assert(2 * kLdsFwd <= 160 * 1024, "two workgroups per CU");
 constexpr int kLdsBwd = kArea + 2 * kC * 4 + kWaves * 2 * kC * 4 + kWaves * kScr;
 
 struct tail_weights {
@@ -159,6 +165,25 @@
   for (int i = threadIdx.x; i < kSlot / 16; i += 512) *(u32x4*)(dst + 16 * i) = *(const u32x4*)(lds + 16 * i);
 }
 
+__device__ __forceinline__ int inproj_chunk(int oc) { return oc < 2 ? oc + 4 : oc - 2; }
+struct pack_in_batch {
+  const float* w[kPackMany];
+  unsigned char* dst[kPackMany];
+};
+__global__ __launch_bounds__(512) void encoder_tail_pack_inproj_k(const pack_in_batch B) {
+  extern __shared__ __attribute__((aligned(16))) unsigned char lds[];
+  const int layer = blockIdx.x / (2 * kNIn), piece = blockIdx.x % (2 * kNIn);
+  const int cc = inproj_chunk(piece >> 1), kh = piece & 1;
+  const int n = threadIdx.x >> 3, k8 = (threadIdx.x & 7) * 8;
+  const float* p = B.w[layer] + (size_t)(64 * cc + n) * kC + 64 * kh + k8;
+  const f32x4 a = *(const f32x4*)p, b = *(const f32x4*)(p + 4);
+  const float r[8] = {a[0], a[1], a[2], a[3], b[0], b[1], b[2], b[3]};
+  store_images(lds, kIP, frag_off(w_lds_row(n), k8, 2), r);
+  __syncthreads();
+  unsigned char* dst = B.dst[layer] + (size_t)piece * kPiece;
+  for (int i = threadIdx.x; i < kPiece / 16; i += 512) *(u32x4*)(dst + 16 * i) = *(const u32x4*)(lds + 16 * i);
+}
+
 __device__ __forceinline__ void barrier_lds_only() { asm volatile("s_waitcnt lgkmcnt(0)\n\ts_barrier" ::: "memory"); }
 
 struct tile_io {
@@ -302,6 +327,34 @@
   }
 }
 
+template <int HALF>
+__device__ __forceinline__ void mma_inproj(const unsigned char* part, int lane_off, const img3 (&y)[4], f32x4 (&acc)[4]) {
+#pragma unroll
+  for (int s2 = 0; s2 < 2; ++s2) {
+    const img3& xs = y[2 * HALF + s2];
+    u32x4 a0[4], a1[4], a2[4];
+#pragma unroll
+    for (int u = 0; u < 4; ++u) {
+      const int off = lane_off + (u * 2 + s2) * kFrag;
+      a0[u] = *(const u32x4*)(part + off);
+      a1[u] = *(const u32x4*)(part + kIP + off);
+      a2[u] = *(const u32x4*)(part + 2 * kIP + off);
+    }
+#pragma unroll
+    for (int u = 0; u < 4; ++u) acc[u] = mma32(a0[u], xs.p2, acc[u]);
+#pragma unroll
+    for (int u = 0; u < 4; ++u) acc[u] = mma32(a2[u], xs.p0, acc[u]);
+#pragma unroll
+    for (int u = 0; u < 4; ++u) acc[u] = mma32(a1[u], xs.p1, acc[u]);
+#pragma unroll
+    for (int u = 0; u < 4; ++u) acc[u] = mma32(a0[u], xs.p1, acc[u]);
+#pragma unroll
+    for (int u = 0; u < 4; ++u) acc[u] = mma32(a1[u], xs.p0, acc[u]);
+#pragma unroll
+    for (int u = 0; u < 4; ++u) acc[u] = mma32(a0[u], xs.p0, acc[u]);
+  }
+}
+
 __device__ __forceinline__ void ln_stats(f32x4 (&v)[4][2], float eps, float& mean, float& rstd) {
   float sum = 0.f;
 #pragma unroll
@@ -336,6 +389,11 @@
   const float* pos_table;
   const int32_t* pos_idx;
   float* y2p;
+  const unsigned char* in_packed;
+  const float* in_bias;
+  const float* in_pos_table;
+  const int32_t* in_pos_idx;
+  float* qkv;
 };
 
 template <int ACT>
@@ -346,8 +404,9 @@
   const int64_t r0 = (int64_t)blockIdx.x * kRowsPerWg + wave * 16;
   const bool valid = r0 + c < P.m;
   const int64_t row = valid ? r0 + c : P.m - 1;
-  const tile_io io = make_tile_io(lds + kArea + kParF * 4 + wave * kScr, lane, r0, P.m);
+  const tile_io io = make_tile_io(lds + kArea + (kParF + kCI) * 4 + wave * kScr, lane, r0, P.m);
   const unsigned char* packed = P.packed;
+  const bool inproj = P.in_packed != nullptr;
   unsigned char* const part2 = lds + kPart1;
   dma_pieces<kWaves>(packed, lds, 3 * kIA / 1024, wave, lane);
   f32x4 ob[4][2], xr[4][2];
@@ -371,6 +430,8 @@
     par[5 * kC + i] = P.n2b[i];
   }
   for (int i = threadIdx.x; i < kFF; i += kNTH) par[6 * kC + i] = P.b1 ? P.b1[i] : 0.f;
+  if (inproj)
+    for (int i = threadIdx.x; i < kCI; i += kNTH) par[kParF + i] = P.in_bias ? P.in_bias[i] : 0.f;
 
   const int lane_offA = lane * 16, lane_off1 = lane * 16, lane_off2 = lane * 16;
   const f32x4 z4 = {0.f, 0.f, 0.f, 0.f};
@@ -431,11 +492,17 @@
     }
     const img3 hs = split8(h0, h1);
     barrier_drain();
-    if (j + 1 < kNF) dma_pieces<kWaves>(packed + (size_t)(j + 3) * kSlot, lds, kPart1 / 1024, wave, lane);
+    if (j + 1 < kNF)
+      dma_pieces<kWaves>(packed + (size_t)(j + 3) * kSlot, lds, kPart1 / 1024, wave, lane);
+    else if (inproj)
+      dma_pieces<kWaves>(P.in_packed, lds, kPiece / 1024, wave, lane);
     mma_second(part2, lane_off2, hs, acc);
     sp0 = p0, sp1 = p1, sh0 = h0, sh1 = h1;
     barrier_drain();
-    if (j + 1 < kNF) dma_pieces<kWaves>(packed + (size_t)(j + 3) * kSlot + kPart1, part2, kPart2 / 1024, wave, lane);
+    if (j + 1 < kNF)
+      dma_pieces<kWaves>(packed + (size_t)(j + 3) * kSlot + kPart1, part2, kPart2 / 1024, wave, lane);
+    else if (inproj)
+      dma_pieces<kWaves>(P.in_packed + kPiece, part2, kPiece / 1024, wave, lane);
   }
   store32<true>(io, P.pre, kFF, kHC * (kNF - 1), sp0, sp1);
   store32<true>(io, P.h, kFF, kHC * (kNF - 1), sh0, sh1);
@@ -460,6 +527,38 @@
     const f32x4 y1 = v[s][1] * rstd * *(const f32x4*)(par + 4 * kC + n0 + 4) + *(const f32x4*)(par + 5 * kC + n0 + 4);
     store32<SST_NT_OUT>(io, P.y2, kC, 32 * s, y0, y1);
     if (prow != nullptr) store32<SST_NT_OUT>(io, P.y2p, kC, 32 * s, y0 + *(const f32x4*)(prow + n0), y1 + *(const f32x4*)(prow + n0 + 4));
+    v[s][0] = y0, v[s][1] = y1;
+  }
+  if (!inproj) return;
+  const float* qrow = P.in_pos_table + (size_t)P.in_pos_idx[row] * kC;
+  const float* bin = par + kParF;
+  img3 yb[4];
+#pragma unroll
+  for (int s = 0; s < 4; ++s) yb[s] = split8(v[s][0], v[s][1]);
+  barrier_drain();
+#pragma unroll 1
+  for (int oc = 0; oc < kNIn; ++oc) {
+    if (oc == 2) {
+#pragma unroll
+      for (int s = 0; s < 4; ++s) {
+        const int n0 = 32 * s + 8 * g;
+        yb[s] = split8(add4(v[s][0], *(const f32x4*)(qrow + n0)), add4(v[s][1], *(const f32x4*)(qrow + n0 + 4)));
+      }
+    }
+    f32x4 a4[4] = {z4, z4, z4, z4};
+    mma_inproj<0>(lds, lane * 16, yb, a4);
+    barrier_drain();
+    if (oc + 1 < kNIn) dma_pieces<kWaves>(P.in_packed + (size_t)(2 * oc + 2) * kPiece, lds, kPiece / 1024, wave, lane);
+    mma_inproj<1>(part2, lane * 16, yb, a4);
+    barrier_drain();
+    if (oc + 1 < kNIn) dma_pieces<kWaves>(P.in_packed + (size_t)(2 * oc + 3) * kPiece, part2, kPiece / 1024, wave, lane);
+    const int col0 = 64 * inproj_chunk(oc);
+#pragma unroll
+    for (int tp = 0; tp < 2; ++tp) {
+      const int n0 = col0 + 32 * tp + 8 * g;
+      store32<false>(io, P.qkv, kCI, col0 + 32 * tp, add4(a4[2 * tp], *(const f32x4*)(bin + n0)),
+                     add4(a4[2 * tp + 1], *(const f32x4*)(bin + n0 + 4)));
+    }
   }
 }
 
@@ -751,6 +850,26 @@
   return sst_encoder_tail_pack_f32x6_many(&d_w_out, &d_w1, &d_w2, &d_packed, 1, stream);
 }
 
+int64_t sst_encoder_tail_inproj_pack_bytes(void) { return kPackIn; }
+
+int sst_encoder_tail_inproj_pack_f32x6_many(const float* const* d_w_in, void* const* d_packed, int n, void* stream) {
+  if (n < 0 || (n > 0 && (!d_w_in || !d_packed))) return SST_ERR_ARG;
+  for (int i = 0; i < n; ++i)
+    if (!d_w_in[i] || !d_packed[i] || !aligned16(d_w_in[i]) || !aligned16(d_packed[i])) return SST_ERR_ARG;
+  for (int base = 0; base < n; base += kPackMany) {
+    pack_in_batch B;
+    const int cnt = n - base < kPackMany ? n - base : kPackMany;
+    for (int i = 0; i < cnt; ++i) B.w[i] = d_w_in[base + i], B.dst[i] = (unsigned char*)d_packed[base + i];
+    hipLaunchKernelGGL(encoder_tail_pack_inproj_k, dim3(cnt * 2 * kNIn), dim3(512), kPiece, (hipStream_t)stream, B);
+  }
+  SST_LAUNCH_CHECK();
+  return SST_OK;
+}
+
+int sst_encoder_tail_inproj_pack_f32x6(const float* d_w_in, void* d_packed, void* stream) {
+  return sst_encoder_tail_inproj_pack_f32x6_many(&d_w_in, &d_packed, 1, stream);
+}
+
 int64_t sst_encoder_tail_bwd_workspace_bytes(int64_t m) {
   if (m < 0) return SST_ERR_ARG;
   return sst_align_up(2 * sst_div_up(m > 0 ? m : 1, (int64_t)kRowsPerWg) * 2 * kC * (int64_t)sizeof(float), 256);
@@ -765,12 +884,21 @@
   if ((a->s1 && !aligned16(a->s1)) || (a->s2 && !aligned16(a->s2))) return SST_ERR_ARG;
   if ((a->pos_table != nullptr) != (a->pos_idx != nullptr) || (a->pos_table != nullptr) != (a->y2p != nullptr)) return SST_ERR_ARG;
   if (a->pos_table && (!aligned16(a->pos_table) || !aligned16(a->y2p))) return SST_ERR_ARG;
+  const bool inproj = a->in_packed != nullptr;
+  if (inproj != (a->in_pos_table != nullptr) || inproj != (a->in_pos_idx != nullptr) || inproj != (a->qkv_next != nullptr) ||
+      (!inproj && a->in_bias != nullptr))
+    return SST_ERR_ARG;
+  if (inproj && (!aligned16(a->in_packed) || !aligned16(a->in_pos_table) || !aligned16(a->qkv_next) ||
+                 (a->in_bias && !aligned16(a->in_bias))))
+    return SST_ERR_ARG;
   tail_fwd_params P;
   P.o = a->o, P.x = a->x, P.packed = (const unsigned char*)a->packed;
   P.b_out = a->b_out, P.b1 = a->b1, P.b2 = a->b2, P.n1w = a->n1w, P.n1b = a->n1b, P.n2w = a->n2w, P.n2b = a->n2b;
   P.eps = a->eps, P.m = a->m;
   P.s1 = a->s1, P.st1 = a->st1, P.y1 = a->y1, P.pre = a->pre, P.h = a->h, P.s2 = a->s2, P.st2 = a->st2, P.y2 = a->y2;
   P.pos_table = a->pos_table, P.pos_idx = a->pos_idx, P.y2p = a->y2p;
+  P.in_packed = (const unsigned char*)a->in_packed, P.in_bias = a->in_bias, P.in_pos_table = a->in_pos_table;
+  P.in_pos_idx = a->in_pos_idx, P.qkv = a->qkv_next;
   const int64_t rows = sst_div_up(a->m, (int64_t)kRowsPerWg);
   if (rows > 0x7fffffff) return SST_ERR_UNSUPPORTED;
   hipStream_t st = (hipStream_t)stream;
diff --git a/sst_amd/dense.py b/sst_amd/dense.py
--- a/sst_amd/dense.py
+++ b/sst_amd/dense.py
@@ -395,7 +395,35 @@
     return out
 
 
-def encoder_tail_fwd(o, x, packed, b_out, b1, b2, n1w, n1b, n2w, n2b, eps, act, save=True, pos=None, out=None):
+def encoder_tail_inproj_pack(w_ins, out=None):
+    import ctypes
+    lib = _lib.load()
+    single = torch.is_tensor(w_ins)
+    ws = [w_ins] if single else list(w_ins)
+    n = len(ws)
+    nbytes = int(lib.sst_encoder_tail_inproj_pack_bytes())
+    if out is None:
+        out = torch.empty(n * nbytes, dtype=torch.uint8, device=ws[0].device)
+    views = [out[i * nbytes:(i + 1) * nbytes] for i in range(n)]
+    P = ctypes.c_void_p * n
+    _lib.check(lib.sst_encoder_tail_inproj_pack_f32x6_many(P(*[w.data_ptr() for w in ws]), P(*[v.data_ptr() for v in views]), n,
+                                                           _lib.stream_ptr()), 'sst_encoder_tail_inproj_pack_f32x6_many')
+    return views[0] if single else views
+
+
+def encoder_tail_inproj_ok(w_in, b_in, pos_spec, m):
+    if _MATMUL_MODE != 'f32x6' or pos_spec is None:
+        return False
+    table, idx = pos_spec
+    return (w_in.shape == (384, 128) and w_in.is_cuda and w_in.dtype == torch.float32 and w_in.is_contiguous()
+            and w_in.data_ptr() % 16 == 0
+            and (b_in is None or (b_in.shape == (384,) and b_in.dtype == torch.float32 and b_in.is_contiguous()
+                                  and b_in.data_ptr() % 16 == 0))
+            and table.dtype == torch.float32 and table.dim() == 2 and table.size(1) == 128 and table.is_contiguous()
+            and table.data_ptr() % 16 == 0 and idx.dtype == torch.int32 and idx.is_contiguous() and idx.numel() == m)
+
+
+def encoder_tail_fwd(o, x, packed, b_out, b1, b2, n1w, n1b, n2w, n2b, eps, act, save=True, pos=None, out=None, inproj=None):
     m = x.size(0)
     dev = x.device
     out = dict(out) if out else {}
@@ -409,11 +437,14 @@
     st1, y1, pre, h, s2, st2, y2 = e('st1', 2), e('y1', 128), e('pre', 256), e('h', 256), e('s2', 128), e('st2', 2), e('y2', 128)
     y2p = e('y2p', 128) if pos is not None else None
     out['y2p'] = y2p
+    qkv_next = e('qkv_next', 384) if inproj is not None else None
+    out['qkv_next'] = qkv_next
     P = lambda t: None if t is None else t.data_ptr()
     args = _lib.EncoderTailFwdArgs(
         m, 1 if act == 'gelu' else 2, 0, float(eps), 0.0, P(o), P(x), P(packed), P(b_out), P(b1), P(b2), P(n1w), P(n1b),
         P(n2w), P(n2b), P(pos[0]) if pos is not None else None, P(pos[1]) if pos is not None else None,
-        P(s1), P(st1), P(y1), P(pre), P(h), P(s2), P(st2), P(y2), P(y2p))
+        P(s1), P(st1), P(y1), P(pre), P(h), P(s2), P(st2), P(y2), P(y2p),
+        *((P(inproj[0]), P(inproj[1]), P(inproj[2][0]), P(inproj[2][1]), P(qkv_next)) if inproj is not None else ()))
     import ctypes
     _lib.check(_lib.load().sst_encoder_tail_fwd_f32x6(ctypes.byref(args), _lib.stream_ptr()), 'sst_encoder_tail_fwd_f32x6')
     return out
diff --git a/sst_amd/sst_basic_block.py b/sst_amd/sst_basic_block.py
--- a/sst_amd/sst_basic_block.py
+++ b/sst_amd/sst_basic_block.py
@@ -9,6 +9,7 @@
 from . import kernels as K
 from .sra_composed import sra_attention_composed
 from .dense import (encoder_tail_ok, encoder_tail_pack, encoder_tail_fwd, encoder_tail_bwd, inproj_pos_ok, inproj_pos,
+                    encoder_tail_inproj_ok, encoder_tail_inproj_pack,
                     EPI_ADD, EPI_BIAS, EPI_GELU, EPI_MUL_GELU_GRAD, EPI_MUL_RELU_GRAD, EPI_RELU, lds_linear, lds_linear_ok,
                     lds_linear_add_ln, lds_linear_add_ln_ok, lds_linear_dqkv_ok, lds_linear_qkv, lds_linear_qkv_ok,
                     weight_bias_grad_group,
@@ -162,6 +163,7 @@
 
 _LAYER_EXEC = int(_os.environ.get('SST_AMD_LAYER_EXEC', '1'))
 _POS_FOLD = int(_os.environ.get('SST_AMD_POS_FOLD', '1'))
+_TAIL_INPROJ = int(_os.environ.get('SST_AMD_TAIL_INPROJ', '0'))
 
 
 def _layer_exec_ok(x, xp, plan, nhead, act, params):
@@ -196,15 +198,27 @@
     return out, off
 
 
+def _handed_qkv(t, m):
+    if t.dtype == torch.uint8:
+        return t[:m * 384 * 4].view(torch.float32).view(m, 384)
+    return t
+
+
 def _layer_exec_fwd(x, xp, plan, nhead, impl, act, params, eps, scale, pos_next, need_bwd, head_scale=None, pos_spec=None,
-                    wpack=None):
+                    wpack=None, qkv_in=None, next_in=None):
     from . import _lib
     import ctypes
     w_in, b_in, w_out, b_out, w1, b1, w2, b2, n1w, n1b, n2w, n2b = params
     m = x.size(0)
     dev = x.device
     offs, total = _slab_offsets(m)
-    slab = torch.empty(total, dtype=torch.uint8, device=dev)
+    if qkv_in is not None and qkv_in.dtype == torch.uint8 and qkv_in.numel() == total:
+        slab = qkv_in
+    else:
+        slab = torch.empty(total, dtype=torch.uint8, device=dev)
+        if qkv_in is not None:
+            _handed_qkv(slab, m).copy_(_handed_qkv(qkv_in, m))
+    next_slab = torch.empty(total, dtype=torch.uint8, device=dev) if next_in is not None else None
     base = slab.data_ptr()
     y2 = torch.empty((m, 128), dtype=torch.float32, device=dev)
     y2p = torch.empty((m, 128), dtype=torch.float32, device=dev) if pos_next is not None else None
@@ -223,12 +237,14 @@
         P(pos_next[0]) if pos_next is not None else None, P(pos_next[1]) if pos_next is not None else None,
         S('qkv'), S('o'), S('lse'), S('y1'), S('s1') if need_bwd else None, S('st1'), S('pre'), S('h'), S('s2'), P(y2), S('st2'),
         P(y2p), P(head_scale), P(wpack), P(pos_spec[0]) if pos_spec is not None else None,
-        P(pos_spec[1]) if pos_spec is not None else None)
+        P(pos_spec[1]) if pos_spec is not None else None,
+        *((P(next_in[0]), P(next_in[2]), P(next_in[3][0]), P(next_in[3][1]), next_slab.data_ptr() + offs['qkv'])
+          if next_in is not None else (None,) * 5), 1 if qkv_in is not None else 0)
     rc = K._bracket('sra_fwd', plan.n_tokens, lambda: lib.sst_encoder_layer_fwd_f32x6(ctypes.byref(args), _lib.stream_ptr()))
     if rc == _lib.SST_ERR_UNSUPPORTED:
         return None
     _lib.check(rc, 'sst_encoder_layer_fwd_f32x6')
-    return slab, y2, y2p, wpack
+    return slab, y2, y2p, wpack, next_slab
 
 
 def _layer_exec_bwd(ctx, dy2, dy2p, saved):
@@ -280,7 +296,7 @@
     _lib.check(rc, 'sst_encoder_layer_bwd_f32x6')
     d_scale = K.head_scale_grad(cos_r, head_scale) if head_scale is not None else None
     return (ds1, None, None, None, None, None, dw_in, db_in, dwo, dbo, dw1, db1, dw2, db2, dn[0], dn[1], dn[2], dn[3], None, None,
-            None, d_scale, None, None, None, None)
+            None, d_scale, None, None, None, None, None, None)
 
 
 def _bn_rows_fwd(bn, s):
@@ -325,7 +341,8 @@
 
     @staticmethod
     def forward(ctx, x, pos, plan, nhead, impl, act, w_in, b_in, w_out, b_out, w1, b1, w2, b2, n1w, n1b, n2w, n2b, eps,
-                xp=None, pos_next=None, head_scale=None, xp_shares_x=False, pos_spec=None, bn=None, wpack=None):
+                xp=None, pos_next=None, head_scale=None, xp_shares_x=False, pos_spec=None, bn=None, wpack=None, qkv_in=None,
+                next_in=None):
         c = x.size(1)
         x = x.contiguous()
         if head_scale is not None:
@@ -347,24 +364,37 @@
         if xp is None and not ctx.pos_fold:
             xp = x + pos if pos is not None else x
         params = (w_in, b_in, w_out, b_out, w1, b1, w2, b2, n1w, n1b, n2w, n2b)
+        if not ctx.pos_fold:
+            qkv_in = None
+        qkv_next = None
+
+        def result(y2, y2p):
+            nonlocal qkv_next
+            ctx.two = pos_next is not None
+            outs = (y2, y2p) if ctx.two else (y2,)
+            if next_in is not None:
+                if qkv_next is None:
+                    qkv_next = inproj_pos(y2, next_in[3], next_in[1], next_in[2])
+                ctx.mark_non_differentiable(qkv_next)
+                outs = outs + (qkv_next,)
+            return outs if len(outs) > 1 else outs[0]
         ctx.exec = False
         ctx.bn = bn is not None
         if bn is None and c == 128 and ctx.fold_xp and _layer_exec_ok(x, xp, plan, nhead, act, params):
             need_bwd = any(ctx.needs_input_grad)
             scale = 1.0 / math.sqrt(16.0)
             done = _layer_exec_fwd(x, xp, plan, nhead, impl, act, params, eps, scale, pos_next, need_bwd, head_scale,
-                                   pos_spec if ctx.pos_fold else None, wpack)
+                                   pos_spec if ctx.pos_fold else None, wpack, qkv_in, next_in)
             if done is not None:
-                slab, y2, y2p, wpack = done
+                slab, y2, y2p, wpack, qkv_next = done
                 if need_bwd:
                     ctx.save_for_backward(x, xp if xp is not None else x, slab, w_in, w_out, w1, w2, n1w, n2w, wpack,
                                           *(pos_spec if ctx.pos_fold else ()), *((head_scale,) if ctx.cosine else ()))
                     ctx.plan, ctx.nhead, ctx.impl, ctx.act, ctx.scale = plan, nhead, impl, act, scale
                     ctx.exec = True
-                ctx.two = pos_next is not None
-                return (y2, y2p) if ctx.two else y2
+                return result(y2, y2p)
         if ctx.pos_fold:
-            qkv = inproj_pos(x, pos_spec, w_in, b_in)
+            qkv = _handed_qkv(qkv_in, x.size(0)) if qkv_in is not None else inproj_pos(x, pos_spec, w_in, b_in)
             qk, v = qkv[:, :2 * c], qkv[:, 2 * c:]
             xp = x
         elif _LDS_LINEAR and c == 128 and lds_linear_qkv_ok(xp, x, w_in):
@@ -390,7 +420,9 @@
                 and encoder_tail_ok(o, x, w_out, w1, w2) and all(t is not None for t in (b_out, b1, b2))):
             if wpack is None:
                 wpack = encoder_tail_pack(w_out, w1, w2)
-            t = encoder_tail_fwd(o, x, wpack, b_out, b1, b2, n1w, n1b, n2w, n2b, eps, act, save=need_bwd, pos=pos_next)
+            t = encoder_tail_fwd(o, x, wpack, b_out, b1, b2, n1w, n1b, n2w, n2b, eps, act, save=need_bwd, pos=pos_next,
+                                 inproj=(next_in[0], next_in[2], next_in[3]) if next_in is not None else None)
+            qkv_next = t['qkv_next']
             s1, st1, y1, pre, h, s2, st2, y2, y2p = (t[k] for k in ('s1', 'st1', 'y1', 'pre', 'h', 's2', 'st2', 'y2', 'y2p'))
             ctx.tail = True
         else:
@@ -401,8 +433,7 @@
                                   *((wpack,) if ctx.tail else ()), *(pos_spec if ctx.pos_fold else ()),
                                   *((head_scale,) if ctx.cosine else ()))
             ctx.plan, ctx.nhead, ctx.impl, ctx.act, ctx.scale = plan, nhead, impl, act, scale
-        ctx.two = pos_next is not None
-        return (y2, y2p) if ctx.two else y2
+        return result(y2, y2p)
 
     @staticmethod
     def _tail_batch_norm(o, x, w_out, b_out, w1, b1, w2, b2, bn, act, pos_next):
@@ -454,8 +485,9 @@
         return y1, s1, st1, pre, h, s2, st2, y2, y2p
 
     @staticmethod
-    def backward(ctx, dy2, dy2p=None):
+    def backward(ctx, dy2, *more):
         from . import dense as _dense
+        dy2p = more[0] if (ctx.two and more) else None
         with _dense.matmul_mode_scope(ctx.matmul):
             return FusedEncoderLayerFn._backward(ctx, dy2, dy2p)
 
@@ -533,7 +565,7 @@
         else:
             dx = ds1.addmm_(dqkv, w_in)
         return (dx, None, None, None, None, None, dw_in, db_in, dwo, dbo, dw1, db1, dw2, db2, dn1w, dn1b, dn2w, dn2b,
-                None, dxp, None, d_scale, None, None, None, None)
+                None, dxp, None, d_scale, None, None, None, None, None, None)
 
 
 class _StackHeadScales(torch.autograd.Function):
@@ -626,39 +658,57 @@
     layers = [enc for block in blocks for enc in block.encoder_list]
     wpacks = stack_tail_images(layers, feats) if (mode == 'f32x6' and _LDS_LINEAR) else [None] * n_layers
 
-    def layer(enc, li, x, xp):
+    next_ins = [None] * n_layers
+    if fold and _TAIL_INPROJ and feats.is_cuda:
+        take = []
+        for li in range(n_layers - 1):
+            nxt = layers[li + 1].win_attn.self_attn
+            if (li // 2 in checkpoint_blocks or (li + 1) // 2 in checkpoint_blocks or wpacks[li] is None or wpacks[li + 1] is None
+                    or not encoder_tail_inproj_ok(nxt.in_proj_weight, nxt.in_proj_bias, pos_specs[(li + 1) % 2], feats.size(0))):
+                continue
+            take.append(li)
+        if take:
+            with torch.no_grad():
+                imgs = encoder_tail_inproj_pack([layers[li + 1].win_attn.self_attn.in_proj_weight for li in take])
+            for li, img in zip(take, imgs):
+                nxt = layers[li + 1].win_attn.self_attn
+                next_ins[li] = (img, nxt.in_proj_weight, nxt.in_proj_bias, pos_specs[(li + 1) % 2])
+
+    def layer(enc, li, x, xp, qkv):
         attn = enc.win_attn.self_attn
         if fold:
             out = FusedEncoderLayerFn.apply(
                 x, None, plans[li % 2], enc.win_attn.nhead, enc.win_attn.impl, enc.act_name, attn.in_proj_weight,
                 attn.in_proj_bias, attn.out_proj.weight, attn.out_proj.bias, enc.linear1.weight, enc.linear1.bias,
                 enc.linear2.weight, enc.linear2.bias, enc.norm1.weight, enc.norm1.bias, enc.norm2.weight, enc.norm2.bias,
-                enc.norm1.eps, None, None, scales[li], False, pos_specs[li % 2], enc.bn_modules(), wpacks[li])
-            return out, None
+                enc.norm1.eps, None, None, scales[li], False, pos_specs[li % 2], enc.bn_modules(), wpacks[li], qkv, next_ins[li])
+            return (out[0], None, out[1]) if next_ins[li] is not None else (out, None, None)
         pos_next = pos_specs[(li + 1) % 2] if li + 1 < n_layers else None
         out = FusedEncoderLayerFn.apply(
             x, None, plans[li % 2], enc.win_attn.nhead, enc.win_attn.impl, enc.act_name, attn.in_proj_weight,
             attn.in_proj_bias, attn.out_proj.weight, attn.out_proj.bias, enc.linear1.weight, enc.linear1.bias,
             enc.linear2.weight, enc.linear2.bias, enc.norm1.weight, enc.norm1.bias, enc.norm2.weight, enc.norm2.bias,
             enc.norm1.eps, xp, pos_next, scales[li], True, None, enc.bn_modules(), wpacks[li])
-        return out if pos_next is not None else (out, None)
+        return (out[0], out[1], None) if pos_next is not None else (out, None, None)
 
     def block_fn(bi):
-        def run(x, xp):
+        def run(x, second):
+            xp, qkv = (None, second) if fold else (second, None)
             with _dense.matmul_mode_scope(mode):
                 for j, enc in enumerate(blocks[bi].encoder_list):
-                    x, xp = layer(enc, 2 * bi + j, x, xp)
-            return (x, xp) if xp is not None else (x,)
+                    x, xp, qkv = layer(enc, 2 * bi + j, x, xp, qkv)
+            second = qkv if fold else xp
+            return (x, second) if second is not None else (x,)
         return run
 
     x = feats.contiguous()
-    xp = None if fold else K.add_table_rows(x, pos_specs[0][0], pos_specs[0][1])
+    second = None if fold else K.add_table_rows(x, pos_specs[0][0], pos_specs[0][1])
     for bi in range(len(blocks)):
         if bi in checkpoint_blocks and torch.is_grad_enabled():
-            out = checkpoint(block_fn(bi), x, xp, use_reentrant=False)
-        else:
-            out = block_fn(bi)(x, xp)
-        x, xp = (out[0], out[1]) if len(out) > 1 else (out[0], None)
+            out = checkpoint(block_fn(bi), x, second, use_reentrant=False)
+        else:
+            out = block_fn(bi)(x, second)
+        x, second = (out[0], out[1]) if len(out) > 1 else (out[0], None)
     return x
 
 
```

After: 98.75. 0.97x the previous value.
